# nzfeng/signed-heat-3d

Hardware: AMD Instinct MI355X
Metric: grid-nodes/sec end-to-end SHM (conv+PCG) (higher is better)
Workload: dtype f64 (Step 1: f64 / packed-f32 tiers)

## Files before the change

include/shm_grid.h:

```cpp
#ifndef SHM_GRID_H
#define SHM_GRID_H

#include <stddef.h>
#include <stdint.h>

#ifdef __cplusplus
extern "C" {
#endif

#define SHM_GRID_ABI_VERSION 5

typedef struct shm_solver shm_solver;

typedef enum {
    SHM_OK = 0,
    SHM_ERR_INVALID = 1,
    SHM_ERR_HIP = 2,
    SHM_ERR_NOMEM = 3,
    SHM_ERR_BREAKDOWN = 4,
    SHM_ERR_NOCONV = 5,
    SHM_ERR_RCCL = 6,
    SHM_ERR_STATE = 7,
    SHM_ERR_SINGULAR = 8
} shm_status;
// ... 24 lines not shown
    int32_t n;
    double bbox_min[3];
    double cell;
} shm_grid;

typedef struct {
    int32_t fast_integration;
    int32_t scrub_nonfinite;
    double tol;
    int32_t max_iters;
    int32_t check_every;
    int32_t preconditioner;
    int32_t solver;
    int32_t step1_arith;
    int32_t dual_form;
    double step1_budget;
} shm_opts;

enum { SHM_DUAL_AUTO = 0, SHM_DUAL_DIRECT = 1, SHM_DUAL_EXPLICIT_S_CG = 2, SHM_DUAL_THROUGH_GRID = 3 };

enum { SHM_STEP1_AUTO = 0, SHM_STEP1_EXACT_F64 = 1, SHM_STEP1_REFERENCE_F64 = 2 };

enum { SHM_SOLVER_AUTO = 0, SHM_SOLVER_PRIMAL = 1, SHM_SOLVER_DUAL = 2, SHM_SOLVER_DUAL_SLABS = 3 };

enum { SHM_PRECOND_AUTO = 0, SHM_PRECOND_NONE = 1, SHM_PRECOND_DCT = 2 };

typedef struct {
    int32_t n, m;
    int64_t S;
    int32_t iters;
    double rel_residual;
    double shift;
    double ms_conv;
    double ms_div;
    double ms_setup;
    double ms_wait_setup;
    double ms_pcg;
    double ms_shift;
    double ms_total;
    double ms_stencil_avg;
    double ms_update_xr_avg;
    double ms_project_avg;
    double ms_update_p_avg;
    double ms_precond_avg;
    int32_t kernel_samples;
    int32_t preconditioner;
    int32_t solver;
    double bytes_per_iter;
    int32_t cg_form;
    double pairs_fp64;
    double pairs_fp32;
    int32_t conv_launches;
    double pairs_redone;
} shm_stats;

shm_status shm_grid_create(const shm_config* cfg, shm_solver** out);
void shm_grid_destroy(shm_solver* s);
const char* shm_grid_last_error(const shm_solver* s);
int32_t shm_grid_abi_version(void);

shm_status shm_grid_set_problem(shm_solver* s, const shm_sources* src, const shm_grid* grid);
shm_status shm_grid_solve(shm_solver* s, const shm_opts* opts, shm_stats* stats);
shm_status shm_grid_get_phi(shm_solver* s, double* phi_out, int32_t* k_begin, int32_t* k_end);
shm_status shm_grid_owned_planes(shm_solver* s, int32_t* k_begin, int32_t* k_end);
shm_status shm_grid_compute_distance(shm_solver* s, const shm_sources* src, const shm_grid* grid,
                                     const shm_opts* opts, double* phi_out, shm_stats* stats);

typedef enum {
    SHM_FIELD_Y0 = 0,
    SHM_FIELD_Y1 = 1,
    SHM_FIELD_Y2 = 2,
    SHM_FIELD_DIV = 3,
    SHM_FIELD_PHI = 4
} shm_field;
shm_status shm_grid_run_conv(shm_solver* s);
shm_status shm_grid_run_conv_arith(shm_solver* s, int32_t step1_arith);
shm_status shm_grid_run_divergence(shm_solver* s, int32_t scrub);
shm_status shm_grid_get_field(shm_solver* s, shm_field f, double* out );
shm_status shm_grid_get_field_planes(shm_solver* s, shm_field f, int32_t k_begin, int32_t k_end, double* out);
shm_status shm_grid_apply_laplacian(shm_solver* s, const double* u, double* out);
shm_status shm_grid_set_phi(shm_solver* s, const double* phi );
shm_status shm_grid_get_constraints(shm_solver* s, int64_t* nodes, double* coeffs, int32_t* m);
shm_status shm_grid_get_schur(shm_solver* s, double* out, int32_t* m);
shm_status shm_grid_spd_solve(shm_solver* s, const double* S, int32_t m, const double* rhs, int32_t form, double* u, int32_t* flag);
shm_status shm_grid_apply_projector(shm_solver* s, double* v);

shm_status shm_grid_apply_preconditioner(shm_solver* s, const double* v, double* out);

enum { SHM_ISO_MARCHING_CUBES = 0, SHM_ISO_MARCHING_TETS = 1 };
shm_status shm_grid_isosurface(shm_solver* s, double isovalue, int64_t* n_vertices, int64_t* n_triangles);
shm_status shm_grid_isosurface_ex(shm_solver* s, double isovalue, int32_t method, int64_t* n_vertices, int64_t* n_triangles);
shm_status shm_grid_get_isosurface(shm_solver* s, double* vertices , int64_t* triangles );

shm_status shm_grid_sample(shm_solver* s, int64_t Q, const double* pts, double* phi_out, double* grad_out, int64_t* n_answered);
shm_status shm_grid_sample_device(shm_solver* s, int64_t Q, const void* d_pts, void* d_phi, void* d_grad, int64_t* n_answered);

shm_status shm_grid_isosurface_indexed(shm_solver* s, double isovalue, int64_t* n_vertices, int64_t* n_triangles);
shm_status shm_grid_get_isosurface_indexed(shm_solver* s, double* vertices , int64_t* triangles );
shm_status shm_grid_get_isosurface_indexed_device(shm_solver* s, void* d_vertices , void* d_triangles );

typedef struct {
    int64_t first_vertex;
    int64_t n_vertices, n_triangles;
    double  area, volume;
    double  lo[3], hi[3];
    int32_t touches_box;
    int32_t reserved;
} shm_iso_component;
shm_status shm_grid_label_mesh_device(shm_solver* s, int64_t nv, int64_t nt, const void* d_triangles , void* d_root , int64_t* n_components);
shm_status shm_grid_isosurface_components(shm_solver* s, int64_t* n_components);
shm_status shm_grid_get_isosurface_components(shm_solver* s, shm_iso_component* comps , int64_t* tri_component ,
                                              int64_t* vertex_component );
shm_status shm_grid_isosurface_keep_components(shm_solver* s, const uint8_t* keep , int64_t* n_vertices, int64_t* n_triangles);

typedef struct {
    int64_t n_audited, n_not_owned, n_nonfinite, n_out_of_zone, n_finite_mismatch;
    double  max_dy;
    int64_t worst_node;
    double  worst_ratio;
    double  min_ratio;
    double  budget;
    int32_t step1_arith;
    int32_t within_budget;
    double  ms;
} shm_step1_audit;
shm_status shm_grid_audit_step1(shm_solver* s, int64_t count, const int64_t* nodes, double* dy_out , double* ratio_out ,
                                shm_step1_audit* out);
int64_t shm_audit_sample_nodes(int32_t n, int32_t k_begin, int32_t k_end, int64_t count, uint64_t seed, int64_t* nodes_out);

shm_status shm_grid_raycast(shm_solver* s, int64_t Q, const double* origins , const double* dirs , double isovalue, double t_min, double t_max,
                            double* t_out , double* grad_out , int64_t* n_hits);
shm_status shm_grid_raycast_device(shm_solver* s, int64_t Q, const void* d_origins, const void* d_dirs, double isovalue, double t_min, double t_max, void* d_t,
                                   void* d_grad, int64_t* n_hits);

typedef struct {
    int64_t n_frozen;
    int64_t n_reached;
    int64_t n_nonfinite;
    int64_t n_block_updates;
    int32_t n_rounds;
    int32_t reserved;
    double max_abs;
    double isovalue, band;
    double ms;
} shm_redistance_stats;
shm_status shm_grid_redistance(shm_solver* s, double isovalue, double band, shm_redistance_stats* out );
shm_status shm_grid_get_redistanced(shm_solver* s, double* psi_out );
shm_status shm_grid_get_redistanced_device(shm_solver* s, void* d_psi );

typedef struct {
    int64_t n_vertices, n_triangles;
    int64_t n_reached;
    int64_t n_candidate_pairs;
    double max_abs;
    double isovalue, band;
    double ms;
} shm_redistance_exact_stats;
shm_status shm_grid_redistance_exact(shm_solver* s, double isovalue, double band, shm_redistance_exact_stats* out );
shm_status shm_grid_isosurface_indexed_psi(shm_solver* s, double distance, int64_t* n_vertices, int64_t* n_triangles);

shm_status shm_grid_closest_point(shm_solver* s, int64_t Q, const double* pts , double max_dist, double* dist_out ,
                                  double* cp_out , int64_t* tri_out , int64_t* n_answered);
shm_status shm_grid_closest_point_device(shm_solver* s, int64_t Q, const void* d_pts, double max_dist, void* d_dist, void* d_cp ,
                                         void* d_tri , int64_t* n_answered);

shm_status shm_comm_unique_id(void* out128);
// ... 9 lines not shown
```

signed-heat-3d_amd/csrc/shm_dct.hip.h:

```cpp
#pragma once
#include <hip/hip_runtime.h>
#include <stdint.h>

#include "shm_fft_core.h"
#include "shm_kernels.hip.h"

#ifndef SHM_DCT_HOIST
#define SHM_DCT_HOIST 0
#endif
#ifndef SHM_DCT_WAVES_HINT
#define SHM_DCT_WAVES_HINT 9
#endif
#ifndef SHM_DCT_WAVES_F32
#define SHM_DCT_WAVES_F32 2
#endif
#ifndef SHM_DCT_SPECTRAL_ORIG
#define SHM_DCT_SPECTRAL_ORIG 0
#endif
#ifndef SHM_DCT_RUNTIME_GATE
#define SHM_DCT_RUNTIME_GATE 1
#endif
#ifndef SHM_DCT_WAVES_256
#define SHM_DCT_WAVES_256 0
#endif
#ifndef SHM_DCT_WAVE_FFT
#define SHM_DCT_WAVE_FFT 0x100
#endif
#ifndef SHM_DCT_LC9_F64
#define SHM_DCT_LC9_F64 4
#endif
#ifndef SHM_DCT_LC10_F32
#define SHM_DCT_LC10_F32 4
#endif
#ifndef SHM_DCT_LC9_F32
#define SHM_DCT_LC9_F32 8
#endif
#ifndef SHM_DCT_LC8
#define SHM_DCT_LC8 4
#endif
#ifndef SHM_DCT_TW_LDS_MAX
#define SHM_DCT_TW_LDS_MAX 8
#endif
#ifndef SHM_DCT_POW_ALWAYS
#define SHM_DCT_POW_ALWAYS 1
#endif

namespace shm {

#if SHM_DCT_RUNTIME_GATE
#define SHM_DCT_DBG(P, bit) ((P).debug_skip & (bit))
#else
#define SHM_DCT_DBG(P, bit) 0
#endif

enum DctMode : int { DCT_FWD = 0, DCT_INV = 1, DCT_FUSED = 2 };
template <int LOG2N, int TB > constexpr int dct_lc() {
    return LOG2N >= 10 ? (TB == 8 ? 4 : SHM_DCT_LC10_F32) : (LOG2N == 8 ? SHM_DCT_LC8 : (LOG2N == 9 ? (TB == 8 ? SHM_DCT_LC9_F64 : SHM_DCT_LC9_F32) : 8));
}
constexpr int dct_lines_for(int log2n, int tb) {
    return log2n >= 10 ? (tb == 8 ? 8 : 2 * SHM_DCT_LC10_F32) : (log2n == 8 ? 2 * SHM_DCT_LC8 : (log2n == 9 ? 2 * (tb == 8 ? SHM_DCT_LC9_F64 : SHM_DCT_LC9_F32) : 16));
}

struct DctAddr {
    long long off;
    long long a_stride, b_stride;
    long long line_stride;
    long long elem_stride;
    long long seg_stride;
    int seg_shift, seg_mask;
};
struct DctParams {
    int ntiles;
    int tiles_a;
    int debug_skip;
    DctAddr in, out;
    int ky0;
    double inv_n3_8;
};
__device__ __forceinline__ long long dct_addr(const DctAddr& A, long long base, int l, int k) {
    return A.off + base + (long long)l * A.line_stride + (long long)(k >> A.seg_shift) * A.seg_stride + (long long)(k & A.seg_mask) * A.elem_stride;
}

template <int LOG2N> constexpr bool dct_tw_in_lds() { return LOG2N <= SHM_DCT_TW_LDS_MAX; }
template <int LOG2N, int TB> constexpr size_t dct_lds_bytes() {
    return ((size_t)(1 << LOG2N) * (dct_lc<LOG2N, TB>() + 1) + (dct_tw_in_lds<LOG2N>() ? (size_t)(1 << LOG2N) : 0)) * (size_t)(2 * TB) + 64;
}

template <int LOG2N, int TB> constexpr size_t dct_stage_bytes() { return (size_t)(1 << LOG2N) * (size_t)(2 * dct_lc<LOG2N, TB>()) * (size_t)TB; }

template <typename TP, int LOG2N, int R, int NS, int SIGN>
__device__ __forceinline__ void dct_fft_pass(Cplx<TP>* buf, const Cplx<TP>* tw, int tid) {
    constexpr int LC = dct_lc<LOG2N, (int)sizeof(TP)>();
    constexpr int items = PassGeom<LOG2N, R, LC>::items;
    constexpr int IPT = (items + kBlock - 1) / kBlock;
    Cplx<TP> v[IPT][R];
#pragma unroll
    for (int a = 0; a < IPT; a++) {
        const int w = tid + a * kBlock;
        if (items % kBlock == 0 || w < items) pass_load<TP, LOG2N, R, NS, SIGN, LC, SHM_DCT_POW_ALWAYS || !dct_tw_in_lds<LOG2N>()>(buf, tw, w, v[a]);
    }
    __syncthreads();
#pragma unroll
    for (int a = 0; a < IPT; a++) {
        const int w = tid + a * kBlock;
        if (items % kBlock == 0 || w < items) pass_store<TP, LOG2N, R, NS, LC>(buf, w, v[a]);
    }
    __syncthreads();
}

template <typename TP, int LOG2N, int SIGN>
__device__ __forceinline__ void dct_fft(Cplx<TP>* buf, const Cplx<TP>* tw, int tid) {
    typedef FftPlan<LOG2N> P;
    dct_fft_pass<TP, LOG2N, P::R0, 1, SIGN>(buf, tw, tid);
    if constexpr (P::npass > 1) dct_fft_pass<TP, LOG2N, P::R1, P::R0, SIGN>(buf, tw, tid);
    if constexpr (P::npass > 2) dct_fft_pass<TP, LOG2N, P::R2, P::R0 * P::R1, SIGN>(buf, tw, tid);
    if constexpr (P::npass > 3) dct_fft_pass<TP, LOG2N, P::R3, P::R0 * P::R1 * P::R2, SIGN>(buf, tw, tid);
}

template <int LOG2N> struct FftPlanWave;
template <> struct FftPlanWave<8> { static constexpr int npass = 4; static constexpr int R0 = 4, R1 = 4, R2 = 4, R3 = 4; };
#ifndef SHM_DCT_WAVE_PLAN9
#define SHM_DCT_WAVE_PLAN9 0
#endif
#if SHM_DCT_WAVE_PLAN9
template <> struct FftPlanWave<9> { static constexpr int npass = 3; static constexpr int R0 = 8, R1 = 8, R2 = 8, R3 = 1; };
#else
template <> struct FftPlanWave<9> { static constexpr int npass = 4; static constexpr int R0 = 8, R1 = 4, R2 = 4, R3 = 4; };
#endif
template <> struct FftPlanWave<10> { static constexpr int npass = 4; static constexpr int R0 = 16, R1 = 4, R2 = 4, R3 = 4; };
template <int LOG2N> constexpr bool dct_wave_fft() { return ((SHM_DCT_WAVE_FFT >> LOG2N) & 1) && LOG2N >= 8 && LOG2N <= 10; }

template <typename TP, int LOG2N, int R, int NS, int SIGN>
__device__ __forceinline__ void dct_fft_pass_wave(Cplx<TP>* buf, const Cplx<TP>* tw, int tid) {
    constexpr int LC = dct_lc<LOG2N, (int)sizeof(TP)>(), n = 1 << LOG2N;
    constexpr int B = n / R;
    constexpr int LW = LC / (kBlock / kWave);
    constexpr int IPL = (B + kWave - 1) / kWave;
    static_assert(LW >= 1 && B % kWave == 0, "wave-local FFT: whole lines per wave, full waves of butterflies");
    const int wave = tid >> 6, lane = tid & 63;
    Cplx<TP> v[LW * IPL][R];
#pragma unroll
    for (int a = 0; a < LW * IPL; a++) {
        const int c = wave + (kBlock / kWave) * (a / IPL), jj = lane + kWave * (a % IPL);
        pass_load<TP, LOG2N, R, NS, SIGN, LC, SHM_DCT_POW_ALWAYS || !dct_tw_in_lds<LOG2N>()>(buf, tw, jj * LC + c, v[a]);
    }
    __builtin_amdgcn_wave_barrier();
#pragma unroll
    for (int a = 0; a < LW * IPL; a++) {
        const int c = wave + (kBlock / kWave) * (a / IPL), jj = lane + kWave * (a % IPL);
        pass_store<TP, LOG2N, R, NS, LC>(buf, jj * LC + c, v[a]);
    }
    __builtin_amdgcn_wave_barrier();
}

template <typename TP, int LOG2N, int SIGN>
__device__ __forceinline__ void dct_fft_wave(Cplx<TP>* buf, const Cplx<TP>* tw, int tid) {
    typedef FftPlanWave<LOG2N> P;
    dct_fft_pass_wave<TP, LOG2N, P::R0, 1, SIGN>(buf, tw, tid);
    dct_fft_pass_wave<TP, LOG2N, P::R1, P::R0, SIGN>(buf, tw, tid);
    dct_fft_pass_wave<TP, LOG2N, P::R2, P::R0 * P::R1, SIGN>(buf, tw, tid);
    if constexpr (P::npass > 3) dct_fft_pass_wave<TP, LOG2N, P::R3, P::R0 * P::R1 * P::R2, SIGN>(buf, tw, tid);
}

#ifndef SHM_DCT_SEG9_ONE_WAVE
#define SHM_DCT_SEG9_ONE_WAVE 1
#endif
template <int LOG2N, int CPLX_BYTES> constexpr int dct_waves_per_simd() {
    constexpr int by_lds = (int)((size_t)(160 * 1024) / dct_lds_bytes<LOG2N, CPLX_BYTES / 2>());
    constexpr int want = LOG2N <= 8 ? (SHM_DCT_WAVES_256 > 0 ? SHM_DCT_WAVES_256 : 1) : (CPLX_BYTES == 8 ? SHM_DCT_WAVES_F32 : 2);
    return by_lds >= want ? want : (by_lds >= 1 ? by_lds : 1);
}
template <typename TP, typename TIn, typename TOut, int MODE, bool DOT, int LOG2N, bool XPASS, bool SEG, bool PF = false>
__global__ __launch_bounds__(kBlock, ((LOG2N >= SHM_DCT_WAVES_HINT || SHM_DCT_WAVES_256 > 0) && !(SHM_DCT_SEG9_ONE_WAVE && SEG && LOG2N == 9 && sizeof(TP) == 8) ? dct_waves_per_simd<LOG2N, (int)sizeof(Cplx<TP>)>() : 1)) void dct_lines_kernel(DctParams P, const TIn* __restrict__ in, TOut* __restrict__ out,
                                                           const Cplx<TP>* __restrict__ tw_g, const Cplx<TP>* __restrict__ om_g,
                                                           const TP* __restrict__ lam_g, const TOut* __restrict__ dot_with,
                                                           double* __restrict__ partials, const int* __restrict__ tile_list ,
                                                           const unsigned* __restrict__ elem_mask ) {
    extern __shared__ __attribute__((aligned(16))) char smem[];
    constexpr int LC = dct_lc<LOG2N, (int)sizeof(TP)>(), kFftRow = LC + 1, kFftLC = LC;
    constexpr int n = 1 << LOG2N, L = 2 * LC, LOG2L = ilog2(L), total = n * L;
    constexpr int EPT = (total + kBlock - 1) / kBlock;
    constexpr int CH = EPT < 16 ? EPT : 16;
    Cplx<TP>* buf = reinterpret_cast<Cplx<TP>*>(smem);
    Cplx<TP>* tw_l = buf + (size_t)n * kFftRow;
    double* red = reinterpret_cast<double*>(tw_l + (dct_tw_in_lds<LOG2N>() ? n : 0));
    const Cplx<TP>* tw = dct_tw_in_lds<LOG2N>() ? tw_l : tw_g;
    const int tid = threadIdx.x;
    if (dct_tw_in_lds<LOG2N>())
        for (int a = tid; a < n; a += kBlock) tw_l[a] = tw_g[a];
    constexpr int kSpStep = kBlock / kFftLC;
    constexpr int kSpIters = (n / 2 + 1 + kSpStep - 1) / kSpStep;
    Cplx<TP> sp_om[(MODE == DCT_FWD || !SHM_DCT_HOIST) ? 1 : kSpIters];
    TP sp_lam[(MODE == DCT_FUSED && SHM_DCT_HOIST) ? kSpIters : 1];
    TP sp_lam_n = (TP)0;
    if (MODE != DCT_FWD && SHM_DCT_HOIST) {
#pragma unroll
        for (int i = 0; i < kSpIters; i++) {
            const int k = min((tid >> ilog2(kFftLC)) + i * kSpStep, n / 2);
            sp_om[i] = om_g[k];
            if (MODE == DCT_FUSED) sp_lam[i] = lam_g[k];
        }
    }
    if (MODE == DCT_FUSED) sp_lam_n = (TP)2 * lam_g[n / 2];
    static_assert(!PF || !SEG, "the prefetching variant serves plain layouts");
    static_assert(!PF || (sizeof(TIn) == sizeof(TP) && (total * sizeof(TIn)) % (16 * kBlock) == 0), "the prefetching variant moves whole 16-byte chunks of same-width input");
    TIn* stage = reinterpret_cast<TIn*>(smem + dct_lds_bytes<LOG2N, (int)sizeof(TP)>());
    auto pf_issue = [&](int lbx) {
        if constexpr (PF) {
            constexpr int kChunkElems = 16 / (int)sizeof(TIn);
            constexpr int kChunks = total / kChunkElems, kPer = kChunks / kBlock;
            const int tx = lbx;
            const long long bin = P.in.off + (long long)(tx % P.tiles_a) * P.in.a_stride + (long long)(tx / P.tiles_a) * P.in.b_stride;
            const int wave0 = (tid >> 6) << 6;
#pragma unroll
            for (int a = 0; a < kPer; a++) {
                const int q = a * kBlock + tid;
                long long g;
                if (XPASS) {
                    constexpr int cpl = n / kChunkElems;
                    g = (long long)(q / cpl) * P.in.line_stride + (long long)((q % cpl) * kChunkElems);
                } else {
                    constexpr int cpr = L / kChunkElems;
                    g = (long long)(q / cpr) * P.in.elem_stride + (long long)((q % cpr) * kChunkElems);
                }
                __builtin_amdgcn_global_load_lds(reinterpret_cast<const char*>(in + (bin + g)), reinterpret_cast<char*>(stage) + (size_t)(a * kBlock + wave0) * 16, 16, 0, 0);
            }
        }
    };
    if (PF) {
        const int lb0 = (int)xcd_remap(blockIdx.x, gridDim.x);
        if (lb0 < P.ntiles) pf_issue(lb0);
    }
    for (int lb = (int)xcd_remap(blockIdx.x, gridDim.x); lb < P.ntiles; lb += (int)gridDim.x) {
    __syncthreads();
    const int t = tile_list ? tile_list[lb] : lb;
    const long long base_in = (long long)(t % P.tiles_a) * P.in.a_stride + (long long)(t / P.tiles_a) * P.in.b_stride;
    const long long base_out = (long long)(t % P.tiles_a) * P.out.a_stride + (long long)(t / P.tiles_a) * P.out.b_stride;

    auto line_of = [&](int idx) { return XPASS ? (idx >> LOG2N) : (idx & (L - 1)); };
    auto elem_of = [&](int idx) { return XPASS ? (idx & (n - 1)) : (idx >> LOG2L); };
    auto thread_off = [&](const DctAddr& A) -> unsigned {
        if (XPASS) return n >= kBlock ? (unsigned)(tid * A.elem_stride) : (unsigned)((tid >> LOG2N) * A.line_stride + (tid & (n - 1)) * A.elem_stride);
        return (unsigned)((tid & (L - 1)) * A.line_stride + (tid >> LOG2L) * A.elem_stride);
    };
    auto uniform_off = [&](const DctAddr& A, int a) -> long long {
        if (XPASS) {
            constexpr int per = n >= kBlock ? n / kBlock : 1, lp = n >= kBlock ? 1 : kBlock / n;
            return n >= kBlock ? (long long)(a / per) * A.line_stride + (long long)((a % per) * kBlock) * A.elem_stride : (long long)(a * lp) * A.line_stride;
        }
        return (long long)(a * (kBlock / L)) * A.elem_stride;
    };
    const unsigned toff_in = SEG ? 0u : thread_off(P.in), toff_out = SEG ? 0u : thread_off(P.out);
    auto in_at = [&](const TIn* base, int a, int idx) -> const TIn* {
        return SEG ? base + dct_addr(P.in, base_in, line_of(idx), elem_of(idx)) : (base + (P.in.off + base_in + uniform_off(P.in, a))) + toff_in;
    };
    auto out_at = [&](auto* base, int a, int idx) {
        return SEG ? base + dct_addr(P.out, base_out, line_of(idx), elem_of(idx)) : (base + (P.out.off + base_out + uniform_off(P.out, a))) + toff_out;
    };

    if constexpr (PF) {
        __builtin_amdgcn_s_waitcnt(0x0f70);
        __syncthreads();
#pragma unroll
        for (int a0 = 0; a0 < EPT; a0 += CH) {
            TP v[CH];
#pragma unroll
            for (int a = 0; a < CH; a++) v[a] = (TP)stage[tid + (a0 + a) * kBlock];
#pragma unroll
            for (int a = 0; a < CH; a++) {
                const int idx = tid + (a0 + a) * kBlock;
                const int l = line_of(idx), j = elem_of(idx);
                const int slot = (MODE == DCT_INV) ? j : makhoul_slot(j, n);
                reinterpret_cast<TP*>(&buf[slot * kFftRow + (l >> 1)])[l & 1] = v[a];
            }
        }
        __syncthreads();
        if (lb + (int)gridDim.x < P.ntiles) pf_issue(lb + (int)gridDim.x);
    } else
#pragma unroll 1
    for (int a0 = 0; a0 < EPT; a0 += CH) {
        TP v[CH];
#pragma unroll
        for (int a = 0; a < CH; a++) {
            const int idx = tid + (a0 + a) * kBlock;
            if (total % kBlock == 0 || idx < total) {
                const int j = elem_of(idx);
                v[a] = (!SHM_DCT_DBG(P, 4) && (!elem_mask || ((elem_mask[j >> 5] >> (j & 31)) & 1u))) ? (TP)*in_at(in, a0 + a, idx) : (TP)0;
            }
        }
#pragma unroll
        for (int a = 0; a < CH; a++) {
            const int idx = tid + (a0 + a) * kBlock;
            if (total % kBlock == 0 || idx < total) {
                const int l = line_of(idx), j = elem_of(idx);
                const int slot = (MODE == DCT_INV) ? j : makhoul_slot(j, n);
                reinterpret_cast<TP*>(&buf[slot * kFftRow + (l >> 1)])[l & 1] = v[a];
            }
        }
    }
    __syncthreads();

    constexpr bool kWaveFft = dct_wave_fft<LOG2N>();
    if ((MODE == DCT_FWD || MODE == DCT_FUSED) && !SHM_DCT_DBG(P, 1)) {
        if constexpr (kWaveFft) dct_fft_wave<TP, LOG2N, -1>(buf, tw, tid);
        else dct_fft<TP, LOG2N, -1>(buf, tw, tid);
    }
    if (kWaveFft && MODE == DCT_FWD) __syncthreads();

    if (MODE == DCT_FWD) {
#pragma unroll 1
        for (int a0 = 0; a0 < EPT; a0 += CH) {
#pragma unroll
            for (int a = 0; a < CH; a++) {
                const int idx = tid + (a0 + a) * kBlock;
                if (total % kBlock == 0 || idx < total) {
                    const int l = line_of(idx), k = elem_of(idx), c = l >> 1;
                    TP xa, xb;
                    dct_fwd_post<TP>(buf[k * kFftRow + c], buf[((n - k) & (n - 1)) * kFftRow + c], om_g[k], xa, xb);
                    *out_at(out, a0 + a, idx) = (TOut)((l & 1) ? xb : xa);
                }
            }
        }
        continue;
    }

#if SHM_DCT_SPECTRAL_ORIG
    if (!SHM_DCT_DBG(P, 2)) {
        const int kx0 = (t % P.tiles_a) * L, ky = P.ky0 + t / P.tiles_a;
        constexpr int pairs = (n / 2 + 1) * kFftLC;
        for (int b = tid; b < pairs; b += kBlock) {
            const int c = b & (kFftLC - 1), k = b >> ilog2(kFftLC);
            const int nk = (n - k) & (n - 1);
            const Cplx<TP> omk = om_g[k], omn = om_g[nk];
            TP xa_k, xb_k, xa_n, xb_n;
            if (MODE == DCT_FUSED) {
                const Cplx<TP> zk = buf[k * kFftRow + c], znk = buf[nk * kFftRow + c];
                dct_fwd_post<TP>(zk, znk, omk, xa_k, xb_k);
                dct_fwd_post<TP>(znk, zk, omn, xa_n, xb_n);
                const int kxa = kx0 + 2 * c, kxb = kxa + 1;
                const TP lxy_a = lam_g[kxa] + lam_g[ky], lxy_b = lam_g[kxb] + lam_g[ky];
                const TP sy = ky == 0 ? (TP)0.5 : (TP)1;
                const TP sa = (kxa == 0 ? (TP)0.5 : (TP)1) * sy * (TP)P.inv_n3_8, sb = sy * (TP)P.inv_n3_8;
                const TP lk = lam_g[k], ln = lam_g[nk];
                const TP szk = k == 0 ? (TP)0.5 : (TP)1;
                const TP da_k = lxy_a + lk, db_k = lxy_b + lk, da_n = lxy_a + ln, db_n = lxy_b + ln;
                auto recip = [](TP d) {
                    TP r = t_rcp<TP>(d);
                    r = fma(fma(-d, r, (TP)1), r, r);
                    r = fma(fma(-d, r, (TP)1), r, r);
                    return r;
                };
                xa_k = da_k > (TP)0 ? xa_k * (sa * szk) * recip(da_k) : (TP)0;
                xb_k = xb_k * (sb * szk) * recip(db_k);
                xa_n = da_n > (TP)0 ? xa_n * (sa * szk) * recip(da_n) : (TP)0;
                xb_n = xb_n * (sb * szk) * recip(db_n);
            } else {
                const Cplx<TP> rk = buf[k * kFftRow + c], rn = buf[nk * kFftRow + c];
                xa_k = rk.x; xb_k = rk.y; xa_n = rn.x; xb_n = rn.y;
            }
            buf[k * kFftRow + c] = dct_inv_pre<TP>(k, xa_k, xa_n, xb_k, xb_n, omk);
            if (nk != k) buf[nk * kFftRow + c] = dct_inv_pre<TP>(nk, xa_n, xa_k, xb_n, xb_k, omn);
        }
        __syncthreads();
    }

#else
    if (!SHM_DCT_DBG(P, 2)) {
        const int kx0 = (t % P.tiles_a) * L, ky = P.ky0 + t / P.tiles_a;
        constexpr int kSpLines = kWaveFft ? kFftLC / (kBlock / kWave) : 1;
#pragma unroll
        for (int cl = 0; cl < kSpLines; cl++) {
        const int c = kWaveFft ? (tid >> 6) + (kBlock / kWave) * cl : (tid & (kFftLC - 1));
        const int kxa = kx0 + 2 * c, kxb = kxa + 1;
        TP lxy_a = (TP)0, lxy_b = (TP)0, sa = (TP)0, sb = (TP)0;
        if (MODE == DCT_FUSED) {
            const TP lky = lam_g[ky];
            lxy_a = lam_g[kxa] + lky;
            lxy_b = lam_g[kxb] + lky;
            const TP sy = ky == 0 ? (TP)0.5 : (TP)1;
            sa = (kxa == 0 ? (TP)0.5 : (TP)1) * sy * (TP)P.inv_n3_8;
            sb = sy * (TP)P.inv_n3_8;
        }
#pragma unroll 1
        for (int i = 0; i < (kWaveFft ? (n / 2 + kWave) / kWave : kSpIters); i++) {
            const int k = kWaveFft ? (tid & 63) + i * kWave : (tid >> ilog2(kFftLC)) + i * kSpStep;
            if (k > n / 2) break;
            const int nk = (n - k) & (n - 1);
            const Cplx<TP> omk = SHM_DCT_HOIST ? sp_om[SHM_DCT_HOIST ? i : 0] : om_g[k];
            const Cplx<TP> omn = k == 0 ? omk : Cplx<TP>{-omk.y, -omk.x};
            TP xa_k, xb_k, xa_n, xb_n;
            if (MODE == DCT_FUSED) {
                const Cplx<TP> zk = buf[k * kFftRow + c], znk = buf[nk * kFftRow + c];
                dct_fwd_post<TP>(zk, znk, omk, xa_k, xb_k);
                dct_fwd_post<TP>(znk, zk, omn, xa_n, xb_n);
                const TP lk = SHM_DCT_HOIST ? sp_lam[SHM_DCT_HOIST ? i : 0] : lam_g[k], ln = k == 0 ? lk : sp_lam_n - lk;
                const TP szk = k == 0 ? (TP)0.5 : (TP)1;
                const TP da_k = lxy_a + lk, db_k = lxy_b + lk, da_n = lxy_a + ln, db_n = lxy_b + ln;
                auto recip = [](TP d) {
                    TP r = t_rcp<TP>(d);
                    r = fma(fma(-d, r, (TP)1), r, r);
                    r = fma(fma(-d, r, (TP)1), r, r);
                    return r;
                };
                xa_k = da_k > (TP)0 ? xa_k * (sa * szk) * recip(da_k) : (TP)0;
                xb_k = xb_k * (sb * szk) * recip(db_k);
                xa_n = da_n > (TP)0 ? xa_n * (sa * szk) * recip(da_n) : (TP)0;
                xb_n = xb_n * (sb * szk) * recip(db_n);
            } else {
                const Cplx<TP> rk = buf[k * kFftRow + c], rn = buf[nk * kFftRow + c];
                xa_k = rk.x; xb_k = rk.y; xa_n = rn.x; xb_n = rn.y;
            }
            buf[k * kFftRow + c] = dct_inv_pre<TP>(k, xa_k, xa_n, xb_k, xb_n, omk);
            if (nk != k) buf[nk * kFftRow + c] = dct_inv_pre<TP>(nk, xa_n, xa_k, xb_n, xb_k, omn);
        }
        }
        if (!kWaveFft) __syncthreads();
    }

#endif
    if (!SHM_DCT_DBG(P, 1)) {
        if constexpr (kWaveFft) dct_fft_wave<TP, LOG2N, +1>(buf, tw, tid);
        else dct_fft<TP, LOG2N, +1>(buf, tw, tid);
    }
    if (kWaveFft) __syncthreads();

    double acc = 0.;
#pragma unroll 1
    for (int a0 = 0; a0 < EPT; a0 += CH) {
        TOut dv[CH];
        if (DOT) {
#pragma unroll
            for (int a = 0; a < CH; a++) {
                const int idx = tid + (a0 + a) * kBlock;
                if (total % kBlock == 0 || idx < total)
                    dv[a] = *out_at(dot_with, a0 + a, idx);
            }
        }
#pragma unroll
        for (int a = 0; a < CH; a++) {
            const int idx = tid + (a0 + a) * kBlock;
            if (total % kBlock == 0 || idx < total) {
                const int l = line_of(idx), j = elem_of(idx);
                const TP v = reinterpret_cast<const TP*>(&buf[makhoul_slot(j, n) * kFftRow + (l >> 1)])[l & 1];
                if (!SHM_DCT_DBG(P, 8) && (!elem_mask || ((elem_mask[j >> 5] >> (j & 31)) & 1u))) *out_at(out, a0 + a, idx) = (TOut)v;
                if (DOT) acc += (double)v * (double)dv[a];
            }
        }
    }
    if (DOT) {
        acc = block_sum(acc, red);
        if (tid == 0) partials[t] = acc;
    }
    }
}

constexpr int kZsPer = 4;
__device__ __forceinline__ double zs_block_exclusive(double v, double* buf , double& total) {
    const int t = threadIdx.x;
    int cur = 0;
    buf[t] = v;
    __syncthreads();
    for (int off = 1; off < kBlock; off <<= 1) {
        const double x = buf[cur * kBlock + t] + (t >= off ? buf[cur * kBlock + t - off] : 0.);
        buf[(cur ^ 1) * kBlock + t] = x;
        cur ^= 1;
        __syncthreads();
    }
    const double incl = buf[cur * kBlock + t];
    total = buf[cur * kBlock + kBlock - 1];
    __syncthreads();
    return incl - v;
}
template <typename T>
__device__ void zsolve_zero_line(int n, int n_act, const int* __restrict__ planes, double inv_h2, const T* __restrict__ in, T* __restrict__ out) {
    __shared__ double fz[kBlock * kZsPer], buf[2 * kBlock];
    const int t = threadIdx.x;
    const size_t plane = (size_t)n * n;
    for (int a = t; a < kBlock * kZsPer; a += kBlock) fz[a] = 0.;
    __syncthreads();
    for (int a = t; a < n_act; a += kBlock) fz[planes[a]] = (double)in[(size_t)planes[a] * plane];
    __syncthreads();
    double f[kZsPer], loc = 0., tot = 0.;
#pragma unroll
    for (int e = 0; e < kZsPer; e++) {
        const int z = t * kZsPer + e;
        f[e] = z < n ? fz[z] : 0.;
        loc += f[e];
    }
    zs_block_exclusive(loc, buf, tot);
    const double fmean = tot / n;
    loc = 0.;
#pragma unroll
    for (int e = 0; e < kZsPer; e++) {
        const int z = t * kZsPer + e;
        f[e] = z < n ? f[e] - fmean : 0.;
        loc += f[e];
    }
    double before = zs_block_exclusive(loc, buf, tot);
    double g[kZsPer];
#pragma unroll
    for (int e = 0; e < kZsPer; e++) {
        before += f[e];
        g[e] = -before;
    }
    loc = 0.;
#pragma unroll
    for (int e = 0; e < kZsPer; e++) loc += (t * kZsPer + e < n) ? g[e] : 0.;
    before = zs_block_exclusive(loc, buf, tot);
    double u[kZsPer], usum = 0.;
#pragma unroll
    for (int e = 0; e < kZsPer; e++) {
        const int z = t * kZsPer + e;
        u[e] = before / inv_h2;
        before += z < n ? g[e] : 0.;
        usum += z < n ? u[e] : 0.;
    }
    zs_block_exclusive(usum, buf, tot);
    const double umean = tot / n;
    const double scale = 0.25 * 4.0 / ((double)n * (double)n);
#pragma unroll
    for (int e = 0; e < kZsPer; e++) fz[t * kZsPer + e] = u[e] - umean;
    __syncthreads();
    for (int a = t; a < n_act; a += kBlock) out[(size_t)planes[a] * plane] = (T)(scale * fz[planes[a]]);
}

constexpr int kZsChunk = 16;
template <typename T>
// ... 86 lines not shown
```

signed-heat-3d_amd/csrc/shm_grid.hip:

```cpp
#include "shm_host.hip.h"
#include "shm_audit_sample.h"


struct shm_solver {
    std::unique_ptr<shm::SolverBase> impl;
    std::string err;
    shm_config cfg;
};

static thread_local std::string g_create_error;

template <typename F> static shm_status guard(shm_solver* s, F&& f) {
    if (!s) return SHM_ERR_INVALID;
    try {
        f();
        s->err.clear();
        return SHM_OK;
    } catch (const shm::Error& e) {
        s->err = e.what();
        return e.code;
    } catch (const std::bad_alloc&) {
        s->err = "host allocation failed";
        return SHM_ERR_NOMEM;
    } catch (const std::exception& e) {
// ... 82 lines not shown
    return guard(s, [&] {
        if (!src || !grid) throw shm::Error(SHM_ERR_INVALID, "null argument");
        s->impl->set_problem(*src, *grid);
    });
}

shm_status shm_grid_solve(shm_solver* s, const shm_opts* opts, shm_stats* stats) {
    return guard(s, [&] {
        shm_opts o;
        memset(&o, 0, sizeof o);
        o.scrub_nonfinite = 1;
        if (opts) o = *opts;
        s->impl->solve(o, stats);
    });
}

shm_status shm_grid_get_phi(shm_solver* s, double* phi_out, int32_t* k_begin, int32_t* k_end) {
    return guard(s, [&] {
        if (!phi_out) throw shm::Error(SHM_ERR_INVALID, "null phi_out");
        s->impl->get_phi(phi_out, k_begin, k_end);
    });
}

shm_status shm_grid_owned_planes(shm_solver* s, int32_t* k_begin, int32_t* k_end) {
    return guard(s, [&] { s->impl->owned_planes(k_begin, k_end); });
}

shm_status shm_grid_compute_distance(shm_solver* s, const shm_sources* src, const shm_grid* grid, const shm_opts* opts, double* phi_out,
                                     shm_stats* stats) {
    shm_status rc = shm_grid_set_problem(s, src, grid);
    if (rc != SHM_OK) return rc;
    if (s->cfg.world != 1) {
        s->err = "shm_grid_compute_distance is the single-process entry point; use set_problem/solve/get_phi per rank";
        return SHM_ERR_INVALID;
    }
    rc = shm_grid_solve(s, opts, stats);
    if (rc != SHM_OK && rc != SHM_ERR_NOCONV) return rc;
    std::string keep = s->err;
    shm_status rc2 = shm_grid_get_phi(s, phi_out, nullptr, nullptr);
    if (rc2 != SHM_OK) return rc2;
    s->err = keep;
    return rc;
}

shm_status shm_grid_run_conv(shm_solver* s) { return guard(s, [&] { s->impl->run_conv(SHM_STEP1_AUTO); }); }
shm_status shm_grid_run_conv_arith(shm_solver* s, int32_t step1_arith) { return guard(s, [&] { s->impl->run_conv(step1_arith); }); }
shm_status shm_grid_run_divergence(shm_solver* s, int32_t scrub) { return guard(s, [&] { s->impl->run_divergence(scrub); }); }
shm_status shm_grid_get_field(shm_solver* s, shm_field f, double* out) {
    return guard(s, [&] {
        if (!out) throw shm::Error(SHM_ERR_INVALID, "null out");
        s->impl->get_field(f, out);
    });
}
shm_status shm_grid_get_field_planes(shm_solver* s, shm_field f, int32_t k_begin, int32_t k_end, double* out) {
    return guard(s, [&] {
        if (!out) throw shm::Error(SHM_ERR_INVALID, "null out");
        s->impl->get_field_planes(f, k_begin, k_end, out);
    });
}
shm_status shm_grid_apply_laplacian(shm_solver* s, const double* u, double* out) {
    return guard(s, [&] {
        if (!u || !out) throw shm::Error(SHM_ERR_INVALID, "null argument");
        s->impl->apply_laplacian(u, out);
    });
}
shm_status shm_grid_set_phi(shm_solver* s, const double* phi) {
    return guard(s, [&] {
        if (!phi) throw shm::Error(SHM_ERR_INVALID, "null argument");
        s->impl->set_phi(phi);
    });
}
shm_status shm_grid_get_constraints(shm_solver* s, int64_t* nodes, double* coeffs, int32_t* m) {
    return guard(s, [&] {
        if (!nodes || !coeffs || !m) throw shm::Error(SHM_ERR_INVALID, "null argument");
        s->impl->get_constraints(nodes, coeffs, m);
    });
}
shm_status shm_grid_get_schur(shm_solver* s, double* out, int32_t* m) {
    return guard(s, [&] {
        if (!out || !m) throw shm::Error(SHM_ERR_INVALID, "null argument");
        s->impl->get_schur(out, m);
    });
}
shm_status shm_grid_spd_solve(shm_solver* s, const double* S, int32_t m, const double* rhs, int32_t form, double* u, int32_t* flag) {
    return guard(s, [&] {
        if (!S || !rhs || !u || !flag) throw shm::Error(SHM_ERR_INVALID, "null argument");
        s->impl->spd_solve(S, m, rhs, form, u, flag);
    });
}
shm_status shm_grid_apply_projector(shm_solver* s, double* v) {
    return guard(s, [&] {
        if (!v) throw shm::Error(SHM_ERR_INVALID, "null argument");
        s->impl->apply_projector(v);
    });
}

shm_status shm_grid_apply_preconditioner(shm_solver* s, const double* v, double* out) {
    return guard(s, [&] {
        if (!v || !out) throw shm::Error(SHM_ERR_INVALID, "null argument");
        s->impl->apply_preconditioner(v, out);
    });
}

shm_status shm_grid_isosurface(shm_solver* s, double isovalue, int64_t* n_vertices, int64_t* n_triangles) {
    return guard(s, [&] { s->impl->isosurface(isovalue, SHM_ISO_MARCHING_CUBES, n_vertices, n_triangles); });
}
shm_status shm_grid_isosurface_ex(shm_solver* s, double isovalue, int32_t method, int64_t* n_vertices, int64_t* n_triangles) {
    return guard(s, [&] { s->impl->isosurface(isovalue, method, n_vertices, n_triangles); });
}
shm_status shm_grid_get_isosurface(shm_solver* s, double* vertices, int64_t* triangles) {
    return guard(s, [&] { s->impl->get_isosurface(vertices, triangles); });
}

shm_status shm_grid_isosurface_indexed(shm_solver* s, double isovalue, int64_t* n_vertices, int64_t* n_triangles) {
    return guard(s, [&] { s->impl->isosurface_indexed(isovalue, n_vertices, n_triangles); });
}
shm_status shm_grid_get_isosurface_indexed(shm_solver* s, double* vertices, int64_t* triangles) {
    return guard(s, [&] { s->impl->get_isosurface_indexed(vertices, triangles); });
}
shm_status shm_grid_get_isosurface_indexed_device(shm_solver* s, void* d_vertices, void* d_triangles) {
    return guard(s, [&] { s->impl->get_isosurface_indexed_device(d_vertices, d_triangles); });
}

shm_status shm_grid_label_mesh_device(shm_solver* s, int64_t nv, int64_t nt, const void* d_triangles, void* d_root, int64_t* n_components) {
    return guard(s, [&] { s->impl->label_mesh_device(nv, nt, d_triangles, d_root, n_components); });
}
shm_status shm_grid_isosurface_components(shm_solver* s, int64_t* n_components) {
    return guard(s, [&] { s->impl->isosurface_components(n_components); });
}
shm_status shm_grid_get_isosurface_components(shm_solver* s, shm_iso_component* comps, int64_t* tri_component, int64_t* vertex_component) {
    return guard(s, [&] { s->impl->get_isosurface_components(comps, tri_component, vertex_component); });
}
shm_status shm_grid_isosurface_keep_components(shm_solver* s, const uint8_t* keep, int64_t* n_vertices, int64_t* n_triangles) {
    return guard(s, [&] { s->impl->isosurface_keep_components(keep, n_vertices, n_triangles); });
}

shm_status shm_grid_sample(shm_solver* s, int64_t Q, const double* pts, double* phi_out, double* grad_out, int64_t* n_answered) {
    return guard(s, [&] { s->impl->sample(Q, pts, phi_out, grad_out, n_answered); });
}
shm_status shm_grid_sample_device(shm_solver* s, int64_t Q, const void* d_pts, void* d_phi, void* d_grad, int64_t* n_answered) {
    return guard(s, [&] { s->impl->sample_device(Q, d_pts, d_phi, d_grad, n_answered); });
}

shm_status shm_grid_raycast(shm_solver* s, int64_t Q, const double* origins, const double* dirs, double isovalue, double t_min, double t_max, double* t_out,
                            double* grad_out, int64_t* n_hits) {
    return guard(s, [&] { s->impl->raycast(Q, origins, dirs, isovalue, t_min, t_max, t_out, grad_out, n_hits); });
}
shm_status shm_grid_raycast_device(shm_solver* s, int64_t Q, const void* d_origins, const void* d_dirs, double isovalue, double t_min, double t_max, void* d_t,
                                   void* d_grad, int64_t* n_hits) {
    return guard(s, [&] { s->impl->raycast_device(Q, d_origins, d_dirs, isovalue, t_min, t_max, d_t, d_grad, n_hits); });
}

shm_status shm_grid_redistance(shm_solver* s, double isovalue, double band, shm_redistance_stats* out) {
    return guard(s, [&] { s->impl->redistance(isovalue, band, out); });
}
shm_status shm_grid_redistance_exact(shm_solver* s, double isovalue, double band, shm_redistance_exact_stats* out) {
    return guard(s, [&] { s->impl->redistance_exact(isovalue, band, out); });
}
shm_status shm_grid_isosurface_indexed_psi(shm_solver* s, double distance, int64_t* n_vertices, int64_t* n_triangles) {
    return guard(s, [&] { s->impl->isosurface_indexed_psi(distance, n_vertices, n_triangles); });
}
shm_status shm_grid_get_redistanced(shm_solver* s, double* psi_out) {
    return guard(s, [&] { s->impl->get_redistanced(psi_out); });
}
shm_status shm_grid_get_redistanced_device(shm_solver* s, void* d_psi) {
    return guard(s, [&] { s->impl->get_redistanced_device(d_psi); });
// ... 36 lines not shown
```

signed-heat-3d_amd/csrc/shm_host.hip.h:

```cpp
#pragma once
#include <hip/hip_runtime.h>
#include <rccl/rccl.h>

#include <dlfcn.h>

#include <algorithm>
#include <atomic>
#include <chrono>
#include <cmath>
#include <cstdarg>
#include <cstdio>
#include <cstring>
#include <limits>
#include <memory>
#include <mutex>
#include <stdexcept>
#include <string>
#include <thread>
#include <unordered_map>
#include <unordered_set>
#include <vector>

#include "../../include/shm_grid.h"
#include "shm_constraints.h"
// ... 409 lines not shown
                            lbs[(size_t)(s - g0)] = rel - lhs_drop;
                            if (lbs[(size_t)(s - g0)] <= ln_tau) {
                                bnd[(size_t)(s - g0)] = std::exp(lbs[(size_t)(s - g0)]) * r_hi / d_box;
                                gsum += bnd[(size_t)(s - g0)];
                            }
                        }
                        const bool soft_ok = R + gsum <= eps_soft;
                        if (soft_ok) R += gsum;
                        for (int64_t s = g0; s < g1; s++) {
                            if (!(wmag[(size_t)s] > 0.)) continue;
                            if (bnd[(size_t)(s - g0)] >= 0. && (soft_ok || lbs[(size_t)(s - g0)] <= ln_tau_hard)) continue;
                            const double lhs = lambda * (dist[(size_t)s] - rt - r_hi), rel = std::log(wmag[(size_t)s]) - ln_near;
                            const double d_box = std::max(0., dist[(size_t)s] - rt), d0 = std::max(0., dmin - rt);
                            const bool in_range = 1.4426950408889634 * lambda * (d_box - d0) + range_c <= std::log2(wmag[(size_t)s]) - lwhi;
                            cost += lhs > tier_log + rel && in_range ? far_cost : 1.0;
                        }
                    }
                } else {
                    for (size_t c = 0; c < crad.size(); c++) {
                        const double dx = cx - ccen[3 * c], dy = cy - ccen[3 * c + 1], dz = cz - ccen[3 * c + 2];
                        const double gap = std::sqrt(dx * dx + dy * dy + dz * dz) - rt - crad[c] - r_hi;
                        if (!(gap * lambda > skip_base + clnw[c] - ln_near)) cost += kCl;
                    }
                }
                acc += cost;
            }
        const double per_plane = acc / ((double)K * K * (double)S) + 1e-3;
        for (int k = L * bz; k < std::min(n, (L + 1) * bz); k++) weights[k] = per_plane;
    };
    const unsigned hw = std::thread::hardware_concurrency();
    const int nthr = (int)std::max(1u, std::min({hw ? hw : 1u, 16u, (unsigned)layers, (unsigned)(((double)layers * K * K * (double)S) / 2e6 + 1.)}));
    std::atomic<int> next{0};
    auto worker = [&]() {
        std::vector<double> dist((size_t)S);
        for (int L = next.fetch_add(1); L < layers; L = next.fetch_add(1)) do_layer(L, dist);
    };
    std::vector<std::thread> pool;
    for (int t = 1; t < nthr; t++) pool.emplace_back(worker);
    worker();
    for (std::thread& t : pool) t.join();
}

static void plan_slabs_weighted(int n, int nslabs, const double* w, int granule, std::vector<int32_t>& bounds) {
    bounds.assign((size_t)nslabs + 1, 0);
    bounds[(size_t)nslabs] = n;
    if (granule < 1) granule = 1;
    if ((long long)granule * nslabs > n) granule = std::max(1, n / nslabs);
    std::vector<double> cum((size_t)n + 1, 0.);
    for (int k = 0; k < n; k++) cum[(size_t)k + 1] = cum[(size_t)k] + (w && w[k] > 0. ? w[k] : 0.);
    if (!(cum[(size_t)n] > 0.))
        for (int k = 0; k <= n; k++) cum[(size_t)k] = k;
    for (int i = 1; i < nslabs; i++) {
        const double target = cum[(size_t)n] * i / nslabs;
        const int lo = bounds[(size_t)i - 1] + granule, hi = n - (nslabs - i) * granule;
        int best = lo;
        double best_err = 1e300;
        for (int k = ((lo + granule - 1) / granule) * granule; k <= hi; k += granule) {
            const double e = std::fabs(cum[(size_t)k] - target);
            if (e < best_err) {
                best_err = e;
                best = k;
            }
        }
        bounds[(size_t)i] = std::min(std::max(best, lo), std::max(lo, hi));
    }
}

struct SolverBase {
    virtual ~SolverBase() = default;
    virtual void set_problem(const shm_sources&, const shm_grid&) = 0;
    virtual void solve(const shm_opts&, shm_stats*) = 0;
    virtual void get_phi(double*, int32_t*, int32_t*) = 0;
    virtual void owned_planes(int32_t*, int32_t*) = 0;
    virtual void run_conv(int step1_arith) = 0;
    virtual void run_divergence(int scrub) = 0;
    virtual void get_field(shm_field, double*) = 0;
    virtual void get_field_planes(shm_field, int, int, double*) = 0;
    virtual void apply_laplacian(const double*, double*) = 0;
    virtual void set_phi(const double*) = 0;
    virtual void get_constraints(int64_t*, double*, int32_t*) = 0;
    virtual void apply_projector(double*) = 0;
    virtual void apply_preconditioner(const double*, double*) = 0;
    virtual void get_schur(double*, int32_t*) = 0;
    virtual void spd_solve(const double*, int32_t, const double*, int32_t, double*, int32_t*) = 0;
    virtual void isosurface(double, int, int64_t*, int64_t*) = 0;
    virtual void get_isosurface(double*, int64_t*) = 0;
    virtual void sample(int64_t, const double*, double*, double*, int64_t*) = 0;
    virtual void sample_device(int64_t, const void*, void*, void*, int64_t*) = 0;
    virtual void isosurface_indexed(double, int64_t*, int64_t*) = 0;
    virtual void get_isosurface_indexed(double*, int64_t*) = 0;
    virtual void get_isosurface_indexed_device(void*, void*) = 0;
    virtual void label_mesh_device(int64_t, int64_t, const void*, void*, int64_t*) = 0;
    virtual void isosurface_components(int64_t*) = 0;
    virtual void get_isosurface_components(shm_iso_component*, int64_t*, int64_t*) = 0;
    virtual void isosurface_keep_components(const uint8_t*, int64_t*, int64_t*) = 0;
    virtual void audit_step1(int64_t, const int64_t*, double*, double*, shm_step1_audit*) = 0;
    virtual void raycast(int64_t, const double*, const double*, double, double, double, double*, double*, int64_t*) = 0;
    virtual void raycast_device(int64_t, const void*, const void*, double, double, double, void*, void*, int64_t*) = 0;
    virtual void redistance(double, double, shm_redistance_stats*) = 0;
    virtual void get_redistanced(double*) = 0;
    virtual void get_redistanced_device(void*) = 0;
    virtual void redistance_exact(double, double, shm_redistance_exact_stats*) = 0;
    virtual void isosurface_indexed_psi(double, int64_t*, int64_t*) = 0;
    virtual void closest_point(int64_t, const double*, double, double*, double*, int64_t*, int64_t*) = 0;
    virtual void closest_point_device(int64_t, const void*, double, void*, void*, void*, int64_t*) = 0;
};

SolverBase* make_solver_f64(const shm_config& cfg);
SolverBase* make_solver_f32(const shm_config& cfg);

}
```

signed-heat-3d_amd/csrc/shm_kernels.hip.h:

```cpp
#pragma once
#include <hip/hip_runtime.h>
#include <stdint.h>

#include <type_traits>

#include "shm_constraints.h"
#include "shm_ldl_plan.h"
#include "shm_mc_table.h"

namespace shm {

constexpr int kBlock = 256;
constexpr int kMaxPartials = 8192;

__device__ __forceinline__ double wave_sum(double v) {
#pragma unroll
    for (int off = 32; off > 0; off >>= 1) v += __shfl_down(v, off, kWave);
    return v;
}

__device__ __forceinline__ double block_sum(double v, double* lds ) {
    v = wave_sum(v);
    const int lane = threadIdx.x & 63, w = threadIdx.x >> 6;
    if (lane == 0) lds[w] = v;
// ... 898 lines not shown
template <typename T>
__global__ __launch_bounds__(kBlock) void bfs_z_kernel(GridParams G, double cell, double bz, const T* __restrict__ Y0, const T* __restrict__ Y1,
                                                       const T* __restrict__ Y2, T* __restrict__ x) {
    const size_t plane = (size_t)G.n * G.n;
    const size_t ij = (size_t)blockIdx.x * kBlock + threadIdx.x;
    if (ij >= plane) return;
    const int kk0 = (G.k0 == 0) ? 1 : 0;
    double phi = -(double)x[(size_t)kk0 * plane + ij];
    for (int kk = kk0; kk < G.nzl; kk++) {
        const int k = G.k0 + kk;
        const double e2 = (k * cell + bz) - ((k - 1) * cell + bz);
        const size_t q = (size_t)(kk + 1) * plane + ij, pidx = q - plane;
        phi = phi + bfs_step<T>(Y0, Y1, Y2, pidx, q, 0., 0., e2);
        x[q] = (T)(-phi);
    }
}

constexpr int kDualBlock = 1024;

__device__ __forceinline__ double block_sum_1024(double v, double* lds ) {
    v = wave_sum(v);
    const int lane = threadIdx.x & 63, w = threadIdx.x >> 6;
    __syncthreads();
    if (lane == 0) lds[w] = v;
    __syncthreads();
    if (threadIdx.x == 0) {
        double s = 0.;
        for (int a = 0; a < kDualBlock / kWave; a++) s += lds[a];
        lds[16] = s;
    }
    __syncthreads();
    return lds[16];
}

template <typename T>
__global__ __launch_bounds__(kBlock) void scatter_rows_to_nodes_kernel(int nnodes, const uint32_t* __restrict__ node_id, const int* __restrict__ node_ptr,
                                                                       const int* __restrict__ ent_row, const double* __restrict__ ent_coef,
                                                                       const double* __restrict__ v, int accumulate, T* __restrict__ w, double scale = 1.0,
                                                                       T* __restrict__ saved = nullptr ) {
    const int t = blockIdx.x * kBlock + threadIdx.x;
    if (t >= nnodes) return;
    double s = 0.;
    for (int e = node_ptr[t]; e < node_ptr[t + 1]; e++) s += ent_coef[e] * v[ent_row[e]];
    const T old = w[node_id[t]];
    if (saved) saved[t] = old;
    w[node_id[t]] = (T)((accumulate ? (double)old : 0.) + scale * s);
}
template <typename T>
__global__ __launch_bounds__(kBlock) void restore_nodes_kernel(int nnodes, const uint32_t* __restrict__ node_id, const T* __restrict__ saved, T* __restrict__ w) {
    const int t = blockIdx.x * kBlock + threadIdx.x;
    if (t < nnodes) w[node_id[t]] = saved[t];
}

static __global__ __launch_bounds__(kBlock) void csr_matvec_kernel(int m, const int* __restrict__ ptr, const int* __restrict__ col, const double* __restrict__ val,
                                                            const double* __restrict__ x, double* __restrict__ y) {
    const int r = blockIdx.x * kBlock + threadIdx.x;
    if (r >= m) return;
    double s = 0.;
    for (int e = ptr[r]; e < ptr[r + 1]; e++) s += val[e] * x[col[e]];
    y[r] = s;
}

template <typename T>
__global__ __launch_bounds__(kBlock) void negate_kernel(size_t count, const T* __restrict__ in, T* __restrict__ out) {
    for (size_t v = (size_t)blockIdx.x * kBlock + threadIdx.x; v < count; v += (size_t)gridDim.x * kBlock) out[v] = -in[v];
}

template <typename T>
__global__ __launch_bounds__(kBlock) void sum_kernel(size_t nown, size_t off, const T* __restrict__ v, double* __restrict__ partials) {
    __shared__ double red[8];
    double acc = 0.;
    for (size_t a = (size_t)blockIdx.x * kBlock + threadIdx.x; a < nown; a += (size_t)gridDim.x * kBlock) acc += (double)v[off + a];
    acc = block_sum(acc, red);
    if (threadIdx.x == 0) partials[blockIdx.x] = acc;
}

static __global__ __launch_bounds__(kDualBlock) void dual_init_mu_kernel(int m, const double* __restrict__ sumb, double* __restrict__ mu, double* __restrict__ sc) {
    const double v = *sumb / (double)m;
    for (int a = threadIdx.x; a < m; a += kDualBlock) mu[a] = v;
    if (threadIdx.x == 0) sc[SC_SUMB] = *sumb;
}

static __global__ __launch_bounds__(kDualBlock) void dual_init_residual_kernel(int m, const double* __restrict__ g, const double* __restrict__ Smu,
                                                                        double* __restrict__ r, double* __restrict__ sc, int set_rr0 = 1) {
    __shared__ double lds[17];
    double s = 0.;
    for (int a = threadIdx.x; a < m; a += kDualBlock) s += g[a] - Smu[a];
    const double mean = block_sum_1024(s, lds) / (double)m;
    double rr = 0.;
    for (int a = threadIdx.x; a < m; a += kDualBlock) {
        const double v = g[a] - Smu[a] - mean;
        r[a] = v;
        rr += v * v;
    }
    rr = block_sum_1024(rr, lds);
    if (threadIdx.x == 0) {
        sc[SC_RR] = rr;
        if (set_rr0) sc[SC_RR0] = rr;
    }
}

static __global__ __launch_bounds__(kDualBlock) void dual_direction_kernel(int m, int init, const double* __restrict__ r, double* __restrict__ z,
                                                                    double* __restrict__ p, double* __restrict__ sc) {
    __shared__ double lds[17];
    double s = 0.;
    for (int a = threadIdx.x; a < m; a += kDualBlock) s += z[a];
    const double mean = block_sum_1024(s, lds) / (double)m;
    double rz = 0.;
    for (int a = threadIdx.x; a < m; a += kDualBlock) {
        const double v = z[a] - mean;
        z[a] = v;
        rz += r[a] * v;
    }
    rz = block_sum_1024(rz, lds);
    const double rz_old = sc[SC_RZ];
    const double beta = (init || rz_old == 0.) ? 0. : rz / rz_old;
    for (int a = threadIdx.x; a < m; a += kDualBlock) p[a] = init ? z[a] : z[a] + beta * p[a];
    __syncthreads();
    if (threadIdx.x == 0) sc[SC_RZ] = rz;
}

static __global__ __launch_bounds__(kDualBlock) void dual_update_kernel(int m, const double* __restrict__ Sp, const double* __restrict__ p, double* __restrict__ mu,
                                                                 double* __restrict__ r, double* __restrict__ sc) {
    __shared__ double lds[17];
    double s = 0.;
    for (int a = threadIdx.x; a < m; a += kDualBlock) s += Sp[a];
    const double mean = block_sum_1024(s, lds) / (double)m;
    double pSp = 0.;
    for (int a = threadIdx.x; a < m; a += kDualBlock) pSp += p[a] * (Sp[a] - mean);
    pSp = block_sum_1024(pSp, lds);
    const double rz_cur = sc[SC_RZ];
    const double alpha = rz_cur == 0. ? 0. : rz_cur / pSp;
    double rr = 0.;
    for (int a = threadIdx.x; a < m; a += kDualBlock) {
        mu[a] += alpha * p[a];
        const double v = r[a] - alpha * (Sp[a] - mean);
        r[a] = v;
        rr += v * v;
    }
    rr = block_sum_1024(rr, lds);
    if (threadIdx.x == 0) sc[SC_RR] = rr;
}

static __global__ __launch_bounds__(kBlock) void sum_slabs_kernel(int nslabs, double* const* __restrict__ bufs, int count) {
    const int a = blockIdx.x * kBlock + threadIdx.x;
    if (a >= count) return;
    double s = 0.;
    for (int t = 0; t < nslabs; t++) s += bufs[t][a];
    for (int t = 0; t < nslabs; t++) bufs[t][a] = s;
}

static __global__ __launch_bounds__(kBlock) void scatter_triplets_kernel(size_t cnt, const uint64_t* __restrict__ idx, const double* __restrict__ val,
                                                                  double* __restrict__ dense) {
    for (size_t a = (size_t)blockIdx.x * kBlock + threadIdx.x; a < cnt; a += (size_t)gridDim.x * kBlock) dense[idx[a]] = val[a];
}

template <typename TS, typename TD>
__global__ __launch_bounds__(kBlock) void convert_kernel(size_t count, const TS* __restrict__ src, TD* __restrict__ dst) {
    for (size_t v = (size_t)blockIdx.x * kBlock + threadIdx.x; v < count; v += (size_t)gridDim.x * kBlock) dst[v] = (TD)src[v];
}


struct GjBatch {
    const int* ptrI;
    const size_t* offD;
    const size_t* offW;
    double* D;
    double* P;
    double* R;
    double* C;
};
__device__ __forceinline__ int gj_batch_ld(const GjBatch& B, int a) { return (B.ptrI[a + 1] - B.ptrI[a] + kGJ - 1) / kGJ * kGJ; }

template <int E, int KR>
// ... 767 lines not shown
```

signed-heat-3d_amd/csrc/shm_plan.h:

```cpp
#pragma once
#include <algorithm>
#include <cmath>
#include <cstdint>
#include <cstdlib>
#include <cstring>

#include "../../include/shm_grid.h"
#include "shm_ldl_plan.h"

namespace shm {

enum Step1Kernel { kStep1TieredF64, kStep1TieredF32, kStep1Untiered };
enum PlanPath { kPathFast, kPathGathered, kPathDualSlabs, kPathDualLocal, kPathPrimalFused, kPathPrimalClassic };

struct PlanKnobs {
    bool no_direct = false;
    bool no_dense_s = false;
    bool dense_s_always = false;
    int s_form = 0;
    int tl_min_m = 6144;
};
template <typename Get> PlanKnobs plan_knobs(Get knob) {
    PlanKnobs k;
    k.no_direct = knob("SHM_DUAL_NO_DIRECT") != nullptr;
    k.no_dense_s = knob("SHM_DUAL_NO_DENSE_S") != nullptr;
    k.dense_s_always = knob("SHM_DUAL_DENSE_S_ALWAYS") != nullptr;
    const char* s_form = knob("SHM_S_FORM");
    if (s_form != nullptr) k.s_form = std::strcmp(s_form, "invert") == 0 ? 1 : std::strcmp(s_form, "factor") == 0 ? 2 : 0;
    if (knob("SHM_TL_MIN_M")) k.tl_min_m = atoi(knob("SHM_TL_MIN_M"));
    return k;
}

constexpr bool kSFactorDefault = true;

struct PlanIn {
    bool f64 = true;
    int n = 0;
    int64_t S = 0;
    int total_slabs = 1;
    bool full_wanted = false, fft_available = false, gemm_dct = false, fused_available = false;
    Step1Kernel step1 = kStep1Untiered;
    double conv_est_total_ms = 1e30;
    int solver = SHM_SOLVER_AUTO, preconditioner = SHM_PRECOND_AUTO, dual_form = SHM_DUAL_AUTO;
    double step1_budget = 0.;
    bool fast = false;
    PlanKnobs knobs;
    bool precond_available() const { return fft_available || gemm_dct; }
    bool tiered() const { return step1 != kStep1Untiered; }
};

struct Plan {
    shm_status status = SHM_OK;
    const char* error = nullptr;
    PlanPath path = kPathPrimalClassic;
    bool precond = false;
    bool dual_requested = false;
    int setup_prio = 1;
    bool green_early = false;
    int dual_form = SHM_DUAL_THROUGH_GRID;
    bool explicit_S = false;
    bool two_level = false;
    bool s_factor = false;
    double est_setup_ms = -1., est_step1_ms = -1.;
};

inline Plan plan_error(shm_status s, const char* msg) { Plan p; p.status = s; p.error = msg; return p; }

inline Plan plan_solve(const PlanIn& in) {
    Plan p;
    if (in.preconditioner == SHM_PRECOND_DCT) {
        if (!in.precond_available())
            return plan_error(SHM_ERR_INVALID, "DCT preconditioner needs n = 2^k in [16,1024] and a power-of-two number of EQUAL z-slabs dividing n (shm_config.slab_plan = SHM_SLAB_PLAN_EQUAL); a single z-slab serves any n in [4,1024]");
        p.precond = true;
    } else if (in.preconditioner == SHM_PRECOND_AUTO) {
        p.precond = in.precond_available();
    } else if (in.preconditioner != SHM_PRECOND_NONE) {
        return plan_error(SHM_ERR_INVALID, "unknown preconditioner");
    }
    if (in.dual_form < SHM_DUAL_AUTO || in.dual_form > SHM_DUAL_THROUGH_GRID) return plan_error(SHM_ERR_INVALID, "unknown dual_form");
    if (in.step1_budget != 0. && !(in.step1_budget >= 1e-12 && in.step1_budget <= 1e-3)) return plan_error(SHM_ERR_INVALID, "step1_budget must lie in [1e-12, 1e-3] (0: default 1e-8)");
    if (in.solver != SHM_SOLVER_AUTO && in.solver != SHM_SOLVER_PRIMAL && in.solver != SHM_SOLVER_DUAL && in.solver != SHM_SOLVER_DUAL_SLABS)
        return plan_error(SHM_ERR_INVALID, "unknown solver");
    if (in.fast) {
        p.path = kPathFast;
        return p;
    }
    const bool with_precond = in.preconditioner != SHM_PRECOND_NONE;
    const bool slab_forms_auto = in.solver == SHM_SOLVER_AUTO && with_precond && in.fft_available && in.total_slabs >= 4 && in.n >= 256 && in.n <= 512 && in.S <= 16384 &&
                                 in.dual_form != SHM_DUAL_THROUGH_GRID;
    if (in.full_wanted && !slab_forms_auto && (in.solver == SHM_SOLVER_AUTO || in.solver == SHM_SOLVER_DUAL) && with_precond) {
        p.path = kPathGathered;
        return p;
    }
    p.dual_requested = (in.solver == SHM_SOLVER_DUAL || in.solver == SHM_SOLVER_DUAL_SLABS || (in.solver == SHM_SOLVER_AUTO && with_precond)) && in.precond_available();
    bool dual = false;
    if (in.solver == SHM_SOLVER_DUAL || in.solver == SHM_SOLVER_DUAL_SLABS) {
        if (!in.precond_available())
            return plan_error(SHM_ERR_INVALID, "the dual solver needs the DCT: n = 2^k in [16,1024] and a power-of-two number of EQUAL z-slabs dividing n (shm_config.slab_plan = SHM_SLAB_PLAN_EQUAL); a single z-slab serves any n in [4,1024]");
        dual = true;
    } else if (in.solver == SHM_SOLVER_AUTO) {
        dual = in.precond_available() && with_precond;
    }
    if (dual) p.path = in.total_slabs > 1 ? kPathDualSlabs : kPathDualLocal;
    else p.path = in.fused_available ? kPathPrimalFused : kPathPrimalClassic;
    return p;
}

inline void plan_setup(const PlanIn& in, Plan& p) {
    p.setup_prio = in.step1 == kStep1TieredF64 && in.conv_est_total_ms >= 150. && in.conv_est_total_ms < 1e29 ? 0 : 1;
    const bool iterative_form = in.dual_form == SHM_DUAL_EXPLICIT_S_CG || in.dual_form == SHM_DUAL_THROUGH_GRID;
    p.green_early = !iterative_form && p.dual_requested && !in.knobs.no_direct && !in.knobs.no_dense_s && (in.total_slabs == 1 || in.fft_available) &&
                    in.precond_available() && !in.gemm_dct && in.n <= 512 && in.S > 0 && in.S <= 4096 &&
                    (in.f64 || in.step1 == kStep1TieredF32 || in.n < 512 || in.dual_form == SHM_DUAL_DIRECT);
}

inline bool plan_explicit_S(const PlanIn& in, int m, bool direct) {
    const bool off = in.knobs.no_dense_s || in.dual_form == SHM_DUAL_THROUGH_GRID;
    if (in.gemm_dct) return !off && m > 0 && m <= 16384;
    if (in.total_slabs > 1) return !off && in.fft_available && m > 0 && m <= 16384 && in.n <= 512;
    const bool asked = in.dual_form == SHM_DUAL_DIRECT || in.dual_form == SHM_DUAL_EXPLICIT_S_CG;
    const int max_m = (in.tiered() || asked) ? 16384 : 8192;
    if (off || !in.precond_available() || m <= 0 || m > max_m || in.n > 512) return false;
    if (in.knobs.dense_s_always || asked || direct) return true;
    const double md = (double)m, width = in.f64 ? 1.0 : 0.5;
    const double schur_est_ms = 2.2e-7 * md * md;
    const double dense_iter_ms = 3.6e-9 * md * md * width + 0.08;
    const double grid_iter_ms = std::max(0.15, 1.4 * std::pow((double)in.n / 512.0, 3.0) * width);
    return in.tiered() && in.conv_est_total_ms >= 3.0 * schur_est_ms && grid_iter_ms > 1.3 * dense_iter_ms;
}

template <typename Est> void plan_rows(const PlanIn& in, int m, Est step1_ms, Plan& p) {
    const bool no_direct = in.knobs.no_direct || in.dual_form == SHM_DUAL_EXPLICIT_S_CG || in.dual_form == SHM_DUAL_THROUGH_GRID;
    const int direct_max_m = in.dual_form == SHM_DUAL_DIRECT ? 16384 : 4096;
    bool direct = p.dual_requested && !no_direct && m <= direct_max_m;
    if (!direct && p.dual_requested && !no_direct && in.tiered() && in.precond_available() && !in.gemm_dct && in.n <= 512 && m > direct_max_m && m <= 16384 &&
        in.conv_est_total_ms < 1e29) {
        const double md = (double)m;
        p.est_setup_ms = 5.5e-11 * md * md * md + 1.4e-7 * md * md + 10.0 * std::pow((double)in.n / 512.0, 4.0);
        p.est_step1_ms = step1_ms();
        direct = p.est_setup_ms <= 0.38 * p.est_step1_ms;
    }
    if (!in.f64 && in.step1 != kStep1TieredF32 && in.n >= 512 && !in.gemm_dct && in.dual_form != SHM_DUAL_DIRECT) direct = false;
    direct = direct && plan_explicit_S(in, m, true);
    p.explicit_S = plan_explicit_S(in, m, direct);
    p.dual_form = direct ? SHM_DUAL_DIRECT : p.explicit_S ? SHM_DUAL_EXPLICIT_S_CG : SHM_DUAL_THROUGH_GRID;
    p.two_level = !direct && m > in.knobs.tl_min_m;
    p.s_factor = direct && (in.knobs.s_form == 2 || (in.knobs.s_form == 0 && kSFactorDefault)) && ldl_applies((m + kLdlTile - 1) / kLdlTile);
}

inline const char* plan_path_name(PlanPath path) {
    static const char* const names[] = {"fast", "gathered", "dual-slabs", "dual", "primal-fused", "primal-classic"};
    return names[path];
}

}
```

signed-heat-3d_amd/csrc/shm_solver.hip.h:

```cpp
#pragma once
#include "shm_host.hip.h"
#include "shm_kernels.hip.h"
#include "shm_conv_tiered.hip.h"
#include "shm_cg_fused.hip.h"
#include "shm_twolevel.hip.h"
#include "shm_schur.hip.h"
#include "shm_dct.hip.h"
#include "shm_dct_gemm.hip.h"
#include "shm_green_fft.hip.h"
#include "shm_sample.hip.h"
#include "shm_audit.hip.h"
#include "shm_iso_indexed.hip.h"
#include "shm_iso_components.hip.h"
#include "shm_raycast.hip.h"
#include "shm_redistance.hip.h"
#include "shm_redistance_exact.hip.h"
#include "shm_closest.hip.h"
#include "shm_plan.h"

namespace shm {

template <typename T> constexpr int vec_width() { return sizeof(T) == 8 ? 2 : 4; }

template <typename T>
// ... 44 lines not shown
    double conv_ctr[3] = {0, 0, 0};
    double conv_wscale = 1.;
    int64_t S = 0;
    std::vector<double> h_pos, h_wn, h_area;
    double area_sum = 0., conv_far_gap = 0., conv_skip_base = 3.0e38, last_host_setup_ms = 0., last_setup_wall_ms = 0.;
    double conv_tier_ring = 0.;
    double conv_tier_log = 0., conv_tier_skip_base = 3.0e38;
    double conv_drop_K = 64., conv_drop_eps64 = 2e-9, conv_drop_eps32 = 6.0e-8;
    double conv_w_span = 0.;
    DevArray<double> d_src_t;
    DevArray<float> d_clusters_t;
    int n_clusters_t = 0;
    bool conv_tiered = false;
    bool conv_tier_exact = false;
    bool conv_tiered32 = false;
    bool conv_reference = false;
    int step1_selected = SHM_STEP1_AUTO;
    int last_step1_arith = SHM_STEP1_AUTO;
    double last_step1_budget = 0.;
    bool fold_pq = false;
    int fold_pq_np = 0;
    double step1_budget = 0.;
    DevArray<unsigned long long> d_pair_counters;
    DevArray<unsigned> d_unit_counters;
    static constexpr int kMaxConvLaunches = 256;
    int conv_launch_index = 0;
    int conv_launches_last = 0;
    int n_clusters = 0;
    int conv_grid_cap = 1 << 30;
    bool o_fast_hint = false;
    int num_cus = 256;
    DevArray<T> d_src;
    DevArray<float> d_src32;
    DevArray<float> d_clusters;
    DevArray<double> d_exptab;
    std::vector<Slab<T>> slabs;
    int total_slabs = 1, first_slab = 0;
    std::vector<int32_t> slab_bounds;
    bool slabs_equal = true;
    void slab_range(int slab, int32_t* k0, int32_t* k1) const {
        *k0 = slab_bounds[(size_t)slab];
        *k1 = slab_bounds[(size_t)slab + 1];
    }
    bool have_problem = false, have_conv = false, have_div = false, have_phi = false, have_constraints = false;
    std::vector<Row> rows;
    std::vector<std::vector<ShiftItem>> shift_host;
    int m = 0, mp = 0;
    DevArray<double> Ginv, gjP, gjR, gjC;
    DevArray<float> Ginv32;
    struct TwoLevel {
        bool on = false;
        int box = 16, P = 0, nI = 0, nS = 0, nSp = 0, ysz = 0;
        DevArray<int> ptrI, ptrS, rowsI, colsS, sepRow, adj_ptr, adj_idx, colour_list, rowBox, chunkBox, chunkCol, tBox, tRow, sBox, sRow;
        DevArray<size_t> offW;
        DevArray<double> gjP, gjR, gjC;
        int nChunks = 0, nTChunks = 0, nbMax = 0;
        int schur_ptr[9] = {0, 0, 0, 0, 0, 0, 0, 0, 0};
        DevArray<size_t> offD, offE;
        DevArray<double> D, E, Tm, tbuf, ybuf, vS, uS;
        DevArray<float> D32, E32, T32;
        int colour_ptr[9] = {0, 0, 0, 0, 0, 0, 0, 0, 0};
        size_t szD = 0, szE = 0;
        TlBoxes view() const { return TlBoxes{ptrI.p, ptrS.p, offD.p, offE.p, rowsI.p, colsS.p}; }
    } tl;
    int ginv_rows = 0, ginv_ld = 0;
    DevArray<int> gjFlag;
    DevArray<double*> d_redptrs;
    DevArray<int> Bptr, Bcol;
    DevArray<double> Bval;
    bool have_B = false;
    using TP = T;
    DevArray<Cplx<TP>> d_tw, d_om;
    DevArray<TP> d_lam;
    DevArray<double> d_lam64;
    DevArray<double> gd_Cm, gd_Ct, gd_W1, gd_W2;
    DevArray<double> gs_lam, gs_ctab, gs_Cm, gs_Ct, gs_W0, gs_W1, gs_T, Sdense, d_rowT;
    DevArray<int> d_rowX;
    std::vector<double> h_gs_lam, h_gs_ctab, h_rowT;
    std::vector<Cplx<double>> h_gs_tw;
    DevArray<Cplx<double>> gs_tw;
    std::vector<int> h_rowX;
    bool have_S = false;
    DevArray<double> Sinv, Sinv_ones ;
    DevArray<double> ldlP, ldlPanels, ldlWork;
    PlanIn plan_in;
    Plan plan;
    double conv_est_total_ms = 1e30;
    int log2n = 0;
    bool precond_ready = false;
    double* h_pinned = nullptr;
    Rccl::comm_t comm = nullptr;
    int vec = 1;
    std::unique_ptr<Solver<T>> full;
    bool solve_only = false;
    bool full_problem_set = false;
    bool pool_held = false;

    explicit Solver(const shm_config& c, bool solve_only_ = false) : cfg(c), solve_only(solve_only_) {
        int ndev = 0;
        hipError_t e = hipGetDeviceCount(&ndev);
        if (e != hipSuccess || ndev <= 0)
            throw Error(SHM_ERR_HIP, fmt("no HIP device available (%s); this library has no CPU fallback",
                                          e == hipSuccess ? "device count 0" : hipGetErrorString(e)));
        if (cfg.device < 0 || cfg.device >= ndev) throw Error(SHM_ERR_INVALID, fmt("device %d out of range [0,%d)", cfg.device, ndev));
        HIPCHK(hipSetDevice(cfg.device));
        HIPCHK(hipStreamCreateWithFlags(&stream, hipStreamNonBlocking));
        {
            hipDeviceProp_t prop;
            HIPCHK(hipGetDeviceProperties(&prop, cfg.device));
            conv_grid_cap = std::max(1, prop.multiProcessorCount * 4);
            num_cus = prop.multiProcessorCount;
        }
        {
            int least = 0, greatest = 0;
            HIPCHK(hipDeviceGetStreamPriorityRange(&least, &greatest));
            HIPCHK(hipStreamCreateWithPriority(&stream2, hipStreamNonBlocking, greatest));
        }
        HIPCHK(hipHostMalloc((void**)&h_pinned, 64 * sizeof(double)));
        if (cfg.world > 1 && !cfg.rccl_unique_id) throw Error(SHM_ERR_INVALID, "world>1 needs rccl_unique_id");
        if (cfg.rccl_unique_id) {
            Rccl& R = Rccl::get();
            Rccl::unique_id id;
            memcpy(&id, cfg.rccl_unique_id, sizeof id);
            R.chk(R.CommInitRank(&comm, cfg.world, id, cfg.rank), "ncclCommInitRank");
        }
        PinnedPool::get().acquire(cfg.device);
        pool_held = true;
    }
    ~Solver() override {
        (void)hipSetDevice(cfg.device);
        if (comm) (void)Rccl::get().CommDestroy(comm);
        if (h_pinned) (void)hipHostFree(h_pinned);
        for (void* b : smp_pinned)
            if (b) (void)hipHostFree(b);
        for (void* b : ray_pinned)
            if (b) (void)hipHostFree(b);
        slabs.clear();
        if (stream) (void)hipStreamDestroy(stream);
        if (stream2) (void)hipStreamDestroy(stream2);
        if (stream3) (void)hipStreamDestroy(stream3);
        if (stream_h) (void)hipStreamDestroy(stream_h);
        if (pool_held) PinnedPool::get().release(cfg.device);
    }

    void log(const char* f, ...) {
        if (!cfg.verbose) return;
        va_list ap;
        va_start(ap, f);
        vfprintf(stderr, f, ap);
        va_end(ap);
        fputc('\n', stderr);
    }

    static int grid_for(size_t work_items, int cap = 2048) {
        size_t b = (work_items + kBlock - 1) / kBlock;
        if (b < 1) b = 1;
        if (b > (size_t)cap) b = cap;
        return (int)b;
    }

    void set_problem(const shm_sources& src, const shm_grid& g) override {
        HIPCHK(hipSetDevice(cfg.device));
        if (g.n < 2) throw Error(SHM_ERR_INVALID, "grid.n must be >= 2");
        if (!(g.cell > 0.) || !std::isfinite(g.cell)) throw Error(SHM_ERR_INVALID, "grid.cell must be positive and finite");
        if (src.S <= 0 || !src.pos || !src.wnormal || !src.area) throw Error(SHM_ERR_INVALID, "sources: S>0 and non-null arrays required");
        if (!(src.lambda > 0.) || !std::isfinite(src.lambda)) throw Error(SHM_ERR_INVALID, "sources.lambda must be positive and finite");
// ... 640 lines not shown
        HIPCHK(hipStreamSynchronize(stream));
    }

    void build_rows() {
        shm::build_rows(S, h_pos.data(), bbox_min, cell, n, rows);
        m = (int)rows.size();
        mp = ((m + kGJ - 1) / kGJ) * kGJ;
    }

    void build_shift_items(hipStream_t stream) {
        shift_host.resize(slabs.size());
        for (size_t si = 0; si < slabs.size(); si++) {
            Slab<T>& sl = slabs[si];
            shift_items_for_slab(S, h_pos.data(), h_area.data(), bbox_min, cell, n, sl.k0, sl.k1, shift_host[si]);
            sl.n_shift = (int)shift_host[si].size();
            sl.shift_items.upload(shift_host[si], stream);
        }
    }
    void upload_red_tables(hipStream_t stream) {
        std::vector<double*> ptrs;
        for (Slab<T>& sl : slabs) ptrs.push_back(sl.red.p);
        for (Slab<T>& sl : slabs) ptrs.push_back(sl.pq.p);
        d_redptrs.upload(ptrs, stream);
        HIPCHK(hipStreamSynchronize(stream));
    }
    void build_shift_items_only() {
        build_shift_items(stream);
        upload_red_tables(stream);
    }

    double estimate_step1_ms_tiered() const {
        if (S <= 0) return 0.;
        if (conv_tier_exact) {
            double nodes = 0.;
            for (const Slab<T>& sl : slabs) nodes += (double)sl.nown;
            return nodes * (double)S * 1.229e-9;
        }
        const int K = (int)std::max<int64_t>(32, std::min<int64_t>(128, 2000000 / S));
        const int64_t stride = std::max<int64_t>(1, (S * K + 1999999) / 2000000);
        uint64_t st = 0x9E3779B97F4A7C15ULL;
        auto rnd = [&]() {
            st = st * 6364136223846793005ULL + 1442695040888963407ULL;
            return (double)(st >> 11) * (1.0 / 9007199254740992.0);
        };
        const double ext = (double)(n - 1) * cell, rt2 = 2.0 * 5.17 * cell;
        const double r_near_gap = rt2 + conv_tier_log / lambda, r_keep_gap = rt2 + std::log(std::min((double)S, conv_drop_K) / (0.875 * 2e-9)) / lambda;
        std::vector<float> d2((size_t)S);
        size_t c_near = 0, c_keep = 0;
        for (int k = 0; k < K; k++) {
            const float x = (float)(bbox_min[0] + rnd() * ext), y = (float)(bbox_min[1] + rnd() * ext), z = (float)(bbox_min[2] + rnd() * ext);
            float dmin = 3.0e38f;
            for (int64_t s = 0; s < S; s += stride) {
                const float dx = x - (float)h_pos[3 * s], dy = y - (float)h_pos[3 * s + 1], dz = z - (float)h_pos[3 * s + 2];
                const float v = dx * dx + dy * dy + dz * dz;
                d2[(size_t)s] = v;
                dmin = std::min(dmin, v);
            }
            const double rn = std::sqrt((double)dmin);
            const float tn = (float)((rn + r_near_gap) * (rn + r_near_gap)), tk = (float)((rn + r_keep_gap) * (rn + r_keep_gap));
            for (int64_t s = 0; s < S; s += stride) {
                c_near += d2[(size_t)s] < tn;
                c_keep += d2[(size_t)s] < tk;
            }
        }
        const double sampled = (double)K * (double)((S + stride - 1) / stride);
        const double f_keep = (double)c_keep / sampled;
        const double f_near = conv_tiered32 ? 0. : (double)c_near / sampled;
        double nodes = 0.;
        for (const Slab<T>& sl : slabs) nodes += (double)sl.nown;
        return nodes * (double)S * (1.229e-9 * f_near + 1.84e-10 * (f_keep - f_near) + 3.3e-12);
    }
    double step1_hidden_ms(double conv_est_ms) const {
        double nodes_here = 0.;
        for (const Slab<T>& sl : slabs) nodes_here += (double)sl.nown;
        const double share = std::min(1.0, conv_est_ms / std::max(1e-30, nodes_here * (double)S / 1.2e9));
        return estimate_step1_ms_tiered() * share;
    }

    void build_constraints(const PlanIn& in, const Plan& p) {
        hipStream_t stream = stream2;
        const auto th0 = std::chrono::steady_clock::now();
        plan_in = in;
        plan = p;
        plan_setup(plan_in, plan);
        auto lap = [&](const char* what) { log("[shm]   setup %-28s %.2f ms", what, std::chrono::duration<double, std::milli>(std::chrono::steady_clock::now() - th0).count()); };
        if (plan.green_early) {
            enqueue_green_table(stream);
            if (!e_gs_done) e_gs_done.reset(new Event());
            e_gs_done->record(stream);
        }
        build_rows();
        lap("rows");
        plan_rows(plan_in, m, [&]() { return step1_hidden_ms(plan_in.conv_est_total_ms); }, plan);
        log("[shm] plan: %s, m=%d, form %s%s, precond %d, green table %s, G^-1 %s, prio %d; direct weighed: set-up alone ~%.1f ms, Step 1 ~%.1f ms",
            plan_path_name(plan.path), m, plan.dual_form == SHM_DUAL_DIRECT ? "direct" : plan.dual_form == SHM_DUAL_EXPLICIT_S_CG ? "explicit-S CG" : "through grid",
            plan.explicit_S ? " (S assembled)" : "", (int)plan.precond, plan.green_early ? "early" : "late", plan.two_level ? "two-level" : "dense", plan.setup_prio,
            plan.est_setup_ms, plan.est_step1_ms);
        const bool dual_direct = plan.dual_form == SHM_DUAL_DIRECT;
        std::vector<Row> no_rows;
        const NodeIndex index(dual_direct ? no_rows : rows);
        lap("sorted entries");
        const Csr G = dual_direct ? Csr((size_t)m) : assemble_G(rows, index);
        lap("G rows");
        DevArray<uint64_t> d_tidx;
        DevArray<double> d_tval;
        Triplets dense;
        tl.on = plan.two_level && build_two_level(G, d_tidx, d_tval);
        if (!tl.on && !dual_direct) {
            dense = dense_triplets(G, m, mp);
            upload_and_scatter_G(dense, m, mp, d_tidx, d_tval);
        }
        prepare_schur();
        if (dual_direct) {
            enqueue_schur();
            lap("explicit S and its inversion enqueued");
        } else {
            enqueue_invert_G();
            lap("G uploaded, inversion enqueued");
            enqueue_schur();
            lap("explicit S enqueued");
        }

        const Csr B = dual_direct ? Csr((size_t)m) : assemble_B(rows, index, n, cell);
        lap("B rows");
        std::vector<SlabLists> lists(slabs.size());
        for (size_t si = 0; si < slabs.size(); si++) {
            lists[si] = slab_lists(rows, slabs[si].k0, slabs[si].k1, (size_t)n * n);
            slabs[si].n_touched = (int)lists[si].node_id.size();
        }
        lap("per-slab lists");
        build_shift_items(stream);
        for (size_t si = 0; si < slabs.size(); si++) {
            Slab<T>& sl = slabs[si];
            SlabLists& L = lists[si];
            sl.row_ptr.upload(L.row_ptr, stream);
            sl.ent_node.upload(L.ent_node, stream);
            sl.ent_coef.upload(L.ent_coef, stream);
            sl.node_id.upload(L.node_id, stream);
            sl.node_ptr.upload(L.node_ptr, stream);
            sl.ent_row.upload(L.ent_row, stream);
            sl.nent_coef.upload(L.nent_coef, stream);
            sl.red.alloc((size_t)m + 1);
            sl.u.alloc((size_t)std::max(m, 1));
            sl.dv.alloc((size_t)7 * std::max(mp, 64));
            sl.touched_save.alloc((size_t)std::max(sl.n_touched, 1));
        }
        lap("slab uploads");
        if (total_slabs == 1 && fft_available() && !dual_direct) build_active_tiles(index.unode);
        lap("active tiles");
        Bptr.upload(B.ptr, stream);
        Bcol.upload(B.col, stream);
        Bval.upload(B.val, stream);
        have_B = !dual_direct;
        lap("B uploaded");
        upload_red_tables(stream);
        lap("B, reduction tables uploaded");
        last_host_setup_ms = std::chrono::duration<double, std::milli>(std::chrono::steady_clock::now() - th0).count();
        log("[shm] constraint set-up: host part %.2f ms (m=%d)", last_host_setup_ms, m);
        finish_invert_G();
        last_setup_wall_ms = std::chrono::duration<double, std::milli>(std::chrono::steady_clock::now() - th0).count();
        have_constraints = true;
    }

    void upload_and_scatter_G(const Triplets& t, int nrows, int ld, DevArray<uint64_t>& d_tidx, DevArray<double>& d_tval) {
        hipStream_t stream = stream2;
        ginv_rows = nrows;
        ginv_ld = ld;
        Ginv.alloc((size_t)ld * ld);
        HIPCHK(hipMemsetAsync(Ginv.p, 0, (size_t)ld * ld * sizeof(double), stream));
        d_tidx.upload(t.idx, stream);
        d_tval.upload(t.val, stream);
        hipLaunchKernelGGL(scatter_triplets_kernel, dim3(grid_for(t.idx.size(), 4096)), dim3(kBlock), 0, stream, (size_t)t.idx.size(), d_tidx.p, d_tval.p, Ginv.p);
        HIPCHK(hipGetLastError());
    }

    bool build_two_level(const Csr& G, DevArray<uint64_t>& d_tidx, DevArray<double>& d_tval) {
        hipStream_t stream = stream2;
        static const int box_env = knob("SHM_TL_BOX") ? atoi(knob("SHM_TL_BOX")) : 0;
        const TwoLevelPartition part = two_level_partition(rows, G, box_env);
        tl.box = part.box;
        if (!part.fits) return false;
        const int P = tl.P = part.P;
        tl.nS = part.nS;
        tl.nI = part.nI;
        tl.nSp = part.nSp;
        tl.ysz = (int)part.colsS.size();
        const size_t szD = tl.szD = part.szD, szE = tl.szE = part.szE;
        tl.nChunks = (int)part.chunkBox.size();
        tl.nTChunks = (int)part.tBox.size();
        tl.nbMax = part.nbMax;
        std::copy(part.colour_ptr, part.colour_ptr + 9, tl.colour_ptr);
        std::copy(part.schur_ptr, part.schur_ptr + 9, tl.schur_ptr);
        tl.ptrI.upload(part.ptrI, stream);
        tl.ptrS.upload(part.ptrS, stream);
        tl.rowsI.upload(part.rowsI, stream);
        tl.rowBox.upload(part.rowBox, stream);
        tl.chunkBox.upload(part.chunkBox, stream);
        tl.chunkCol.upload(part.chunkCol, stream);
        tl.tBox.upload(part.tBox, stream);
        tl.tRow.upload(part.tRow, stream);
        tl.sBox.upload(part.sBox, stream);
        tl.sRow.upload(part.sRow, stream);
        tl.offW.upload(part.offW, stream);
        tl.gjP.alloc((size_t)P * kGJ * kGJ);
        tl.gjR.alloc(std::max<size_t>(part.szW, 1));
        tl.gjC.alloc(std::max<size_t>(part.szW, 1));
        tl.colsS.upload(part.colsS, stream);
        tl.sepRow.upload(part.sepRow, stream);
        tl.adj_ptr.upload(part.adj_ptr, stream);
        tl.adj_idx.upload(part.adj_idx, stream);
        tl.colour_list.upload(part.colour_list, stream);
        tl.offD.upload(part.offD, stream);
        tl.offE.upload(part.offE, stream);
        tl.D.upload(part.hD, stream);
        tl.E.upload(part.hE, stream);
        tl.Tm.alloc(std::max<size_t>(szE, 1));
        tl.tbuf.alloc((size_t)tl.nI);
        tl.ybuf.alloc(std::max<size_t>(part.colsS.size(), 1));
        tl.vS.alloc((size_t)tl.nSp);
        tl.uS.alloc((size_t)tl.nSp);
        HIPCHK(hipMemsetAsync(tl.vS.p, 0, (size_t)tl.nSp * sizeof(double), stream));
        upload_and_scatter_G(part.F, tl.nS, tl.nSp, d_tidx, d_tval);
        gjFlag.alloc(2);
        HIPCHK(hipMemsetAsync(gjFlag.p + 1, 0, sizeof(int), stream));
        {
            const GjBatch Bt{tl.ptrI.p, tl.offD.p, tl.offW.p, tl.D.p, tl.gjP.p, tl.gjR.p, tl.gjC.p};
            const unsigned nb = (unsigned)tl.nbMax, uP = (unsigned)P;
            for (unsigned kb = 0; kb < nb; kb++) {
                hipLaunchKernelGGL(gj_pivot_kernel<4>, dim3(1, uP), dim3(256), 0, stream, (double*)nullptr, 0, (int)kb, (double*)nullptr, gjFlag.p + 1, plan.setup_prio, Bt);
                hipLaunchKernelGGL(gj_panels_kernel, dim3(nb, uP), dim3(kBlock), 0, stream, (const double*)nullptr, 0, (int)kb, (const double*)nullptr, (double*)nullptr, 0,
                                   (double*)nullptr, kGJ, 0, plan.setup_prio, Bt);
// ... 172 lines not shown
                HIPCHK(hipMemsetAsync(W1.p, 0, (size_t)n * n * P * sizeof(double), st));
                hipLaunchKernelGGL(green_symbol_kernel, dim3((unsigned)std::min(n * n, 8 * num_cus)), dim3(kBlock), 0, st, n, gs_lam.p, W0.p);
                const long long Pl = P, n1l = (long long)n1;
                auto pass = [&](bool xpass, int ntiles, int tiles_a, DctAddr in, DctAddr out, const double* src, double* dst) {
                    CosiParams C;
                    C.ntiles = ntiles;
                    C.tiles_a = tiles_a;
                    C.in = in;
                    C.out = out;
                    const dim3 g((unsigned)std::min(ntiles, 16 * num_cus));
                    const Cplx<double>*tw = gs_tw.p, *om = gs_tw.p + n;
                    int l2 = 0;
                    while ((1 << l2) < n) l2++;
#define SHM_COSI_CASE(L)                                                                                                                              \
    case L:                                                                                                                                            \
        if (xpass) hipLaunchKernelGGL((cosi_lines_kernel<L, true>), g, dim3(kBlock), 0, st, C, src, dst, tw, om, plan.setup_prio);                         \
        else hipLaunchKernelGGL((cosi_lines_kernel<L, false>), g, dim3(kBlock), 0, st, C, src, dst, tw, om, plan.setup_prio);                              \
        break;
                    switch (l2) {
                        SHM_COSI_CASE(4) SHM_COSI_CASE(5) SHM_COSI_CASE(6) SHM_COSI_CASE(7) SHM_COSI_CASE(8) SHM_COSI_CASE(9)
                        default: throw Error(SHM_ERR_INVALID, "Green's table by FFT: n out of range");
                    }
#undef SHM_COSI_CASE
                };
                auto addr = [](long long a_stride, long long b_stride, long long line_stride, long long elem_stride) {
                    DctAddr A;
                    A.off = 0; A.a_stride = a_stride; A.b_stride = b_stride; A.line_stride = line_stride; A.elem_stride = elem_stride;
                    A.seg_stride = 0; A.seg_shift = 30; A.seg_mask = 0x3fffffff;
                    return A;
                };
                const int L = kCosiL;
                pass(true, n * n / L, n * n / L, addr((long long)L * n, 0, n, 1), addr((long long)L * Pl, 0, Pl, 1), W0.p, W1.p);
                pass(false, n * (P / L), P / L, addr(L, (long long)n * Pl, 1, Pl), addr(L, n1l * Pl, 1, Pl), W1.p, W2.p);
                pass(false, (int)(n1l * Pl / L), (int)(n1l * Pl / L), addr(L, 0, 1, n1l * Pl), addr(L, 0, 1, n1l * Pl), W2.p, gs_T.p);
                HIPCHK(hipGetLastError());
                return;
            }
            HIPCHK(hipMemsetAsync(gs_Ct.p, 0, (size_t)n * P * sizeof(double), st));
            hipLaunchKernelGGL(cosine_tables_kernel, dim3(grid_for(n1 * n, 1024)), dim3(kBlock), 0, st, n, P, gs_ctab.p, gs_Cm.p, gs_Ct.p);
            hipLaunchKernelGGL(green_symbol_kernel, dim3((unsigned)std::min(n * n, 8 * num_cus)), dim3(kBlock), 0, st, n, gs_lam.p, W0.p);
            const bool narrow = plan_in.tiered();
            auto tiles = [](size_t v) { return (unsigned)((v + kGemmT - 1) / kGemmT); };
            auto gemm = [&](unsigned batches, int M, int N, int K, const double* A, int lda, long long sA, const double* B, int ldb, long long sB, double* C, int ldc, long long sC) {
                if (narrow)
                    hipLaunchKernelGGL(dgemm_rm_kernel<1>, dim3((unsigned)((N + 31) / 32), tiles((size_t)M), batches), dim3(kBlock), 0, st, M, N, K, A, lda, sA, B, ldb, sB, C, ldc, sC, plan.setup_prio);
                else
                    hipLaunchKernelGGL(dgemm_rm_kernel<4>, dim3(tiles((size_t)N), tiles((size_t)M), batches), dim3(kBlock), 0, st, M, N, K, A, lda, sA, B, ldb, sB, C, ldc, sC, plan.setup_prio);
            };
            gemm(1, n * n, P, n, W0.p, n, 0LL, gs_Ct.p, P, 0LL, W1.p, P, 0LL);
            gemm((unsigned)n, (int)n1, P, n, gs_Cm.p, n, 0LL, W1.p, P, (long long)n * P, W2.p, P, (long long)(n1 * P));
            gemm(1, (int)n1, (int)(n1 * P), n, gs_Cm.p, n, 0LL, W2.p, (int)(n1 * P), 0LL, gs_T.p, (int)(n1 * P), 0LL);
            HIPCHK(hipGetLastError());
        }
    }
    void prepare_schur() {
        hipStream_t st = stream2;
        have_S = false;
        if (!plan.explicit_S) return;
        if (!plan.green_early) enqueue_green_table(st);
        schur_row_order(rows, h_rowX, h_rowT);
        d_rowX.upload(h_rowX, st);
        d_rowT.upload(h_rowT, st);
        Sdense.alloc((size_t)mp * mp);
        if (!stream3) {
            int least = 0, greatest = 0;
            HIPCHK(hipDeviceGetStreamPriorityRange(&least, &greatest));
            HIPCHK(hipStreamCreateWithPriority(&stream3, hipStreamNonBlocking, greatest));
            e_sch_in.reset(new Event());
            e_sch_done.reset(new Event());
        }
        e_sch_in->record(st);
    }
    void enqueue_schur() {
        if (!plan.explicit_S) return;
        const bool dual_direct = plan.dual_form == SHM_DUAL_DIRECT;
        hipStream_t st = dual_direct ? stream2 : stream3;
        HIPCHK(hipStreamWaitEvent(st, e_sch_in->e, 0));
        const int P = n + 8;
        if (plan.green_early) HIPCHK(hipStreamWaitEvent(st, e_gs_done->e, 0));
        HIPCHK(hipMemsetAsync(Sdense.p, 0, (size_t)mp * mp * sizeof(double), st));
        const unsigned mt = (unsigned)((m + 15) / 16);
        hipLaunchKernelGGL(schur_assemble_kernel, dim3(mt, mt), dim3(kBlock), 0, st, m, mp, n, P, d_rowX.p, d_rowT.p, gs_T.p, Sdense.p, plan.setup_prio);
        HIPCHK(hipGetLastError());
        if (dual_direct) {
            Sinv.alloc((size_t)mp * mp);
            HIPCHK(hipMemcpyAsync(Sinv.p, Sdense.p, (size_t)mp * mp * sizeof(double), hipMemcpyDeviceToDevice, st));
            if (mp > m) hipLaunchKernelGGL(set_diagonal_kernel, dim3((unsigned)((mp - m + kBlock - 1) / kBlock)), dim3(kBlock), 0, st, Sinv.p, mp, m, mp, 1.0);
            if (plan.s_factor) enqueue_ldl_factor(Sinv.p, mp, ldlP, ldlPanels);
            else enqueue_gj_invert(Sinv.p, mp, true);
            Sinv_ones.alloc((size_t)2 * mp);
            hipLaunchKernelGGL(fill_kernel, dim3((unsigned)((m + kBlock - 1) / kBlock)), dim3(kBlock), 0, st, Sinv_ones.p + mp, m, 1.0);
            if (plan.s_factor) {
                ldlWork.alloc((size_t)3 * mp);
                apply_ldl(st, m, mp, Sinv.p, ldlP.p, ldlWork.p, Sinv_ones.p + mp, Sinv_ones.p);
            } else launch_ginv_matvec<double>(st, m, m, mp, Sinv.p, Sinv_ones.p + mp, Sinv_ones.p);
        } else {
            e_sch_done->record(st);
            HIPCHK(hipStreamWaitEvent(stream2, e_sch_done->e, 0));
        }
        have_S = true;
    }
    void finish_invert_G() {
        hipStream_t stream = stream2;
        int flag[2] = {0, 0};
        if (!tl.on) HIPCHK(hipMemsetAsync(gjFlag.p + 1, 0, sizeof(int), stream));
        HIPCHK(hipMemcpyAsync(flag, gjFlag.p, 2 * sizeof(int), hipMemcpyDeviceToHost, stream));
        HIPCHK(hipStreamSynchronize(stream));
        if (flag[0] || flag[1]) throw Error(SHM_ERR_SINGULAR, "A A^T is not positive definite (duplicate or degenerate constraint rows)");
    }

    void allreduce(int which , int count) {
        auto buf = [&](Slab<T>& sl) { return which == 0 ? sl.red.p : sl.pq.p; };
        if (slabs.size() > 1) {
            double** slot = d_redptrs.p + (which ? slabs.size() : 0);
            hipLaunchKernelGGL(sum_slabs_kernel, dim3((count + kBlock - 1) / kBlock), dim3(kBlock), 0, stream, (int)slabs.size(), slot, count);
        }
        if (comm) {
            Rccl& R = Rccl::get();
            R.chk(R.AllReduce(buf(slabs[0]), buf(slabs[0]), (size_t)count, Rccl::kFloat64, Rccl::kSum, comm, stream), "ncclAllReduce");
            for (size_t s = 1; s < slabs.size(); s++)
                HIPCHK(hipMemcpyAsync(buf(slabs[s]), buf(slabs[0]), (size_t)count * sizeof(double), hipMemcpyDeviceToDevice, stream));
        }
    }

    void halo_exchange_p() { halo_exchange(ARR_P); }
    void halo_exchange(int sel) { halo_exchange(sel, stream); }
    void halo_exchange(int sel, hipStream_t stream) {
        const size_t pb = slabs[0].plane * sizeof(T);
        for (size_t s = 0; s + 1 < slabs.size(); s++) {
            Slab<T>&a = slabs[s], &b = slabs[s + 1];
            HIPCHK(hipMemcpyAsync(arr(b, sel), arr(a, sel) + (size_t)a.nzl * a.plane, pb, hipMemcpyDeviceToDevice, stream));
            HIPCHK(hipMemcpyAsync(arr(a, sel) + (size_t)(a.nzl + 1) * a.plane, arr(b, sel) + b.plane, pb, hipMemcpyDeviceToDevice, stream));
        }
        if (comm) {
            Rccl& R = Rccl::get();
            const int dt = sizeof(T) == 8 ? Rccl::kFloat64 : Rccl::kFloat32;
            Slab<T>&lo = slabs.front(), &hi = slabs.back();
            const size_t cnt = lo.plane;
            R.chk(R.GroupStart(), "ncclGroupStart");
            if (cfg.rank > 0) {
                R.chk(R.Send(arr(lo, sel) + lo.plane, cnt, dt, cfg.rank - 1, comm, stream), "ncclSend(lo)");
                R.chk(R.Recv(arr(lo, sel), cnt, dt, cfg.rank - 1, comm, stream), "ncclRecv(lo)");
            }
            if (cfg.rank < cfg.world - 1) {
                R.chk(R.Send(arr(hi, sel) + (size_t)hi.nzl * hi.plane, cnt, dt, cfg.rank + 1, comm, stream), "ncclSend(hi)");
                R.chk(R.Recv(arr(hi, sel) + (size_t)(hi.nzl + 1) * hi.plane, cnt, dt, cfg.rank + 1, comm, stream), "ncclRecv(hi)");
            }
            R.chk(R.GroupEnd(), "ncclGroupEnd");
        }
    }

    struct StencilLaunch {
        dim3 grid, block;
        int xchunks, yblocks, zc;
    };
    StencilLaunch stencil_dims(const Slab<T>& sl) const {
        const int per_row = (n + vec - 1) / vec;
        int tx = 1;
        while (tx < per_row && tx < kBlock) tx <<= 1;
        const int tyb = kBlock / tx;
        const int xchunks = (per_row + tx - 1) / tx;
        const int yblocks = (n + tyb * kStRY - 1) / (tyb * kStRY);
        int zc = 16;
        while (zc > 4 && (long long)xchunks * yblocks * ((sl.nzl + zc - 1) / zc) < 1024) zc >>= 1;
        const int zchunks = (sl.nzl + zc - 1) / zc;
        return {dim3((unsigned)(xchunks * yblocks * zchunks)), dim3((unsigned)tx, (unsigned)tyb), xchunks, yblocks, zc};
// ... 143 lines not shown
        log2n = 0;
        while ((1 << log2n) < n) log2n++;
        std::vector<Cplx<TP>> tw(n), om(n);
        std::vector<TP> lam(n);
        const double pi = 3.14159265358979323846;
        for (int k = 0; k < n; k++) {
            tw[k] = {(TP)std::cos(-2. * pi * k / n), (TP)std::sin(-2. * pi * k / n)};
            om[k] = {(TP)std::cos(-pi * k / (2. * n)), (TP)std::sin(-pi * k / (2. * n))};
            lam[k] = (TP)((2. - 2. * std::cos(pi * k / n)) / (cell * cell));
        }
        d_tw.upload(tw, stream);
        d_om.upload(om, stream);
        d_lam.upload(lam, stream);
        std::vector<double> lam64(n);
        for (int k = 0; k < n; k++) lam64[k] = (2. - 2. * std::cos(pi * k / n)) / (cell * cell);
        d_lam64.upload(lam64, stream);
        for (Slab<T>& sl : slabs) {
            if (!gemm_dct()) sl.W1.alloc(sl.nown);
            if (total_slabs > 1) sl.W2.alloc(sl.nown);
            sl.z.alloc(sl.ntot);
            HIPCHK(hipMemsetAsync(sl.z.p, 0, sl.ntot * sizeof(T), stream));
        }
        if (gemm_dct()) {
            std::vector<double> ctab(4 * (size_t)n);
            for (int r = 0; r < 4 * n; r++) ctab[(size_t)r] = std::cos(pi * r / (2. * n));
            DevArray<double> d_ctab;
            d_ctab.upload(ctab, stream);
            gd_Cm.alloc((size_t)n * n);
            gd_Ct.alloc((size_t)n * n);
            gd_W1.alloc((size_t)n * n * n);
            gd_W2.alloc((size_t)n * n * n);
            hipLaunchKernelGGL(dct_matrix_kernel, dim3(grid_for((size_t)n * n, 1024)), dim3(kBlock), 0, stream, n, d_ctab.p, gd_Cm.p, gd_Ct.p);
            HIPCHK(hipGetLastError());
            HIPCHK(hipStreamSynchronize(stream));
        }
        HIPCHK(hipStreamSynchronize(stream));
        precond_ready = true;
    }

    void launch_dgemm(hipStream_t st, bool narrow, int prio, unsigned batches, int M, int N, int K, const double* A, int lda, long long sA, const double* B, int ldb,
                      long long sB, double* C, int ldc, long long sC) {
        auto tiles = [](size_t v) { return (unsigned)((v + kGemmT - 1) / kGemmT); };
        if (narrow)
            hipLaunchKernelGGL(dgemm_rm_kernel<1>, dim3((unsigned)((N + 31) / 32), tiles((size_t)M), batches), dim3(kBlock), 0, st, M, N, K, A, lda, sA, B, ldb, sB, C, ldc, sC, prio);
        else
            hipLaunchKernelGGL(dgemm_rm_kernel<4>, dim3(tiles((size_t)N), tiles((size_t)M), batches), dim3(kBlock), 0, st, M, N, K, A, lda, sA, B, ldb, sB, C, ldc, sC, prio);
    }

    int launch_precond_gemm(bool dot, int in_sel, int out_sel) {
        Slab<T>& sl = slabs[0];
        const size_t N3 = (size_t)n * n * n;
        const int nn = n, n2 = n * n;
        double *W1 = gd_W1.p, *W2 = gd_W2.p;
        const double* X;
        double* Z;
        if constexpr (sizeof(T) == 8) {
            X = reinterpret_cast<const double*>(arr(sl, in_sel)) + sl.plane;
            Z = reinterpret_cast<double*>(arr(sl, out_sel)) + sl.plane;
        } else {
            hipLaunchKernelGGL((convert_kernel<T, double>), dim3(grid_for(N3, 4096)), dim3(kBlock), 0, stream, N3, arr(sl, in_sel) + sl.plane, W2);
            X = W2;
            Z = W2;
        }
        auto gemm = [&](unsigned batches, int M, int Nc, int K, const double* A, int lda, long long sA, const double* B, int ldb, long long sB, double* C, int ldc, long long sC) {
            launch_dgemm(stream, false, 0, batches, M, Nc, K, A, lda, sA, B, ldb, sB, C, ldc, sC);
        };
        gemm(1, n2, nn, nn, X, nn, 0LL, gd_Ct.p, nn, 0LL, W1, nn, 0LL);
        gemm((unsigned)n, nn, nn, nn, gd_Cm.p, nn, 0LL, W1, nn, (long long)n2, W2, nn, (long long)n2);
        gemm(1, nn, n2, nn, gd_Cm.p, nn, 0LL, W2, n2, 0LL, W1, n2, 0LL);
        hipLaunchKernelGGL(spectral_scale_kernel, dim3(grid_for(N3, 4096)), dim3(kBlock), 0, stream, n, d_lam64.p, W1);
        gemm(1, nn, n2, nn, gd_Ct.p, nn, 0LL, W1, n2, 0LL, W2, n2, 0LL);
        gemm((unsigned)n, nn, nn, nn, gd_Ct.p, nn, 0LL, W2, nn, (long long)n2, W1, nn, (long long)n2);
        gemm(1, n2, nn, nn, W1, nn, 0LL, gd_Cm.p, nn, 0LL, Z, nn, 0LL);
        if constexpr (sizeof(T) != 8) hipLaunchKernelGGL((convert_kernel<double, T>), dim3(grid_for(N3, 4096)), dim3(kBlock), 0, stream, N3, W2, arr(sl, out_sel) + sl.plane);
        int np = 0;
        if (dot) {
            np = grid_for(N3, 2048);
            hipLaunchKernelGGL((dot_partial_kernel<T>), dim3(np), dim3(kBlock), 0, stream, N3, arr(sl, in_sel) + sl.plane, arr(sl, out_sel) + sl.plane, sl.partials.p);
        }
        return np;
    }

    template <int MODE, typename TIn, typename TOut, bool DOT, int LOG2N, bool XPASS>
    void launch_dct_n(const DctParams& P, int ntiles, const TIn* in, TOut* out, const TOut* dotw, double* partials, const int* tile_list, const unsigned* elem_mask) {
        constexpr bool kCanSeg = !XPASS && MODE != DCT_FUSED && !DOT;
        const bool seg = P.in.seg_shift < 30 || P.out.seg_shift < 30;
        if (seg && !kCanSeg) throw Error(SHM_ERR_INVALID, "DCT: segmented layout in a sweep that does not support it");
        if constexpr (kCanSeg) {
            if (seg) {
                launch_dct_pf<MODE, TIn, TOut, DOT, LOG2N, XPASS, true, false>(P, ntiles, in, out, dotw, partials, tile_list, elem_mask);
                return;
            }
        }
        launch_dct_pf<MODE, TIn, TOut, DOT, LOG2N, XPASS, false, false>(P, ntiles, in, out, dotw, partials, tile_list, elem_mask);
    }
    template <int MODE, typename TIn, typename TOut, bool DOT, int LOG2N, bool XPASS, bool SEG, bool PF>
    void launch_dct_pf(const DctParams& P, int ntiles, const TIn* in, TOut* out, const TOut* dotw, double* partials, const int* tile_list, const unsigned* elem_mask) {
        static uint64_t configured = 0;
        constexpr size_t lds = dct_lds_bytes<LOG2N, (int)sizeof(TP)>() + (PF ? dct_stage_bytes<LOG2N, (int)sizeof(TP)>() : 0);
        const uint64_t dev_bit = 1ull << (cfg.device & 63);
        if (!(configured & dev_bit) || cfg.device >= 64) {
            HIPCHK(hipFuncSetAttribute(reinterpret_cast<const void*>(&dct_lines_kernel<TP, TIn, TOut, MODE, DOT, LOG2N, XPASS, SEG, PF>), hipFuncAttributeMaxDynamicSharedMemorySize, (int)lds));
            configured |= dev_bit;
        }
        DctParams Q = P;
        Q.ntiles = ntiles;
        Q.debug_skip = 0;
        hipLaunchKernelGGL((dct_lines_kernel<TP, TIn, TOut, MODE, DOT, LOG2N, XPASS, SEG, PF>), dim3((unsigned)ntiles), dim3(kBlock), lds, stream, Q, in, out, d_tw.p, d_om.p, d_lam.p, dotw,
                           partials, tile_list, elem_mask);
    }
    template <int MODE, typename TIn, typename TOut, bool DOT, bool XPASS>
    void launch_dct(const DctParams& P, int ntiles, const TIn* in, TOut* out, const TOut* dotw, double* partials, const int* tile_list = nullptr,
                    const unsigned* elem_mask = nullptr) {
        switch (log2n) {
            case 4: launch_dct_n<MODE, TIn, TOut, DOT, 4, XPASS>(P, ntiles, in, out, dotw, partials, tile_list, elem_mask); break;
            case 5: launch_dct_n<MODE, TIn, TOut, DOT, 5, XPASS>(P, ntiles, in, out, dotw, partials, tile_list, elem_mask); break;
            case 6: launch_dct_n<MODE, TIn, TOut, DOT, 6, XPASS>(P, ntiles, in, out, dotw, partials, tile_list, elem_mask); break;
            case 7: launch_dct_n<MODE, TIn, TOut, DOT, 7, XPASS>(P, ntiles, in, out, dotw, partials, tile_list, elem_mask); break;
            case 8: launch_dct_n<MODE, TIn, TOut, DOT, 8, XPASS>(P, ntiles, in, out, dotw, partials, tile_list, elem_mask); break;
            case 9: launch_dct_n<MODE, TIn, TOut, DOT, 9, XPASS>(P, ntiles, in, out, dotw, partials, tile_list, elem_mask); break;
            case 10: launch_dct_n<MODE, TIn, TOut, DOT, 10, XPASS>(P, ntiles, in, out, dotw, partials, tile_list, elem_mask); break;
            default: throw Error(SHM_ERR_INVALID, "DCT preconditioner: unsupported grid size");
        }
    }

    static DctAddr plain_addr(long long off, long long a_stride, long long b_stride, long long line_stride, long long elem_stride) {
        DctAddr A{};
        A.off = off; A.a_stride = a_stride; A.b_stride = b_stride; A.line_stride = line_stride; A.elem_stride = elem_stride;
        A.seg_stride = 0; A.seg_shift = 30; A.seg_mask = (1 << 30) - 1;
        return A;
    }

    void alltoall_blocks(bool w1_to_w2, size_t blk) {
        auto srcp = [&](Slab<T>& sl) { return w1_to_w2 ? sl.W1.p : sl.W2.p; };
        auto dstp = [&](Slab<T>& sl) { return w1_to_w2 ? sl.W2.p : sl.W1.p; };
        const int ls = cfg.local_slabs;
        for (int a = 0; a < ls; a++)
            for (int b = 0; b < ls; b++)
                HIPCHK(hipMemcpyAsync(dstp(slabs[b]) + (size_t)(first_slab + a) * blk, srcp(slabs[a]) + (size_t)(first_slab + b) * blk, blk * sizeof(T),
                                      hipMemcpyDeviceToDevice, stream));
        if (comm) {
            Rccl& R = Rccl::get();
            const int dt = sizeof(T) == 8 ? Rccl::kFloat64 : Rccl::kFloat32;
            R.chk(R.GroupStart(), "ncclGroupStart");
            for (int peer = 0; peer < cfg.world; peer++) {
                if (peer == cfg.rank) continue;
                for (int a = 0; a < ls; a++)
                    for (int b = 0; b < ls; b++)
                        R.chk(R.Send(srcp(slabs[a]) + (size_t)(peer * ls + b) * blk, blk, dt, peer, comm, stream), "ncclSend(a2a)");
                for (int b = 0; b < ls; b++)
                    for (int a = 0; a < ls; a++)
                        R.chk(R.Recv(dstp(slabs[a]) + (size_t)(peer * ls + b) * blk, blk, dt, peer, comm, stream), "ncclRecv(a2a)");
            }
            R.chk(R.GroupEnd(), "ncclGroupEnd");
        }
    }

    enum ArrSel { ARR_R = 0, ARR_Z = 1, ARR_P = 2, ARR_X = 3, ARR_Q = 4, ARR_Y0 = 5, ARR_Y1 = 6, ARR_Y2 = 7 };
    static T* arr(Slab<T>& sl, int sel) {
        switch (sel) {
            case ARR_R: return sl.r.p;
            case ARR_Z: return sl.z.p;
            case ARR_P: return sl.p.p;
            case ARR_X: return sl.x.p;
            case ARR_Y0: return sl.Y0.p;
            case ARR_Y1: return sl.Y1.p;
            case ARR_Y2: return sl.Y2.p;
            default: return sl.q.p;
        }
    }
    int launch_precond(bool dot, int in_sel = ARR_R, int out_sel = ARR_Z, double scale = 1.0 ) {
        if (gemm_dct()) {
            if (scale != 1.0) throw Error(SHM_ERR_INVALID, "launch_precond: no scale on the dense-product transforms");
            return launch_precond_gemm(dot, in_sel, out_sel);
        }
        const long long nn = n, plane = (long long)n * n;
        const int P = total_slabs;
        const int nzl = n / P, nyl = n / P;
        const double inv8 = scale * 8.0 / ((double)n * n * n);
        const int kDctLines = dct_lines_for(log2n, (int)sizeof(TP));
        const int tiles_slab = (int)((long long)nzl * nn / kDctLines);
        int log2nyl = 0;
        while ((1 << log2nyl) < nyl) log2nyl++;
        const long long blk = (long long)nzl * nyl * nn;
        for (int pass = 0; pass < 7; pass++) {
            if (P == 1 && (pass == 2 || pass == 4)) continue;
            if (pass == 2) { alltoall_blocks(false, (size_t)blk); continue; }
            if (pass == 4) { alltoall_blocks(true, (size_t)blk); continue; }
            for (size_t si = 0; si < slabs.size(); si++) {
                Slab<T>& sl = slabs[si];
                const int g = first_slab + (int)si;
                DctParams Q{};
                Q.inv_n3_8 = inv8;
                Q.ky0 = 0;
                switch (pass) {
                    case 0:
                        Q.tiles_a = tiles_slab;
                        Q.in = plain_addr((long long)sl.plane, (long long)kDctLines * nn, 0, nn, 1);
                        Q.out = plain_addr(0, (long long)kDctLines * nn, 0, nn, 1);
                        launch_dct<DCT_FWD, T, TP, false, true>(Q, tiles_slab, arr(sl, in_sel), sl.W1.p, (const TP*)nullptr, nullptr);
                        break;
                    case 1:
                        Q.tiles_a = n / kDctLines;
                        Q.in = plain_addr(0, kDctLines, plane, 1, nn);
                        if (P == 1) {
                            Q.out = Q.in;
                            launch_dct<DCT_FWD, TP, TP, false, false>(Q, tiles_slab, sl.W1.p, sl.W1.p, (const TP*)nullptr, nullptr);
                        } else {
                            Q.out = plain_addr(0, kDctLines, (long long)nyl * nn, 1, nn);
                            Q.out.seg_shift = log2nyl; Q.out.seg_mask = nyl - 1; Q.out.seg_stride = blk;
                            launch_dct<DCT_FWD, TP, TP, false, false>(Q, tiles_slab, sl.W1.p, sl.W2.p, (const TP*)nullptr, nullptr);
                        }
                        break;
                    case 3: {
                        Q.tiles_a = n / kDctLines;
                        Q.in = plain_addr(0, kDctLines, nn, 1, (long long)nyl * nn);
                        Q.out = Q.in;
                        Q.ky0 = g * nyl;
                        const int tiles_z = (n / kDctLines) * nyl;
                        launch_dct<DCT_FUSED, TP, TP, false, false>(Q, tiles_z, sl.W1.p, sl.W1.p, (const TP*)nullptr, nullptr);
                        break;
                    }
                    case 5:
                        Q.tiles_a = n / kDctLines;
                        Q.out = plain_addr(0, kDctLines, plane, 1, nn);
                        if (P == 1) {
                            Q.in = Q.out;
                            launch_dct<DCT_INV, TP, TP, false, false>(Q, tiles_slab, sl.W1.p, sl.W1.p, (const TP*)nullptr, nullptr);
                        } else {
                            Q.in = plain_addr(0, kDctLines, (long long)nyl * nn, 1, nn);
                            Q.in.seg_shift = log2nyl; Q.in.seg_mask = nyl - 1; Q.in.seg_stride = blk;
                            launch_dct<DCT_INV, TP, TP, false, false>(Q, tiles_slab, sl.W2.p, sl.W1.p, (const TP*)nullptr, nullptr);
                        }
                        break;
                    case 6:
                        Q.tiles_a = tiles_slab;
                        Q.in = plain_addr(0, (long long)kDctLines * nn, 0, nn, 1);
                        Q.out = plain_addr((long long)sl.plane, (long long)kDctLines * nn, 0, nn, 1);
                        if (dot) launch_dct<DCT_INV, TP, T, true, true>(Q, tiles_slab, sl.W1.p, arr(sl, out_sel), arr(sl, in_sel), sl.partials.p);
                        else launch_dct<DCT_INV, TP, T, false, true>(Q, tiles_slab, sl.W1.p, arr(sl, out_sel), (const T*)nullptr, nullptr);
                        break;
                    default: break;
                }
            }
        }
        return dot ? tiles_slab : 0;
    }

    struct SolveClock {
        Event e_start, e_conv, e_div;
        Event e_s2a, e_s2b;
        Event e_setup;
        std::chrono::steady_clock::time_point wall0 = std::chrono::steady_clock::now();
        bool has_step1 = true;
        bool has_setup = true;
    };
    void fill_phase_stats(shm_stats* st, SolveClock& c, Event& e_pcg, Event& e_end, int iters, double rel_residual) {
        const auto wall1 = std::chrono::steady_clock::now();
        memset(st, 0, sizeof *st);
        st->n = n;
        st->S = S;
        st->iters = iters;
        st->rel_residual = rel_residual;
        st->shift = h_pinned[SC_SHIFT];
        if (c.has_step1) {
            st->ms_conv = elapsed(c.e_start, c.e_conv);
            st->ms_div = elapsed(c.e_conv, c.e_div);
        }
        if (c.has_setup) {
            st->m = m;
            HIPCHK(hipEventSynchronize(c.e_s2b.e));
            st->ms_setup = last_setup_wall_ms;
            if (c.has_step1) st->ms_wait_setup = elapsed(c.e_div, c.e_setup);
        }
        st->ms_pcg = elapsed(c.has_setup ? c.e_setup : c.e_div, e_pcg);
        st->ms_shift = elapsed(e_pcg, e_end);
        st->ms_total = std::chrono::duration<double, std::milli>(wall1 - c.wall0).count();
    }
    struct Residual {
        double rr0 = 0., rr = 0.;
        bool finite = true;
        double rel() const { return rr0 > 0. ? std::sqrt(std::fabs(rr / rr0)) : 0.; }
        bool below(double tol) const { return rr <= tol * tol * rr0; }
    };
    Residual fetch_residual(int extra_slot = -1 ) {
        HIPCHK(hipMemcpyAsync(h_pinned, slabs[0].sc.p, SC_COUNT * sizeof(double), hipMemcpyDeviceToHost, stream));
        HIPCHK(hipStreamSynchronize(stream));
        Residual r;
        r.rr0 = h_pinned[SC_RR0];
        r.rr = h_pinned[SC_RR];
        r.finite = std::isfinite(r.rr) && std::isfinite(r.rr0) && (extra_slot < 0 || std::isfinite(h_pinned[extra_slot]));
        return r;
    }
    void throw_loop_end(const char* name, bool breakdown, bool converged, int it, const Residual& r, const shm_opts& o) {
        if (breakdown) throw Error(SHM_ERR_BREAKDOWN, fmt("%s broke down at iteration %d (rr=%g, rr0=%g)", name, it, r.rr, r.rr0));
        if (!converged) throw Error(SHM_ERR_NOCONV, fmt("%s: max_iters=%d reached, rel. residual %.3e > tol %.1e", name, o.max_iters, r.rel(), o.tol));
    }
    struct SampleTimer {
        std::vector<std::unique_ptr<Event>> ev;
        const int max_samples, per;
        int n = 0;
        bool on = false;
        SampleTimer(bool enabled, int max_samples_, int events_per_sample) : max_samples(max_samples_), per(events_per_sample) {
            if (enabled) for (int a = 0; a < per * max_samples; a++) ev.emplace_back(new Event());
        }
        bool begin(bool wanted = true) { return on = !ev.empty() && n < max_samples && wanted; }
        void mark(int k, hipStream_t st) { if (on) ev[(size_t)(per * n + k)]->record(st); }
        void end() { if (on) n++; on = false; }
        double avg(int i, int j) const {
            double a = 0.;
            for (int q = 0; q < n; q++) a += elapsed(*ev[(size_t)(per * q + i)], *ev[(size_t)(per * q + j)]);
            return n ? a / n : 0.;
        }
    };
    void primal_prologue(bool pre, std::vector<int>& nparts, std::vector<int>& zparts) {
        for (size_t s = 0; s < slabs.size(); s++) {
            Slab<T>& sl = slabs[s];
            HIPCHK(hipMemsetAsync(sl.x.p, 0, sl.ntot * sizeof(T), stream));
            nparts[s] = stream_grid(sl);
            if (vec == 1) launch_norm2<1>(sl, sl.r.p, nparts[s]);
            else launch_norm2<vec_width<T>()>(sl, sl.r.p, nparts[s]);
        }
        launch_projection(nparts, false, 2);
        if (pre) {
            const int np = launch_precond(true);
            for (auto& v : zparts) v = np;
            launch_projection(zparts, true, 0);
        }
// ... 17 lines not shown
        Event e_int, e_end;
        build_shift_items_only();
        Rccl* R = comm ? &Rccl::get() : nullptr;
        const int dt = sizeof(T) == 8 ? Rccl::kFloat64 : Rccl::kFloat32;
        for (size_t si = 0; si < slabs.size(); si++) {
            Slab<T>& sl = slabs[si];
            if (sl.k0 == 0) {
                hipLaunchKernelGGL((bfs_plane0_kernel<T>), dim3(1), dim3(std::min(1024, ((n + 63) / 64) * 64)), 0, stream, n, cell, bbox_min[0], bbox_min[1],
                                   sl.Y0.p, sl.Y1.p, sl.Y2.p, sl.x.p);
            } else if (si == 0) {
                R->chk(R->Recv(sl.x.p, sl.plane, dt, cfg.rank - 1, comm, stream), "ncclRecv(bfs)");
            }
            hipLaunchKernelGGL((bfs_z_kernel<T>), dim3((unsigned)((sl.plane + kBlock - 1) / kBlock)), dim3(kBlock), 0, stream, sl.gp, cell, bbox_min[2], sl.Y0.p,
                               sl.Y1.p, sl.Y2.p, sl.x.p);
            const T* top = sl.x.p + (size_t)sl.nzl * sl.plane;
            if (si + 1 < slabs.size()) HIPCHK(hipMemcpyAsync(slabs[si + 1].x.p, top, sl.plane * sizeof(T), hipMemcpyDeviceToDevice, stream));
            else if (comm && cfg.rank < cfg.world - 1) R->chk(R->Send(top, sl.plane, dt, cfg.rank + 1, comm, stream), "ncclSend(bfs)");
        }
        HIPCHK(hipGetLastError());
        e_int.record(stream);
        launch_shift_and_phi();
        e_end.record(stream);
        fetch_residual();
        have_phi = true;
        if (st) {
            fill_phase_stats(st, clk, e_int, e_end, 0, 0.);
            st->preconditioner = SHM_PRECOND_NONE;
        }
    }

    void build_active_tiles(const std::vector<int64_t>& touched_nodes) {
        Slab<T>& sl = slabs[0];
        const int L = dct_lines_for(log2n_of(n), (int)sizeof(TP));
        const ActiveTiles at = active_tiles(touched_nodes, n, L);
        sl.act_z.upload(at.zmask, stream2);
        sl.n_act_planes = (int)at.planes.size();
        sl.act_planes.upload(at.planes, stream2);
        sl.n_act_x = (int)at.ax.size();
        sl.n_act_y = (int)at.ay.size();
        sl.act_x.upload(at.ax, stream2);
        sl.act_y.upload(at.ay, stream2);
        sl.S1.alloc(sl.nown);
        sl.S2.alloc(sl.nown);
        sl.S4.alloc(sl.nown);
        sl.W1.alloc(sl.nown);
        HIPCHK(hipMemsetAsync(sl.S1.p, 0, sl.nown * sizeof(T), stream2));
        HIPCHK(hipStreamSynchronize(stream2));
    }
    static int log2n_of(int v) {
        int l = 0;
        while ((1 << l) < v) l++;
        return l;
    }
    void launch_precond_sparse(int in_sel, int out_sel) {
        Slab<T>& sl = slabs[0];
        const long long nn = n, plane = (long long)n * n;
        const int L = dct_lines_for(log2n, (int)sizeof(TP));
        const int tiles_all = (int)(plane * nn / L / nn);
        DctParams Q{};
        Q.inv_n3_8 = 8.0 / ((double)n * n * n);
        Q.ky0 = 0;
        Q.tiles_a = tiles_all;
        Q.in = plain_addr((long long)sl.plane, (long long)L * nn, 0, nn, 1);
        Q.out = plain_addr(0, (long long)L * nn, 0, nn, 1);
        launch_dct<DCT_FWD, T, TP, false, true>(Q, sl.n_act_x, arr(sl, in_sel), sl.S1.p, (const TP*)nullptr, nullptr, sl.act_x.p);
        Q.tiles_a = n / L;
        Q.in = plain_addr(0, L, plane, 1, nn);
        Q.out = Q.in;
        launch_dct<DCT_FWD, TP, TP, false, false>(Q, sl.n_act_y, sl.S1.p, sl.S2.p, (const TP*)nullptr, nullptr, sl.act_y.p);
        Q.in = plain_addr(0, L, nn, 1, plane);
        Q.out = Q.in;
        if (n < 256) launch_dct<DCT_FUSED, TP, TP, false, false>(Q, tiles_all, sl.S2.p, sl.W1.p, (const TP*)nullptr, nullptr, nullptr, sl.act_z.p);
        else {
            hipLaunchKernelGGL((zsolve_sparse_kernel<TP>), dim3((unsigned)((plane + kBlock - 1) / kBlock) + 1), dim3(kBlock), 0, stream, n, sl.n_act_planes,
                               sl.act_planes.p, d_lam64.p, sl.gp.inv_h2, sl.S2.p, sl.W1.p);
        }
        Q.in = plain_addr(0, L, plane, 1, nn);
        Q.out = Q.in;
        launch_dct<DCT_INV, TP, TP, false, false>(Q, sl.n_act_y, sl.W1.p, sl.S4.p, (const TP*)nullptr, nullptr, sl.act_y.p);
        Q.tiles_a = tiles_all;
        Q.in = plain_addr(0, (long long)L * nn, 0, nn, 1);
        Q.out = plain_addr((long long)sl.plane, (long long)L * nn, 0, nn, 1);
        launch_dct<DCT_INV, TP, T, false, true>(Q, sl.n_act_x, sl.S4.p, arr(sl, out_sel), (const T*)nullptr, nullptr, sl.act_x.p);
    }

    void solve_dual(const shm_opts& o, shm_stats* st, SolveClock& clk) {
        Event e_pcg, e_end;
        const int check_every = o.check_every > 0 ? std::min(o.check_every, 4) : 2;
        auto mv = [&](Slab<T>& sl, int k) { return sl.dv.p + (size_t)k * mp; };
        enum { V_MU = 0, V_R = 1, V_P = 2, V_Z = 3, V_T1 = 4, V_T2 = 5, V_G = 6 };
        const std::vector<int> nopart(slabs.size(), 0);
        auto gather = [&](int sel) {
            for (Slab<T>& sl : slabs)
                hipLaunchKernelGGL((gather_rows_kernel<T>), dim3(1 + (8 * m + kBlock - 1) / kBlock), dim3(kBlock), 0, stream, m, sl.row_ptr.p, sl.ent_node.p,
                                   sl.ent_coef.p, arr(sl, sel), sl.partials.p, 0, sl.red.p);
            allreduce(0, 1 + m);
        };
        auto scatter = [&](int vec, int sel, int accumulate, double scale = 1.0, bool save = false) {
            for (Slab<T>& sl : slabs)
                hipLaunchKernelGGL((scatter_rows_to_nodes_kernel<T>), dim3((sl.n_touched + kBlock - 1) / kBlock + 1), dim3(kBlock), 0, stream, sl.n_touched,
                                   sl.node_id.p, sl.node_ptr.p, sl.ent_row.p, sl.nent_coef.p, mv(sl, vec), accumulate, arr(sl, sel), scale, save ? sl.touched_save.p : (T*)nullptr);
        };
        auto precondition = [&](int init) {
            for (Slab<T>& sl : slabs) {
                apply_Ginv(mv(sl, V_R), mv(sl, V_T1), true, stream);
                hipLaunchKernelGGL(csr_matvec_kernel, dim3((m + kBlock - 1) / kBlock), dim3(kBlock), 0, stream, m, Bptr.p, Bcol.p, Bval.p, mv(sl, V_T1), mv(sl, V_T2));
                apply_Ginv(mv(sl, V_T2), mv(sl, V_Z), true, stream);
                hipLaunchKernelGGL(dual_direction_kernel, dim3(1), dim3(kDualBlock), 0, stream, m, init, mv(sl, V_R), mv(sl, V_Z), mv(sl, V_P), sl.sc.p);
            }
        };
        launch_precond(false, ARR_R, ARR_Z);
        gather(ARR_Z);
        for (Slab<T>& sl : slabs) {
            HIPCHK(hipMemcpyAsync(mv(sl, V_G), sl.red.p + 1, (size_t)m * sizeof(double), hipMemcpyDeviceToDevice, stream));
            if (sl.div_sum_blocks > 0) {
                hipLaunchKernelGGL(finalize_sum_kernel, dim3(1), dim3(kBlock), 0, stream, sl.div_partials.p, sl.div_sum_blocks, sl.pq.p);
                continue;
            }
            const int g = grid_for(sl.nown, 1024);
            hipLaunchKernelGGL((sum_kernel<T>), dim3(g), dim3(kBlock), 0, stream, sl.nown, sl.plane, sl.r.p, sl.partials.p);
            hipLaunchKernelGGL(finalize_sum_kernel, dim3(1), dim3(kBlock), 0, stream, sl.partials.p, g, sl.pq.p);
        }
        allreduce(1, 1);
        for (Slab<T>& sl : slabs) {
            hipLaunchKernelGGL(dual_init_mu_kernel, dim3(1), dim3(kDualBlock), 0, stream, m, sl.pq.p, mv(sl, V_MU), sl.sc.p);
        }
        const bool sparse_ok = total_slabs == 1 && slabs[0].n_act_x > 0;
        const bool dense_S = have_S;
        if (!dense_S)
            for (Slab<T>& sl : slabs) HIPCHK(hipMemsetAsync(sl.p.p, 0, sl.ntot * sizeof(T), stream));
        auto apply_S = [&](int vec) {
            for (Slab<T>& sl : slabs) launch_ginv_matvec<double>(stream, m, m, mp, Sdense.p, mv(sl, vec), sl.red.p + 1);
        };
        if (dense_S) apply_S(V_MU);
        else {
            scatter(V_MU, ARR_P, 0);
            if (sparse_ok) launch_precond_sparse(ARR_P, ARR_Z);
            else launch_precond(false, ARR_P, ARR_Z);
            gather(ARR_Z);
        }
        for (Slab<T>& sl : slabs)
            hipLaunchKernelGGL(dual_init_residual_kernel, dim3(1), dim3(kDualBlock), 0, stream, m, mv(sl, V_G), sl.red.p + 1, mv(sl, V_R), sl.sc.p, 1);
        const bool direct = plan.dual_form == SHM_DUAL_DIRECT && dense_S;
        if (!direct) precondition(1);
        HIPCHK(hipGetLastError());

        SampleTimer tm(st != nullptr, 32, 3);
        int it = 0;
        Residual res;
        bool converged = false, breakdown = false;
        auto finish = [&]() {
            if (gemm_dct()) {
                for (Slab<T>& sl : slabs)
                    hipLaunchKernelGGL((negate_kernel<T>), dim3(grid_for(sl.ntot, 4096)), dim3(kBlock), 0, stream, sl.ntot, sl.r.p, sl.q.p);
                scatter(V_MU, ARR_Q, 1);
                launch_precond(false, ARR_Q, ARR_X);
            } else {
                scatter(V_MU, ARR_R, 1, -1.0, true);
                launch_precond(false, ARR_R, ARR_X, -1.0);
                for (Slab<T>& sl : slabs)
                    hipLaunchKernelGGL((restore_nodes_kernel<T>), dim3((sl.n_touched + kBlock - 1) / kBlock + 1), dim3(kBlock), 0, stream, sl.n_touched, sl.node_id.p,
                                       sl.touched_save.p, sl.r.p);
            }
            gather(ARR_X);
            for (Slab<T>& sl : slabs) hipLaunchKernelGGL(finalize_sum_kernel, dim3(1), dim3(kBlock), 0, stream, sl.red.p + 1, m, sl.sc.p + SC_AXSUM);
            e_pcg.record(stream);
            launch_shift_and_phi();
            e_end.record(stream);
            return fetch_residual();
        };
        bool finished = false;
        if (direct) {
            auto apply_Sinv = [&](const double* w, double* u) {
                if (plan.s_factor) apply_ldl(stream, m, mp, Sinv.p, ldlP.p, ldlWork.p, w, u);
                else launch_ginv_matvec<double>(stream, m, m, mp, Sinv.p, w, u);
            };
            const int max_passes = std::min(o.max_iters, 6);
            double rr_prev = -1.;
            while (it < max_passes && !converged && !breakdown) {
                tm.begin();
                tm.mark(0, stream);
                for (Slab<T>& sl : slabs) {
                    apply_Sinv(mv(sl, V_R), mv(sl, V_T1));
                    hipLaunchKernelGGL(dual_bordered_kernel, dim3(1), dim3(kDualBlock), 0, stream, m, mv(sl, V_T1), Sinv_ones.p, (const double*)nullptr, 1, mv(sl, V_MU));
                }
                tm.mark(1, stream);
                apply_S(V_MU);
                for (Slab<T>& sl : slabs)
                    hipLaunchKernelGGL(dual_init_residual_kernel, dim3(1), dim3(kDualBlock), 0, stream, m, mv(sl, V_G), sl.red.p + 1, mv(sl, V_R), sl.sc.p, 0);
                tm.mark(2, stream);
                tm.end();
                it++;
                HIPCHK(hipGetLastError());
                res = finish();
                finished = true;
                if (!res.finite) breakdown = true;
                else if (res.below(o.tol)) converged = true;
                else if (rr_prev >= 0. && res.rr > 0.0625 * rr_prev && res.rr <= 1e-18 * res.rr0) converged = true;
                rr_prev = res.rr;
                log("[shm] dual (direct) pass=%d rel_res=%.3e", it, res.rel());
            }
        }
        while (!direct && it < o.max_iters && !converged && !breakdown) {
            const int batch_end = std::min(o.max_iters, it + check_every);
            for (; it < batch_end; it++) {
                tm.begin();
                if (!dense_S) scatter(V_P, ARR_P, 0);
                tm.mark(0, stream);
                if (dense_S) apply_S(V_P);
                else if (sparse_ok) launch_precond_sparse(ARR_P, ARR_Z);
                else launch_precond(false, ARR_P, ARR_Z);
                tm.mark(1, stream);
                if (!dense_S) gather(ARR_Z);
                for (Slab<T>& sl : slabs)
                    hipLaunchKernelGGL(dual_update_kernel, dim3(1), dim3(kDualBlock), 0, stream, m, sl.red.p + 1, mv(sl, V_P), mv(sl, V_MU), mv(sl, V_R), sl.sc.p);
                precondition(0);
                tm.mark(2, stream);
                tm.end();
            }
            HIPCHK(hipGetLastError());
            res = fetch_residual(SC_RZ);
            if (!res.finite) breakdown = true;
            else if (res.below(o.tol)) converged = true;
            log("[shm] dual it=%d rel_res=%.3e", it, res.rel());
        }
        if (!finished) finish();
        have_phi = true;
        have_div = false;
        if (st) {
            fill_phase_stats(st, clk, e_pcg, e_end, it, res.rel());
            st->shift += h_pinned[SC_AXSUM] / (double)m;
            st->ms_precond_avg = tm.avg(0, 1);
            st->ms_project_avg = tm.avg(1, 2);
            st->kernel_samples = tm.n;
            st->preconditioner = SHM_PRECOND_DCT;
            st->solver = total_slabs > 1 ? SHM_SOLVER_DUAL_SLABS : SHM_SOLVER_DUAL;
            if (direct) {
                st->bytes_per_iter = 2.0 * (double)m * m * sizeof(double);
                st->cg_form = 2;
            } else if (dense_S) {
                st->bytes_per_iter = (double)m * m * (sizeof(double) + 2.0 * sizeof(float));
                st->cg_form = 3;
            } else if (sparse_ok) {
                const double L = dct_lines_for(log2n, (int)sizeof(TP)), tile_bytes = L * n * sizeof(TP);
                const double planes_active = (double)slabs[0].n_act_y / (n / L);
                st->bytes_per_iter = 4.0 * slabs[0].n_act_x * tile_bytes + 4.0 * slabs[0].n_act_y * tile_bytes + 2.0 * planes_active * n * n * sizeof(TP);
            } else {
                st->bytes_per_iter = (double)N * (3.0 * sizeof(T) + 8.0 * sizeof(TP)) - (double)N * sizeof(T);
            }
        }
        throw_loop_end("dual CG", breakdown, converged, it, res, o);
    }

    void solve_gathered(const shm_opts& o, const PlanIn& in, shm_stats* st, SolveClock& clk) {
        Solver<T>& F = *full;
        Slab<T>& fs = F.slabs[0];
        Event e_gather;
        SolveClock fclk;
        fclk.wall0 = clk.wall0;
        fclk.has_step1 = false;
        fclk.e_s2a.record(F.stream2);
        PlanIn fin = in;
        fin.total_slabs = 1; fin.fft_available = F.fft_available(); fin.gemm_dct = F.gemm_dct();
        fin.step1 = in.tiered() ? kStep1TieredF64 : kStep1Untiered;
        Plan fplan;
        fplan.path = kPathGathered; fplan.dual_requested = true;
        F.build_constraints(fin, fplan);
        fclk.e_s2b.record(F.stream2);
        F.setup_precond();
        const size_t plane = (size_t)n * n;
        for (Slab<T>& sl : slabs)
            HIPCHK(hipMemcpyAsync(fs.r.p + (size_t)(sl.k0 + 1) * plane, sl.r.p + plane, sl.nown * sizeof(T), hipMemcpyDeviceToDevice, stream));
        if (comm) {
            Rccl& R = Rccl::get();
            const int dt = sizeof(T) == 8 ? Rccl::kFloat64 : Rccl::kFloat32;
            R.chk(R.GroupStart(), "ncclGroupStart");
            for (int peer = 0; peer < cfg.world; peer++) {
                if (peer == cfg.rank) continue;
                for (Slab<T>& sl : slabs) R.chk(R.Send(sl.r.p + plane, sl.nown, dt, peer, comm, stream), "ncclSend(gather b)");
                for (int b = 0; b < cfg.local_slabs; b++) {
                    int32_t k0, k1;
                    slab_range(peer * cfg.local_slabs + b, &k0, &k1);
                    R.chk(R.Recv(fs.r.p + (size_t)(k0 + 1) * plane, (size_t)(k1 - k0) * plane, dt, peer, comm, stream), "ncclRecv(gather b)");
                }
            }
            R.chk(R.GroupEnd(), "ncclGroupEnd");
        }
        e_gather.record(stream);
        HIPCHK(hipStreamWaitEvent(F.stream, e_gather.e, 0));
        fclk.e_start.record(F.stream);
        fclk.e_setup.record(F.stream);
        F.have_div = true;
        F.sum_b_in_div_order(fs, F.stream);
        shm_stats cst;
        memset(&cst, 0, sizeof cst);
        bool noconv = false;
        std::string noconv_msg;
        try {
            F.solve_dual(o, &cst, fclk);
        } catch (const Error& e) {
            if (e.code != SHM_ERR_NOCONV) throw;
            noconv = true;
            noconv_msg = e.what();
        }
        for (Slab<T>& sl : slabs)
            HIPCHK(hipMemcpyAsync(sl.q.p + plane, fs.q.p + (size_t)(sl.k0 + 1) * plane, sl.nown * sizeof(T), hipMemcpyDeviceToDevice, stream));
        HIPCHK(hipStreamSynchronize(stream));
        have_phi = true;
        if (st) {
            *st = cst;
// ... 330 lines not shown
        if (kb) *kb = slabs.front().k0;
        if (ke) *ke = slabs.back().k1;
    }

    void get_field(shm_field f, double* out) override {
        need_problem();
        HIPCHK(hipSetDevice(cfg.device));
        if ((f == SHM_FIELD_Y0 || f == SHM_FIELD_Y1 || f == SHM_FIELD_Y2) && !have_conv) throw Error(SHM_ERR_STATE, "Y not computed");
        if (f == SHM_FIELD_DIV && !have_div) throw Error(SHM_ERR_STATE, "divergence not computed");
        if (f == SHM_FIELD_PHI && !have_phi) throw Error(SHM_ERR_STATE, "phi not computed");
        copy_owned_to_host((int)f, out);
    }

    void get_field_planes(shm_field f, int ka, int kb, double* out) override {
        need_problem();
        HIPCHK(hipSetDevice(cfg.device));
        if ((f == SHM_FIELD_Y0 || f == SHM_FIELD_Y1 || f == SHM_FIELD_Y2) && !have_conv) throw Error(SHM_ERR_STATE, "Y not computed");
        if (f == SHM_FIELD_DIV && !have_div) throw Error(SHM_ERR_STATE, "divergence not computed");
        if (f == SHM_FIELD_PHI && !have_phi) throw Error(SHM_ERR_STATE, "phi not computed");
        if (ka < slabs.front().k0 || kb > slabs.back().k1 || kb < ka) throw Error(SHM_ERR_INVALID, "plane range outside the planes this process owns");
        copy_planes_to_host((int)f, ka, kb, out);
    }

    void upload_owned(const double* in, int which) {
        std::vector<T> tmp;
        for (Slab<T>& sl : slabs) {
            tmp.assign(sl.ntot, (T)0);
            const int klo = std::max(0, sl.k0 - 1), khi = std::min(n, sl.k1 + 1);
            for (int k = klo; k < khi; k++)
                for (size_t a = 0; a < sl.plane; a++) tmp[(size_t)(k - sl.k0 + 1) * sl.plane + a] = (T)in[(size_t)k * sl.plane + a];
            T* dst = which == 0 ? sl.p.p : which == 1 ? sl.r.p : sl.q.p;
            HIPCHK(hipMemcpyAsync(dst, tmp.data(), sl.ntot * sizeof(T), hipMemcpyHostToDevice, stream));
            HIPCHK(hipStreamSynchronize(stream));
        }
    }

    void apply_laplacian(const double* u, double* out) override {
        need_problem();
        if (cfg.world != 1) throw Error(SHM_ERR_INVALID, "apply_laplacian is a single-process test entry point");
        HIPCHK(hipSetDevice(cfg.device));
        upload_owned(u, 0);
        for (Slab<T>& sl : slabs)
            hipLaunchKernelGGL((laplacian_kernel<T>), dim3(grid_for(sl.nown, 4096)), dim3(kBlock), 0, stream, sl.gp, sl.p.p, sl.q.p);
        HIPCHK(hipGetLastError());
        copy_owned_to_host(SHM_FIELD_PHI, out);
        have_phi = false;
        iso_idx_valid = false;
        ray_bricks_valid = false;
        redist_valid = false;
    }

    void set_phi(const double* phi) override {
        need_problem();
        if (cfg.world != 1) throw Error(SHM_ERR_INVALID, "set_phi is a single-process test entry point");
        HIPCHK(hipSetDevice(cfg.device));
        upload_owned(phi, 2);
        have_phi = true;
        iso_idx_valid = false;
        cmp_valid = false;
        ray_bricks_valid = false;
        redist_valid = false;
    }

    void get_constraints(int64_t* nodes, double* coeffs, int32_t* m_out) override {
        need_problem();
        build_rows();
        for (int r = 0; r < m; r++)
            for (int e = 0; e < 8; e++) {
                nodes[8 * (size_t)r + e] = rows[r].nodes[e];
                coeffs[8 * (size_t)r + e] = rows[r].coeffs[e];
            }
        *m_out = m;
    }

    void get_schur(double* out, int32_t* m_out) override {
        need_problem();
        if (cfg.world != 1) throw Error(SHM_ERR_INVALID, "get_schur is a single-process test entry point");
        HIPCHK(hipSetDevice(cfg.device));
        build_constraints(plan_inputs(nullptr), Plan());
        *m_out = m;
        if (!have_S) throw Error(SHM_ERR_STATE, "no explicit Schur complement for this problem (several slabs, more than 16384 rows, or n = 2^k where the plan applies S through the grid: n > 512, or the estimate of plan_explicit_S without SHM_DUAL_DENSE_S_ALWAYS)");
        HIPCHK(hipMemcpy2DAsync(out, (size_t)m * sizeof(double), Sdense.p, (size_t)mp * sizeof(double), (size_t)m * sizeof(double), (size_t)m, hipMemcpyDeviceToHost, stream2));
        HIPCHK(hipStreamSynchronize(stream2));
    }

    void spd_solve(const double* S, int32_t m_, const double* rhs, int32_t form, double* u, int32_t* flag) override {
        if (cfg.world != 1) throw Error(SHM_ERR_INVALID, "spd_solve is a single-process test entry point");
        if (m_ < 1 || m_ > 4096 || (form != 0 && form != 1)) throw Error(SHM_ERR_INVALID, "spd_solve: m in [1, 4096], form 0 (factor) or 1 (invert)");
        const int mp_ = (m_ + kGJ - 1) / kGJ * kGJ;
        if (form == 0 && !ldl_applies(mp_ / kGJ)) throw Error(SHM_ERR_INVALID, "spd_solve: the factorisation serves fewer than 64 pivot blocks");
        HIPCHK(hipSetDevice(cfg.device));
        hipStream_t st = stream2;
        DevArray<double> M, Pd, panels, vecs;
        M.alloc((size_t)mp_ * mp_);
        vecs.alloc((size_t)5 * mp_);
        HIPCHK(hipMemsetAsync(M.p, 0, (size_t)mp_ * mp_ * sizeof(double), st));
        HIPCHK(hipMemsetAsync(vecs.p, 0, (size_t)5 * mp_ * sizeof(double), st));
        HIPCHK(hipMemcpy2DAsync(M.p, (size_t)mp_ * sizeof(double), S, (size_t)m_ * sizeof(double), (size_t)m_ * sizeof(double), (size_t)m_, hipMemcpyHostToDevice, st));
        HIPCHK(hipMemcpyAsync(vecs.p, rhs, (size_t)m_ * sizeof(double), hipMemcpyHostToDevice, st));
        if (mp_ > m_) hipLaunchKernelGGL(set_diagonal_kernel, dim3((unsigned)((mp_ - m_ + kBlock - 1) / kBlock)), dim3(kBlock), 0, st, M.p, mp_, m_, mp_, 1.0);
        if (form == 0) {
            enqueue_ldl_factor(M.p, mp_, Pd, panels);
            apply_ldl(st, m_, mp_, M.p, Pd.p, vecs.p + 2 * (size_t)mp_, vecs.p, vecs.p + mp_);
        } else {
            enqueue_gj_invert(M.p, mp_, true);
            launch_ginv_matvec<double>(st, m_, m_, mp_, M.p, vecs.p, vecs.p + mp_);
        }
        HIPCHK(hipGetLastError());
        int f = 0;
        HIPCHK(hipMemcpyAsync(&f, gjFlag.p, sizeof(int), hipMemcpyDeviceToHost, st));
        HIPCHK(hipMemcpyAsync(u, vecs.p + mp_, (size_t)m_ * sizeof(double), hipMemcpyDeviceToHost, st));
        HIPCHK(hipStreamSynchronize(st));
        *flag = f;
    }

    void apply_projector(double* v) override {
        need_problem();
        if (cfg.world != 1) throw Error(SHM_ERR_INVALID, "apply_projector is a single-process test entry point");
        HIPCHK(hipSetDevice(cfg.device));
        build_constraints(plan_inputs(nullptr), Plan());
        upload_owned(v, 1);
        std::vector<int> nparts(slabs.size(), 0);
        launch_projection(nparts);
        HIPCHK(hipGetLastError());
        have_div = true;
        copy_owned_to_host(SHM_FIELD_DIV, v);
        have_div = false;
    }

    std::vector<double> iso_vertices;
    std::vector<int64_t> iso_triangles;

    void isosurface(double iso, int method, int64_t* nv, int64_t* nt) override {
        need_problem();
        if (method != SHM_ISO_MARCHING_CUBES && method != SHM_ISO_MARCHING_TETS) throw Error(SHM_ERR_INVALID, fmt("isosurface: unknown method %d", method));
        const bool mc = method == SHM_ISO_MARCHING_CUBES;
        if (!have_phi) throw Error(SHM_ERR_STATE, "no phi: shm_grid_solve has not completed");
        HIPCHK(hipSetDevice(cfg.device));
        halo_exchange(ARR_Q);
        iso_vertices.clear();
        iso_triangles.clear();
        std::unordered_map<uint64_t, int64_t> weld;
        for (Slab<T>& sl : slabs) {
            IsoParams P;
            P.n = n; P.nzl = sl.nzl; P.k0 = sl.k0;
            for (int a = 0; a < 3; a++) P.bbox_min[a] = bbox_min[a];
            P.cell = cell; P.iso = iso;
            DevArray<unsigned long long> counter, keys, sortk;
            DevArray<double> pos;
            counter.alloc(1);
            HIPCHK(hipMemsetAsync(counter.p, 0, sizeof(unsigned long long), stream));
            const size_t ncells = (size_t)(n - 1) * (n - 1) * (size_t)std::max(0, std::min(sl.nzl, n - 1 - sl.k0));
            const int grid = grid_for(ncells, 8192);
            if (mc) hipLaunchKernelGGL((iso_mc_kernel<T, false>), dim3(grid), dim3(kBlock), 0, stream, P, sl.q.p, counter.p, (double*)nullptr, (unsigned long long*)nullptr,
                                       (unsigned long long*)nullptr, 0ULL);
            else hipLaunchKernelGGL((iso_kernel<T, false>), dim3(grid), dim3(kBlock), 0, stream, P, sl.q.p, counter.p, (double*)nullptr, (unsigned long long*)nullptr,
                                    (unsigned long long*)nullptr, 0ULL);
            unsigned long long ntri = 0;
            HIPCHK(hipMemcpyAsync(&ntri, counter.p, sizeof ntri, hipMemcpyDeviceToHost, stream));
            HIPCHK(hipStreamSynchronize(stream));
            if (ntri == 0) continue;
            pos.alloc(ntri * 9);
            keys.alloc(ntri * 3);
            sortk.alloc(ntri);
            HIPCHK(hipMemsetAsync(counter.p, 0, sizeof(unsigned long long), stream));
            if (mc) hipLaunchKernelGGL((iso_mc_kernel<T, true>), dim3(grid), dim3(kBlock), 0, stream, P, sl.q.p, counter.p, pos.p, keys.p, sortk.p, ntri);
// ... 1020 lines not shown
```

signed-heat-3d_amd/grid_abi.py:

```python
from __future__ import annotations

import ctypes as C
import os

import numpy as np

SHM_F64, SHM_F32 = 64, 32
_HERE = os.path.dirname(os.path.abspath(__file__))

STATUS_NAMES = {0: "SHM_OK", 1: "SHM_ERR_INVALID", 2: "SHM_ERR_HIP", 3: "SHM_ERR_NOMEM", 4: "SHM_ERR_BREAKDOWN",
                5: "SHM_ERR_NOCONV", 6: "SHM_ERR_RCCL", 7: "SHM_ERR_STATE", 8: "SHM_ERR_SINGULAR"}

ABI_SYMBOLS = ["shm_grid_owned_planes", "shm_grid_create", "shm_grid_destroy", "shm_grid_last_error", "shm_grid_abi_version", "shm_grid_set_problem",
               "shm_grid_solve", "shm_grid_get_phi", "shm_grid_compute_distance", "shm_grid_run_conv", "shm_grid_run_conv_arith", "shm_grid_run_divergence",
               "shm_grid_get_field", "shm_grid_get_field_planes", "shm_grid_apply_laplacian", "shm_grid_set_phi", "shm_grid_get_constraints", "shm_grid_get_schur", "shm_grid_spd_solve", "shm_grid_apply_projector", "shm_grid_apply_preconditioner", "shm_grid_isosurface", "shm_grid_isosurface_ex", "shm_grid_get_isosurface",
               "shm_grid_isosurface_indexed", "shm_grid_get_isosurface_indexed", "shm_grid_get_isosurface_indexed_device",
               "shm_grid_label_mesh_device", "shm_grid_isosurface_components", "shm_grid_get_isosurface_components", "shm_grid_isosurface_keep_components",
               "shm_grid_sample", "shm_grid_sample_device", "shm_grid_raycast", "shm_grid_raycast_device",
               "shm_grid_redistance", "shm_grid_get_redistanced", "shm_grid_get_redistanced_device", "shm_grid_redistance_exact", "shm_grid_isosurface_indexed_psi",
               "shm_grid_closest_point", "shm_grid_closest_point_device",
               "shm_grid_audit_step1", "shm_comm_unique_id", "shm_plan_slab", "shm_step1_plane_weights", "shm_plan_slab_weighted"]


class ShmError(RuntimeError):
    def __init__(self, status, message):
        super().__init__("%s: %s" % (STATUS_NAMES.get(status, status), message))
        self.status = status


class _Config(C.Structure):
    _fields_ = [("device", C.c_int32), ("precision", C.c_int32), ("local_slabs", C.c_int32), ("rank", C.c_int32),
                ("world", C.c_int32), ("verbose", C.c_int32), ("rccl_unique_id", C.c_void_p), ("slab_plan", C.c_int32)]


class _Sources(C.Structure):
    _fields_ = [("S", C.c_int64), ("pos", C.c_void_p), ("wnormal", C.c_void_p), ("area", C.c_void_p), ("lam", C.c_double)]


class _Grid(C.Structure):
    _fields_ = [("n", C.c_int32), ("bbox_min", C.c_double * 3), ("cell", C.c_double)]


class _Opts(C.Structure):
    _fields_ = [("fast_integration", C.c_int32), ("scrub_nonfinite", C.c_int32), ("tol", C.c_double), ("max_iters", C.c_int32),
                ("check_every", C.c_int32), ("preconditioner", C.c_int32), ("solver", C.c_int32), ("step1_arith", C.c_int32),
                ("dual_form", C.c_int32), ("step1_budget", C.c_double)]


class ShmStats(C.Structure):
    _fields_ = [("n", C.c_int32), ("m", C.c_int32), ("S", C.c_int64), ("iters", C.c_int32), ("rel_residual", C.c_double),
                ("shift", C.c_double), ("ms_conv", C.c_double), ("ms_div", C.c_double), ("ms_setup", C.c_double), ("ms_wait_setup", C.c_double),
                ("ms_pcg", C.c_double), ("ms_shift", C.c_double), ("ms_total", C.c_double), ("ms_stencil_avg", C.c_double),
                ("ms_update_xr_avg", C.c_double), ("ms_project_avg", C.c_double), ("ms_update_p_avg", C.c_double),
                ("ms_precond_avg", C.c_double), ("kernel_samples", C.c_int32), ("preconditioner", C.c_int32),
                ("solver", C.c_int32), ("bytes_per_iter", C.c_double), ("cg_form", C.c_int32), ("pairs_fp64", C.c_double), ("pairs_fp32", C.c_double), ("conv_launches", C.c_int32), ("pairs_redone", C.c_double)]

    def as_dict(self):
        return {k: getattr(self, k) for k, _ in self._fields_}


class ShmStep1Audit(C.Structure):
    _fields_ = [("n_audited", C.c_int64), ("n_not_owned", C.c_int64), ("n_nonfinite", C.c_int64), ("n_out_of_zone", C.c_int64),
                ("n_finite_mismatch", C.c_int64), ("max_dy", C.c_double), ("worst_node", C.c_int64), ("worst_ratio", C.c_double), ("min_ratio", C.c_double),
                ("budget", C.c_double), ("step1_arith", C.c_int32), ("within_budget", C.c_int32), ("ms", C.c_double)]

    def as_dict(self):
        return {k: getattr(self, k) for k, _ in self._fields_}


class ShmRedistanceStats(C.Structure):
    _fields_ = [("n_frozen", C.c_int64), ("n_reached", C.c_int64), ("n_nonfinite", C.c_int64), ("n_block_updates", C.c_int64), ("n_rounds", C.c_int32),
                ("reserved", C.c_int32), ("max_abs", C.c_double), ("isovalue", C.c_double), ("band", C.c_double), ("ms", C.c_double)]

    def as_dict(self):
        return {k: getattr(self, k) for k, _ in self._fields_ if k != "reserved"}


class ShmRedistanceExactStats(C.Structure):
    _fields_ = [("n_vertices", C.c_int64), ("n_triangles", C.c_int64), ("n_reached", C.c_int64), ("n_candidate_pairs", C.c_int64), ("max_abs", C.c_double),
                ("isovalue", C.c_double), ("band", C.c_double), ("ms", C.c_double)]

    def as_dict(self):
        return {k: getattr(self, k) for k, _ in self._fields_}


class ShmIsoComponent(C.Structure):
    _fields_ = [("first_vertex", C.c_int64), ("n_vertices", C.c_int64), ("n_triangles", C.c_int64), ("area", C.c_double), ("volume", C.c_double),
                ("lo", C.c_double * 3), ("hi", C.c_double * 3), ("touches_box", C.c_int32), ("reserved", C.c_int32)]


ISO_COMPONENT_DTYPE = np.dtype([("first_vertex", "<i8"), ("n_vertices", "<i8"), ("n_triangles", "<i8"), ("area", "<f8"), ("volume", "<f8"),
                                ("lo", "<f8", (3,)), ("hi", "<f8", (3,)), ("touches_box", "<i4"), ("reserved", "<i4")])
assert ISO_COMPONENT_DTYPE.itemsize == C.sizeof(ShmIsoComponent) == 96


def largest_components_mask(comps, keep_largest=None, min_triangles=None):
    nc = len(comps)
    mask = np.ones(nc, dtype=np.uint8)
    if min_triangles is not None:
        mask &= (comps["n_triangles"] >= int(min_triangles)).astype(np.uint8)
    if keep_largest is not None:
        order = np.lexsort((comps["first_vertex"], -comps["n_triangles"]))
        top = np.zeros(nc, dtype=np.uint8)
        top[order[:max(0, int(keep_largest))]] = 1
        mask &= top
    return mask


def lib_path():
    return os.environ.get("SHM_GRID_LIB") or os.path.join(_HERE, "lib", "libshm_grid.so")


_LIB = None


def load_library():
    global _LIB
    if _LIB is not None:
        return _LIB
    path = lib_path()
    if not os.path.exists(path):
        raise OSError("libshm_grid.so not built: run `python -c 'import __graft_entry__ as g; g.build()'` (%s)" % path)
    lib = C.CDLL(path)
    lib.shm_grid_last_error.restype = C.c_char_p
    lib.shm_grid_last_error.argtypes = [C.c_void_p]
    lib.shm_grid_create.argtypes = [C.POINTER(_Config), C.POINTER(C.c_void_p)]
    lib.shm_grid_destroy.argtypes = [C.c_void_p]
    lib.shm_grid_destroy.restype = None
    lib.shm_grid_set_problem.argtypes = [C.c_void_p, C.POINTER(_Sources), C.POINTER(_Grid)]
    lib.shm_grid_solve.argtypes = [C.c_void_p, C.POINTER(_Opts), C.POINTER(ShmStats)]
    lib.shm_grid_get_phi.argtypes = [C.c_void_p, C.c_void_p, C.POINTER(C.c_int32), C.POINTER(C.c_int32)]
    lib.shm_grid_compute_distance.argtypes = [C.c_void_p, C.POINTER(_Sources), C.POINTER(_Grid), C.POINTER(_Opts), C.c_void_p,
                                              C.POINTER(ShmStats)]
    lib.shm_grid_run_conv.argtypes = [C.c_void_p]
    lib.shm_grid_run_conv_arith.argtypes = [C.c_void_p, C.c_int32]
    lib.shm_grid_run_divergence.argtypes = [C.c_void_p, C.c_int32]
    lib.shm_grid_get_field.argtypes = [C.c_void_p, C.c_int, C.c_void_p]
    lib.shm_grid_get_field_planes.argtypes = [C.c_void_p, C.c_int, C.c_int32, C.c_int32, C.c_void_p]
    lib.shm_grid_apply_laplacian.argtypes = [C.c_void_p, C.c_void_p, C.c_void_p]
    lib.shm_grid_set_phi.argtypes = [C.c_void_p, C.c_void_p]
    lib.shm_grid_get_constraints.argtypes = [C.c_void_p, C.c_void_p, C.c_void_p, C.POINTER(C.c_int32)]
    lib.shm_grid_get_schur.argtypes = [C.c_void_p, C.c_void_p, C.POINTER(C.c_int32)]
    if hasattr(lib, "shm_grid_spd_solve"):
        lib.shm_grid_spd_solve.argtypes = [C.c_void_p, C.c_void_p, C.c_int32, C.c_void_p, C.c_int32, C.c_void_p, C.POINTER(C.c_int32)]
    lib.shm_grid_apply_projector.argtypes = [C.c_void_p, C.c_void_p]
    lib.shm_grid_apply_preconditioner.argtypes = [C.c_void_p, C.c_void_p, C.c_void_p]
    lib.shm_grid_isosurface.argtypes = [C.c_void_p, C.c_double, C.POINTER(C.c_int64), C.POINTER(C.c_int64)]
    lib.shm_grid_isosurface_ex.argtypes = [C.c_void_p, C.c_double, C.c_int32, C.POINTER(C.c_int64), C.POINTER(C.c_int64)]
    lib.shm_grid_get_isosurface.argtypes = [C.c_void_p, C.c_void_p, C.c_void_p]
    lib.shm_grid_sample.argtypes = [C.c_void_p, C.c_int64, C.c_void_p, C.c_void_p, C.c_void_p, C.POINTER(C.c_int64)]
    lib.shm_grid_sample_device.argtypes = [C.c_void_p, C.c_int64, C.c_void_p, C.c_void_p, C.c_void_p, C.POINTER(C.c_int64)]
    if hasattr(lib, "shm_grid_isosurface_indexed"):
        lib.shm_grid_isosurface_indexed.argtypes = [C.c_void_p, C.c_double, C.POINTER(C.c_int64), C.POINTER(C.c_int64)]
        lib.shm_grid_get_isosurface_indexed.argtypes = [C.c_void_p, C.c_void_p, C.c_void_p]
        lib.shm_grid_get_isosurface_indexed_device.argtypes = [C.c_void_p, C.c_void_p, C.c_void_p]
    if hasattr(lib, "shm_grid_label_mesh_device"):
        lib.shm_grid_label_mesh_device.argtypes = [C.c_void_p, C.c_int64, C.c_int64, C.c_void_p, C.c_void_p, C.POINTER(C.c_int64)]
        lib.shm_grid_isosurface_components.argtypes = [C.c_void_p, C.POINTER(C.c_int64)]
        lib.shm_grid_get_isosurface_components.argtypes = [C.c_void_p, C.c_void_p, C.c_void_p, C.c_void_p]
        lib.shm_grid_isosurface_keep_components.argtypes = [C.c_void_p, C.c_void_p, C.POINTER(C.c_int64), C.POINTER(C.c_int64)]
    if hasattr(lib, "shm_grid_audit_step1"):
        lib.shm_grid_audit_step1.argtypes = [C.c_void_p, C.c_int64, C.c_void_p, C.c_void_p, C.c_void_p, C.POINTER(ShmStep1Audit)]
        lib.shm_audit_sample_nodes.argtypes = [C.c_int32, C.c_int32, C.c_int32, C.c_int64, C.c_uint64, C.c_void_p]
        lib.shm_audit_sample_nodes.restype = C.c_int64
    if hasattr(lib, "shm_grid_raycast"):
        lib.shm_grid_raycast.argtypes = [C.c_void_p, C.c_int64, C.c_void_p, C.c_void_p, C.c_double, C.c_double, C.c_double, C.c_void_p, C.c_void_p, C.POINTER(C.c_int64)]
        lib.shm_grid_raycast_device.argtypes = lib.shm_grid_raycast.argtypes
    if hasattr(lib, "shm_grid_redistance"):
        lib.shm_grid_redistance.argtypes = [C.c_void_p, C.c_double, C.c_double, C.POINTER(ShmRedistanceStats)]
        lib.shm_grid_get_redistanced.argtypes = [C.c_void_p, C.c_void_p]
        lib.shm_grid_get_redistanced_device.argtypes = [C.c_void_p, C.c_void_p]
    if hasattr(lib, "shm_grid_redistance_exact"):
        lib.shm_grid_redistance_exact.argtypes = [C.c_void_p, C.c_double, C.c_double, C.POINTER(ShmRedistanceExactStats)]
        lib.shm_grid_isosurface_indexed_psi.argtypes = [C.c_void_p, C.c_double, C.POINTER(C.c_int64), C.POINTER(C.c_int64)]
    if hasattr(lib, "shm_grid_closest_point"):
        lib.shm_grid_closest_point.argtypes = [C.c_void_p, C.c_int64, C.c_void_p, C.c_double, C.c_void_p, C.c_void_p, C.c_void_p, C.POINTER(C.c_int64)]
        lib.shm_grid_closest_point_device.argtypes = lib.shm_grid_closest_point.argtypes
    lib.shm_grid_owned_planes.argtypes = [C.c_void_p, C.POINTER(C.c_int32), C.POINTER(C.c_int32)]
    lib.shm_comm_unique_id.argtypes = [C.c_void_p]
    lib.shm_plan_slab.argtypes = [C.c_int32, C.c_int32, C.c_int32, C.POINTER(C.c_int32), C.POINTER(C.c_int32)]
    lib.shm_plan_slab.restype = None
    lib.shm_step1_plane_weights.argtypes = [C.c_void_p, C.c_void_p, C.c_int32, C.c_void_p]
    lib.shm_plan_slab_weighted.argtypes = [C.c_int32, C.c_int32, C.c_int32, C.c_void_p, C.c_int32, C.POINTER(C.c_int32), C.POINTER(C.c_int32)]
    lib.shm_plan_slab_weighted.restype = None
    _LIB = lib
    return lib


def plan_slab(n, nslabs, slab):
    lib = load_library()
    k0, k1 = C.c_int32(), C.c_int32()
    lib.shm_plan_slab(n, nslabs, slab, C.byref(k0), C.byref(k1))
    return k0.value, k1.value


def audit_sample_nodes(n, k_begin, k_end, count, seed=0):
    lib = load_library()
    out = np.empty(max(0, min(int(count), max(0, int(k_end) - int(k_begin)) * int(n) * int(n))), dtype=np.int64)
    got = lib.shm_audit_sample_nodes(int(n), int(k_begin), int(k_end), int(out.size), int(seed) & 0xFFFFFFFFFFFFFFFF, out.ctypes.data) if out.size else 0
    return out[:got]


def step1_plane_weights(pos, wnormal, lam, n, bbox_min, cell, precision=SHM_F64):
    lib = load_library()
    pos, wn = _f64(pos).reshape(-1), _f64(wnormal).reshape(-1)
    area = np.zeros(pos.size // 3)
    src = _Sources(pos.size // 3, pos.ctypes.data, wn.ctypes.data, area.ctypes.data, float(lam))
    g = _Grid(int(n), (C.c_double * 3)(*[float(x) for x in bbox_min]), float(cell))
    w = np.zeros(int(n))
    rc = lib.shm_step1_plane_weights(C.byref(src), C.byref(g), int(precision), w.ctypes.data)
    if rc != 0:
        raise ShmError(rc, "shm_step1_plane_weights: invalid argument")
    return w


def plan_slab_weighted(n, nslabs, slab, weights, granule):
    lib = load_library()
    w = _f64(weights)
    k0, k1 = C.c_int32(), C.c_int32()
    lib.shm_plan_slab_weighted(int(n), int(nslabs), int(slab), w.ctypes.data, int(granule), C.byref(k0), C.byref(k1))
    return k0.value, k1.value


def comm_unique_id():
    lib = load_library()
# ... 52 lines not shown
        self._chk(self._lib.shm_grid_set_problem(self._h, C.byref(src), C.byref(g)))
        self.n, self.S, self.cell = int(n), S, float(cell)

    def owned_planes(self):
        k0, k1 = C.c_int32(), C.c_int32()
        self._chk(self._lib.shm_grid_owned_planes(self._h, C.byref(k0), C.byref(k1)))
        return k0.value, k1.value

    PRECOND = {"auto": 0, "none": 1, "dct": 2}

    SOLVER = {"auto": 0, "primal": 1, "dual": 2, "dual_slabs": 3}

    STEP1 = {"auto": 0, "exact_f64": 1, "reference_f64": 2}

    DUAL_FORM = {"auto": 0, "direct": 1, "explicit_s_cg": 2, "through_grid": 3}

    def solve(self, tol=0.0, max_iters=0, check_every=0, scrub=True, fast=False, allow_noconv=False, precond="auto", solver="auto", step1="auto",
              dual_form="auto", step1_budget=0.0):
        o = _Opts(int(fast), int(scrub), float(tol), int(max_iters), int(check_every), self.PRECOND[precond], self.SOLVER[solver], self.STEP1[step1],
                  self.DUAL_FORM[dual_form], float(step1_budget))
        st = ShmStats()
        self._chk(self._lib.shm_grid_solve(self._h, C.byref(o), C.byref(st)), allow=(5,) if allow_noconv else ())
        return st

    def _owned_count(self):
        k0, k1 = self.owned_planes()
        return (k1 - k0) * self.n * self.n

    def get_phi(self):
        out = np.empty(self._owned_count(), dtype=np.float64)
        k0, k1 = C.c_int32(), C.c_int32()
        self._chk(self._lib.shm_grid_get_phi(self._h, out.ctypes.data, C.byref(k0), C.byref(k1)))
        return out, (k0.value, k1.value)

    def run_conv(self, step1="auto"):
        if step1 == "auto":
            self._chk(self._lib.shm_grid_run_conv(self._h))
        else:
            self._chk(self._lib.shm_grid_run_conv_arith(self._h, self.STEP1[step1]))

    def run_divergence(self, scrub=True):
        self._chk(self._lib.shm_grid_run_divergence(self._h, int(scrub)))

    def get_field(self, which):
        out = np.empty(self._owned_count(), dtype=np.float64)
        self._chk(self._lib.shm_grid_get_field(self._h, int(which), out.ctypes.data))
        return out

    def get_field_planes(self, which, k_begin, k_end):
        out = np.empty((int(k_end) - int(k_begin)) * self.n * self.n, dtype=np.float64)
        self._chk(self._lib.shm_grid_get_field_planes(self._h, int(which), int(k_begin), int(k_end), out.ctypes.data))
        return out

    def apply_laplacian(self, u):
        u = _f64(u).reshape(-1)
        out = np.empty_like(u)
        self._chk(self._lib.shm_grid_apply_laplacian(self._h, u.ctypes.data, out.ctypes.data))
        return out

    def set_phi(self, phi):
        if phi is None:
            self._chk(self._lib.shm_grid_set_phi(self._h, None))
            return
        phi = _f64(phi).reshape(-1)
        if self.n and phi.size != self.n ** 3:
            raise ValueError("set_phi: phi must hold n^3 = %d values, got %d" % (self.n ** 3, phi.size))
        self._chk(self._lib.shm_grid_set_phi(self._h, phi.ctypes.data))

    def get_constraints(self):
        nodes = np.empty(8 * self.S, dtype=np.int64)
        coeffs = np.empty(8 * self.S, dtype=np.float64)
        m = C.c_int32()
        self._chk(self._lib.shm_grid_get_constraints(self._h, nodes.ctypes.data, coeffs.ctypes.data, C.byref(m)))
        return nodes[:8 * m.value].reshape(-1, 8).copy(), coeffs[:8 * m.value].reshape(-1, 8).copy()

    def get_schur(self):
        m = len(self.get_constraints()[0])
        out = np.empty((m, m), dtype=np.float64)
        mm = C.c_int32(0)
        self._chk(self._lib.shm_grid_get_schur(self._h, out.ctypes.data, C.byref(mm)))
        assert mm.value == m
        return out

    def spd_solve(self, S, rhs, form="factor"):
        S = np.ascontiguousarray(S, dtype=np.float64)
        rhs = np.ascontiguousarray(rhs, dtype=np.float64).reshape(-1)
        m = S.shape[0]
        if S.shape != (m, m) or rhs.size != m:
            raise ValueError("spd_solve: S must be m x m and rhs hold m values")
        u = np.empty(m, dtype=np.float64)
        flag = C.c_int32(0)
        self._chk(self._lib.shm_grid_spd_solve(self._h, S.ctypes.data, m, rhs.ctypes.data, {"factor": 0, "invert": 1}[form], u.ctypes.data, C.byref(flag)))
        return u, flag.value

    def apply_projector(self, v):
        v = _f64(v).reshape(-1).copy()
        self._chk(self._lib.shm_grid_apply_projector(self._h, v.ctypes.data))
        return v

    def apply_preconditioner(self, v):
        v = _f64(v).reshape(-1)
        out = np.empty_like(v)
        self._chk(self._lib.shm_grid_apply_preconditioner(self._h, v.ctypes.data, out.ctypes.data))
        return out

    ISO_METHOD = {"marching_cubes": 0, "marching_tets": 1}

    def isosurface(self, isovalue=0.0, method="marching_cubes"):
        nv, nt = C.c_int64(), C.c_int64()
        if method == "marching_cubes":
            self._chk(self._lib.shm_grid_isosurface(self._h, float(isovalue), C.byref(nv), C.byref(nt)))
        else:
            self._chk(self._lib.shm_grid_isosurface_ex(self._h, float(isovalue), self.ISO_METHOD[method], C.byref(nv), C.byref(nt)))
        V = np.empty((nv.value, 3), dtype=np.float64)
        F = np.empty((nt.value, 3), dtype=np.int64)
        self._chk(self._lib.shm_grid_get_isosurface(self._h, V.ctypes.data, F.ctypes.data))
        return V, F

    def isosurface_indexed(self, isovalue=0.0, device=False, keep_largest=None, min_triangles=None):
        nv, nt = C.c_int64(), C.c_int64()
        self._chk(self._lib.shm_grid_isosurface_indexed(self._h, float(isovalue), C.byref(nv), C.byref(nt)))
        if keep_largest is not None or min_triangles is not None:
            nv.value, nt.value = self.isosurface_keep(largest_components_mask(self.isosurface_components(), keep_largest, min_triangles))
        return self.get_isosurface_indexed(nv.value, nt.value, device)

    def get_isosurface_indexed(self, nv, nt, device=False):
        if not device:
            V = np.empty((nv, 3), dtype=np.float64)
            F = np.empty((nt, 3), dtype=np.int64)
            self._chk(self._lib.shm_grid_get_isosurface_indexed(self._h, V.ctypes.data if nv else None, F.ctypes.data if nt else None))
            return V, F
        import torch
        if not torch.cuda.is_available():
            raise RuntimeError("isosurface_indexed: torch sees no HIP device (was torch imported after libshm_grid.so was loaded? import it first)")
        dev = torch.device("cuda", self.device)
        V = torch.empty((nv, 3), dtype=torch.float64 if self.precision == SHM_F64 else torch.float32, device=dev)
        F = torch.empty((nt, 3), dtype=torch.int64, device=dev)
        self._chk(self._lib.shm_grid_get_isosurface_indexed_device(self._h, V.data_ptr() if nv else None, F.data_ptr() if nt else None))
        return V, F

    def label_mesh_device(self, triangles, nv):
        import torch
        if not torch.cuda.is_available():
            raise RuntimeError("label_mesh_device: torch sees no HIP device (was torch imported after libshm_grid.so was loaded? import it first)")
        if triangles.dtype != torch.int64 or not triangles.is_contiguous() or triangles.numel() % 3:
            raise ValueError("label_mesh_device: triangles must be a contiguous int64 tensor of 3 nt indices")
        nt = triangles.numel() // 3
        root = torch.empty(int(nv), dtype=torch.int64, device=triangles.device)
        if triangles.is_cuda:
            torch.cuda.current_stream(triangles.device).synchronize()
        nc = C.c_int64()
        self._chk(self._lib.shm_grid_label_mesh_device(self._h, int(nv), nt, triangles.data_ptr() if nt else None, root.data_ptr() if nv else None, C.byref(nc)))
        return root, nc.value

    def isosurface_components(self, labels=False):
        nc = C.c_int64()
        self._chk(self._lib.shm_grid_isosurface_components(self._h, C.byref(nc)))
        comps = np.zeros(nc.value, dtype=ISO_COMPONENT_DTYPE)
        if not labels:
            self._chk(self._lib.shm_grid_get_isosurface_components(self._h, comps.ctypes.data if nc.value else None, None, None))
            return comps
        self._chk(self._lib.shm_grid_get_isosurface_components(self._h, comps.ctypes.data if nc.value else None, None, None))
        nv, nt = int(comps["n_vertices"].sum()), int(comps["n_triangles"].sum())
        tc = np.empty(nt, dtype=np.int64)
        vc = np.empty(nv, dtype=np.int64)
        self._chk(self._lib.shm_grid_get_isosurface_components(self._h, comps.ctypes.data if nc.value else None, tc.ctypes.data if nt else None,
# ... 183 lines not shown
```

Measured before the change: 714.0 million.

## Reuse the K^+ spectrum across the dual solve's first and final grid solves

Adds a kplus_reuse plan path for the single-slab explicit-S dual solve. The first preconditioner application saves the scaled spectrum (DCT_FUSED_SAVE), and the final solve subtracts it (DCT_FUSED_SUB) instead of redoing the full transform. S·ones is precomputed once so the initial residual needs no dense S mat-vec. The DCT kernels gain two fused modes, and the change adds a spectrum buffer, an extra active-tile build, and a get_multipliers test entry point. The risk is correctness of the spectral subtraction and the extra memory traffic for the saved spectrum.

```diff
diff --git a/include/shm_grid.h b/include/shm_grid.h
--- a/include/shm_grid.h
+++ b/include/shm_grid.h
@@ -130,6 +130,7 @@
 shm_status shm_grid_set_phi(shm_solver* s, const double* phi );
 shm_status shm_grid_get_constraints(shm_solver* s, int64_t* nodes, double* coeffs, int32_t* m);
 shm_status shm_grid_get_schur(shm_solver* s, double* out, int32_t* m);
+shm_status shm_grid_get_multipliers(shm_solver* s, double* out, int32_t* m);
 shm_status shm_grid_spd_solve(shm_solver* s, const double* S, int32_t m, const double* rhs, int32_t form, double* u, int32_t* flag);
 shm_status shm_grid_apply_projector(shm_solver* s, double* v);
 
diff --git a/signed-heat-3d_amd/csrc/shm_dct.hip.h b/signed-heat-3d_amd/csrc/shm_dct.hip.h
--- a/signed-heat-3d_amd/csrc/shm_dct.hip.h
+++ b/signed-heat-3d_amd/csrc/shm_dct.hip.h
@@ -53,7 +53,7 @@
 #define SHM_DCT_DBG(P, bit) 0
 #endif
 
-enum DctMode : int { DCT_FWD = 0, DCT_INV = 1, DCT_FUSED = 2 };
+enum DctMode : int { DCT_FWD = 0, DCT_INV = 1, DCT_FUSED = 2, DCT_FUSED_SAVE = 3, DCT_FUSED_SUB = 4 };
 template <int LOG2N, int TB > constexpr int dct_lc() {
     return LOG2N >= 10 ? (TB == 8 ? 4 : SHM_DCT_LC10_F32) : (LOG2N == 8 ? SHM_DCT_LC8 : (LOG2N == 9 ? (TB == 8 ? SHM_DCT_LC9_F64 : SHM_DCT_LC9_F32) : 8));
 }
@@ -88,6 +88,8 @@
 
 template <int LOG2N, int TB> constexpr size_t dct_stage_bytes() { return (size_t)(1 << LOG2N) * (size_t)(2 * dct_lc<LOG2N, TB>()) * (size_t)TB; }
 
+template <bool WAVE, int N, int LC> __device__ __forceinline__ int dct_spec_slot(int c, int k) { return WAVE ? c * N + k : k * LC + c; }
+
 template <typename TP, int LOG2N, int R, int NS, int SIGN>
 __device__ __forceinline__ void dct_fft_pass(Cplx<TP>* buf, const Cplx<TP>* tw, int tid) {
     constexpr int LC = dct_lc<LOG2N, (int)sizeof(TP)>();
@@ -175,7 +177,12 @@
                                                            const Cplx<TP>* __restrict__ tw_g, const Cplx<TP>* __restrict__ om_g,
                                                            const TP* __restrict__ lam_g, const TOut* __restrict__ dot_with,
                                                            double* __restrict__ partials, const int* __restrict__ tile_list ,
-                                                           const unsigned* __restrict__ elem_mask ) {
+                                                           const unsigned* __restrict__ elem_mask ,
+                                                           Cplx<TP>* __restrict__ spec ) {
+    constexpr bool kFused = MODE >= DCT_FUSED;
+    static_assert(!(MODE > DCT_FUSED) || !SHM_DCT_SPECTRAL_ORIG, "the spectrum is kept by the current spectral step only");
+    const unsigned* const mask_in = MODE == DCT_FUSED_SAVE ? nullptr : elem_mask;
+    const unsigned* const mask_out = MODE == DCT_FUSED_SUB ? nullptr : elem_mask;
     extern __shared__ __attribute__((aligned(16))) char smem[];
     constexpr int LC = dct_lc<LOG2N, (int)sizeof(TP)>(), kFftRow = LC + 1, kFftLC = LC;
     constexpr int n = 1 << LOG2N, L = 2 * LC, LOG2L = ilog2(L), total = n * L;
@@ -191,17 +198,17 @@
     constexpr int kSpStep = kBlock / kFftLC;
     constexpr int kSpIters = (n / 2 + 1 + kSpStep - 1) / kSpStep;
     Cplx<TP> sp_om[(MODE == DCT_FWD || !SHM_DCT_HOIST) ? 1 : kSpIters];
-    TP sp_lam[(MODE == DCT_FUSED && SHM_DCT_HOIST) ? kSpIters : 1];
+    TP sp_lam[(kFused && SHM_DCT_HOIST) ? kSpIters : 1];
     TP sp_lam_n = (TP)0;
     if (MODE != DCT_FWD && SHM_DCT_HOIST) {
 #pragma unroll
         for (int i = 0; i < kSpIters; i++) {
             const int k = min((tid >> ilog2(kFftLC)) + i * kSpStep, n / 2);
             sp_om[i] = om_g[k];
-            if (MODE == DCT_FUSED) sp_lam[i] = lam_g[k];
-        }
-    }
-    if (MODE == DCT_FUSED) sp_lam_n = (TP)2 * lam_g[n / 2];
+            if (kFused) sp_lam[i] = lam_g[k];
+        }
+    }
+    if (kFused) sp_lam_n = (TP)2 * lam_g[n / 2];
     static_assert(!PF || !SEG, "the prefetching variant serves plain layouts");
     static_assert(!PF || (sizeof(TIn) == sizeof(TP) && (total * sizeof(TIn)) % (16 * kBlock) == 0), "the prefetching variant moves whole 16-byte chunks of same-width input");
     TIn* stage = reinterpret_cast<TIn*>(smem + dct_lds_bytes<LOG2N, (int)sizeof(TP)>());
@@ -285,7 +292,7 @@
             const int idx = tid + (a0 + a) * kBlock;
             if (total % kBlock == 0 || idx < total) {
                 const int j = elem_of(idx);
-                v[a] = (!SHM_DCT_DBG(P, 4) && (!elem_mask || ((elem_mask[j >> 5] >> (j & 31)) & 1u))) ? (TP)*in_at(in, a0 + a, idx) : (TP)0;
+                v[a] = (!SHM_DCT_DBG(P, 4) && (!mask_in || ((mask_in[j >> 5] >> (j & 31)) & 1u))) ? (TP)*in_at(in, a0 + a, idx) : (TP)0;
             }
         }
 #pragma unroll
@@ -301,7 +308,26 @@
     __syncthreads();
 
     constexpr bool kWaveFft = dct_wave_fft<LOG2N>();
-    if ((MODE == DCT_FWD || MODE == DCT_FUSED) && !SHM_DCT_DBG(P, 1)) {
+    constexpr int kSpLines = kWaveFft ? kFftLC / (kBlock / kWave) : 1;
+    constexpr int kSpCount = kWaveFft ? (n / 2 + kWave) / kWave : kSpIters;
+    auto sp_line = [&](int cl) { return kWaveFft ? (tid >> 6) + (kBlock / kWave) * cl : (tid & (kFftLC - 1)); };
+    auto sp_k = [&](int i) { return kWaveFft ? (tid & 63) + i * kWave : (tid >> ilog2(kFftLC)) + i * kSpStep; };
+    constexpr bool kSpecAhead = MODE == DCT_FUSED_SUB && LOG2N <= 8;
+    constexpr int kSpUnroll = kSpecAhead ? kSpCount : 1;
+    Cplx<TP>* const spec_t = MODE > DCT_FUSED ? spec + (size_t)t * (size_t)(n * kFftLC) : nullptr;
+    Cplx<TP> spec_k[kSpecAhead ? kSpLines : 1][kSpecAhead ? kSpCount : 1], spec_n[kSpecAhead ? kSpLines : 1][kSpecAhead ? kSpCount : 1];
+    if constexpr (kSpecAhead) {
+#pragma unroll
+        for (int cl = 0; cl < kSpLines; cl++) {
+#pragma unroll
+            for (int i = 0; i < kSpCount; i++) {
+                const int c = sp_line(cl), k = min(sp_k(i), n / 2), nk = (n - k) & (n - 1);
+                spec_k[cl][i] = spec_t[dct_spec_slot<kWaveFft, n, kFftLC>(c, k)];
+                spec_n[cl][i] = spec_t[dct_spec_slot<kWaveFft, n, kFftLC>(c, nk)];
+            }
+        }
+    }
+    if ((MODE == DCT_FWD || kFused) && !SHM_DCT_DBG(P, 1)) {
         if constexpr (kWaveFft) dct_fft_wave<TP, LOG2N, -1>(buf, tw, tid);
         else dct_fft<TP, LOG2N, -1>(buf, tw, tid);
     }
@@ -333,7 +359,7 @@
             const int nk = (n - k) & (n - 1);
             const Cplx<TP> omk = om_g[k], omn = om_g[nk];
             TP xa_k, xb_k, xa_n, xb_n;
-            if (MODE == DCT_FUSED) {
+            if (kFused) {
                 const Cplx<TP> zk = buf[k * kFftRow + c], znk = buf[nk * kFftRow + c];
                 dct_fwd_post<TP>(zk, znk, omk, xa_k, xb_k);
                 dct_fwd_post<TP>(znk, zk, omn, xa_n, xb_n);
@@ -367,13 +393,12 @@
 #else
     if (!SHM_DCT_DBG(P, 2)) {
         const int kx0 = (t % P.tiles_a) * L, ky = P.ky0 + t / P.tiles_a;
-        constexpr int kSpLines = kWaveFft ? kFftLC / (kBlock / kWave) : 1;
 #pragma unroll
         for (int cl = 0; cl < kSpLines; cl++) {
-        const int c = kWaveFft ? (tid >> 6) + (kBlock / kWave) * cl : (tid & (kFftLC - 1));
+        const int c = sp_line(cl);
         const int kxa = kx0 + 2 * c, kxb = kxa + 1;
         TP lxy_a = (TP)0, lxy_b = (TP)0, sa = (TP)0, sb = (TP)0;
-        if (MODE == DCT_FUSED) {
+        if (kFused) {
             const TP lky = lam_g[ky];
             lxy_a = lam_g[kxa] + lky;
             lxy_b = lam_g[kxb] + lky;
@@ -381,15 +406,15 @@
             sa = (kxa == 0 ? (TP)0.5 : (TP)1) * sy * (TP)P.inv_n3_8;
             sb = sy * (TP)P.inv_n3_8;
         }
-#pragma unroll 1
-        for (int i = 0; i < (kWaveFft ? (n / 2 + kWave) / kWave : kSpIters); i++) {
-            const int k = kWaveFft ? (tid & 63) + i * kWave : (tid >> ilog2(kFftLC)) + i * kSpStep;
+#pragma unroll kSpUnroll
+        for (int i = 0; i < kSpCount; i++) {
+            const int k = sp_k(i);
             if (k > n / 2) break;
             const int nk = (n - k) & (n - 1);
             const Cplx<TP> omk = SHM_DCT_HOIST ? sp_om[SHM_DCT_HOIST ? i : 0] : om_g[k];
             const Cplx<TP> omn = k == 0 ? omk : Cplx<TP>{-omk.y, -omk.x};
             TP xa_k, xb_k, xa_n, xb_n;
-            if (MODE == DCT_FUSED) {
+            if (kFused) {
                 const Cplx<TP> zk = buf[k * kFftRow + c], znk = buf[nk * kFftRow + c];
                 dct_fwd_post<TP>(zk, znk, omk, xa_k, xb_k);
                 dct_fwd_post<TP>(znk, zk, omn, xa_n, xb_n);
@@ -406,6 +431,21 @@
                 xb_k = xb_k * (sb * szk) * recip(db_k);
                 xa_n = da_n > (TP)0 ? xa_n * (sa * szk) * recip(da_n) : (TP)0;
                 xb_n = xb_n * (sb * szk) * recip(db_n);
+                if constexpr (MODE == DCT_FUSED_SAVE) {
+                    spec_t[dct_spec_slot<kWaveFft, n, kFftLC>(c, k)] = Cplx<TP>{xa_k, xb_k};
+                    if (nk != k) spec_t[dct_spec_slot<kWaveFft, n, kFftLC>(c, nk)] = Cplx<TP>{xa_n, xb_n};
+                }
+                if constexpr (MODE == DCT_FUSED_SUB) {
+                    Cplx<TP> sk, sn;
+                    if constexpr (kSpecAhead) {
+                        sk = spec_k[cl][kSpecAhead ? i : 0];
+                        sn = spec_n[cl][kSpecAhead ? i : 0];
+                    } else {
+                        sk = spec_t[dct_spec_slot<kWaveFft, n, kFftLC>(c, k)];
+                        sn = nk != k ? spec_t[dct_spec_slot<kWaveFft, n, kFftLC>(c, nk)] : sk;
+                    }
+                    xa_k -= sk.x; xb_k -= sk.y; xa_n -= sn.x; xb_n -= sn.y;
+                }
             } else {
                 const Cplx<TP> rk = buf[k * kFftRow + c], rn = buf[nk * kFftRow + c];
                 xa_k = rk.x; xb_k = rk.y; xa_n = rn.x; xb_n = rn.y;
@@ -442,7 +482,7 @@
             if (total % kBlock == 0 || idx < total) {
                 const int l = line_of(idx), j = elem_of(idx);
                 const TP v = reinterpret_cast<const TP*>(&buf[makhoul_slot(j, n) * kFftRow + (l >> 1)])[l & 1];
-                if (!SHM_DCT_DBG(P, 8) && (!elem_mask || ((elem_mask[j >> 5] >> (j & 31)) & 1u))) *out_at(out, a0 + a, idx) = (TOut)v;
+                if (!SHM_DCT_DBG(P, 8) && (!mask_out || ((mask_out[j >> 5] >> (j & 31)) & 1u))) *out_at(out, a0 + a, idx) = (TOut)v;
                 if (DOT) acc += (double)v * (double)dv[a];
             }
         }
diff --git a/signed-heat-3d_amd/csrc/shm_grid.hip b/signed-heat-3d_amd/csrc/shm_grid.hip
--- a/signed-heat-3d_amd/csrc/shm_grid.hip
+++ b/signed-heat-3d_amd/csrc/shm_grid.hip
@@ -188,6 +188,12 @@
         s->impl->get_schur(out, m);
     });
 }
+shm_status shm_grid_get_multipliers(shm_solver* s, double* out, int32_t* m) {
+    return guard(s, [&] {
+        if (!out || !m) throw shm::Error(SHM_ERR_INVALID, "null argument");
+        s->impl->get_multipliers(out, m);
+    });
+}
 shm_status shm_grid_spd_solve(shm_solver* s, const double* S, int32_t m, const double* rhs, int32_t form, double* u, int32_t* flag) {
     return guard(s, [&] {
         if (!S || !rhs || !u || !flag) throw shm::Error(SHM_ERR_INVALID, "null argument");
diff --git a/signed-heat-3d_amd/csrc/shm_host.hip.h b/signed-heat-3d_amd/csrc/shm_host.hip.h
--- a/signed-heat-3d_amd/csrc/shm_host.hip.h
+++ b/signed-heat-3d_amd/csrc/shm_host.hip.h
@@ -515,6 +515,7 @@
     virtual void apply_projector(double*) = 0;
     virtual void apply_preconditioner(const double*, double*) = 0;
     virtual void get_schur(double*, int32_t*) = 0;
+    virtual void get_multipliers(double*, int32_t*) = 0;
     virtual void spd_solve(const double*, int32_t, const double*, int32_t, double*, int32_t*) = 0;
     virtual void isosurface(double, int, int64_t*, int64_t*) = 0;
     virtual void get_isosurface(double*, int64_t*) = 0;
diff --git a/signed-heat-3d_amd/csrc/shm_kernels.hip.h b/signed-heat-3d_amd/csrc/shm_kernels.hip.h
--- a/signed-heat-3d_amd/csrc/shm_kernels.hip.h
+++ b/signed-heat-3d_amd/csrc/shm_kernels.hip.h
@@ -1004,14 +1004,16 @@
 }
 
 static __global__ __launch_bounds__(kDualBlock) void dual_init_residual_kernel(int m, const double* __restrict__ g, const double* __restrict__ Smu,
-                                                                        double* __restrict__ r, double* __restrict__ sc, int set_rr0 = 1) {
+                                                                        double* __restrict__ r, double* __restrict__ sc, int set_rr0 = 1,
+                                                                        const double* __restrict__ sumb = nullptr) {
     __shared__ double lds[17];
+    const double c = sumb ? *sumb / (double)m : 1.;
     double s = 0.;
-    for (int a = threadIdx.x; a < m; a += kDualBlock) s += g[a] - Smu[a];
+    for (int a = threadIdx.x; a < m; a += kDualBlock) s += g[a] - c * Smu[a];
     const double mean = block_sum_1024(s, lds) / (double)m;
     double rr = 0.;
     for (int a = threadIdx.x; a < m; a += kDualBlock) {
-        const double v = g[a] - Smu[a] - mean;
+        const double v = g[a] - c * Smu[a] - mean;
         r[a] = v;
         rr += v * v;
     }
diff --git a/signed-heat-3d_amd/csrc/shm_plan.h b/signed-heat-3d_amd/csrc/shm_plan.h
--- a/signed-heat-3d_amd/csrc/shm_plan.h
+++ b/signed-heat-3d_amd/csrc/shm_plan.h
@@ -18,6 +18,7 @@
     bool no_dense_s = false;
     bool dense_s_always = false;
     int s_form = 0;
+    int kplus_reuse = 1;
     int tl_min_m = 6144;
 };
 template <typename Get> PlanKnobs plan_knobs(Get knob) {
@@ -27,6 +28,8 @@
     k.dense_s_always = knob("SHM_DUAL_DENSE_S_ALWAYS") != nullptr;
     const char* s_form = knob("SHM_S_FORM");
     if (s_form != nullptr) k.s_form = std::strcmp(s_form, "invert") == 0 ? 1 : std::strcmp(s_form, "factor") == 0 ? 2 : 0;
+    const char* kplus = knob("SHM_KPLUS_REUSE");
+    if (kplus != nullptr) k.kplus_reuse = std::strcmp(kplus, "dense") == 0 ? 2 : atoi(kplus) != 0 ? 1 : 0;
     if (knob("SHM_TL_MIN_M")) k.tl_min_m = atoi(knob("SHM_TL_MIN_M"));
     return k;
 }
@@ -60,6 +63,8 @@
     int dual_form = SHM_DUAL_THROUGH_GRID;
     bool explicit_S = false;
     bool two_level = false;
+    bool kplus_reuse = false;
+    bool kplus_dense_halves = false;
     bool s_factor = false;
     double est_setup_ms = -1., est_step1_ms = -1.;
 };
@@ -145,6 +150,8 @@
     p.explicit_S = plan_explicit_S(in, m, direct);
     p.dual_form = direct ? SHM_DUAL_DIRECT : p.explicit_S ? SHM_DUAL_EXPLICIT_S_CG : SHM_DUAL_THROUGH_GRID;
     p.two_level = !direct && m > in.knobs.tl_min_m;
+    p.kplus_reuse = in.knobs.kplus_reuse != 0 && p.dual_requested && p.explicit_S && in.total_slabs == 1 && in.fft_available;
+    p.kplus_dense_halves = p.kplus_reuse && in.knobs.kplus_reuse == 2;
     p.s_factor = direct && (in.knobs.s_form == 2 || (in.knobs.s_form == 0 && kSFactorDefault)) && ldl_applies((m + kLdlTile - 1) / kLdlTile);
 }
 
diff --git a/signed-heat-3d_amd/csrc/shm_solver.hip.h b/signed-heat-3d_amd/csrc/shm_solver.hip.h
--- a/signed-heat-3d_amd/csrc/shm_solver.hip.h
+++ b/signed-heat-3d_amd/csrc/shm_solver.hip.h
@@ -150,6 +150,9 @@
     std::vector<int> h_rowX;
     bool have_S = false;
     DevArray<double> Sinv, Sinv_ones ;
+    DevArray<double> S_ones;
+    bool have_mu = false;
+    int sweeps_dense = 0, sweeps_sparse = 0, matvecs = 0;
     DevArray<double> ldlP, ldlPanels, ldlWork;
     PlanIn plan_in;
     Plan plan;
@@ -956,6 +959,7 @@
         const auto th0 = std::chrono::steady_clock::now();
         plan_in = in;
         plan = p;
+        have_mu = false;
         plan_setup(plan_in, plan);
         auto lap = [&](const char* what) { log("[shm]   setup %-28s %.2f ms", what, std::chrono::duration<double, std::milli>(std::chrono::steady_clock::now() - th0).count()); };
         if (plan.green_early) {
@@ -1021,6 +1025,13 @@
         }
         lap("slab uploads");
         if (total_slabs == 1 && fft_available() && !dual_direct) build_active_tiles(index.unode);
+        else if (plan.kplus_reuse) {
+            std::vector<int64_t> touched(lists[0].node_id.begin(), lists[0].node_id.end());
+            for (int64_t& g : touched) g -= (int64_t)slabs[0].plane;
+            build_active_tiles(touched);
+        }
+        if (plan.kplus_reuse)
+            HIPCHK(hipMemsetAsync(slabs[0].p.p, 0, slabs[0].ntot * sizeof(T), stream));
         lap("active tiles");
         Bptr.upload(B.ptr, stream);
         Bcol.upload(B.col, stream);
@@ -1359,6 +1370,11 @@
         const unsigned mt = (unsigned)((m + 15) / 16);
         hipLaunchKernelGGL(schur_assemble_kernel, dim3(mt, mt), dim3(kBlock), 0, st, m, mp, n, P, d_rowX.p, d_rowT.p, gs_T.p, Sdense.p, plan.setup_prio);
         HIPCHK(hipGetLastError());
+        if (plan.kplus_reuse) {
+            S_ones.alloc((size_t)2 * mp);
+            hipLaunchKernelGGL(fill_kernel, dim3((unsigned)((m + kBlock - 1) / kBlock)), dim3(kBlock), 0, st, S_ones.p + mp, m, 1.0);
+            launch_ginv_matvec<double>(st, m, m, mp, Sdense.p, S_ones.p + mp, S_ones.p);
+        }
         if (dual_direct) {
             Sinv.alloc((size_t)mp * mp);
             HIPCHK(hipMemcpyAsync(Sinv.p, Sdense.p, (size_t)mp * mp * sizeof(double), hipMemcpyDeviceToDevice, st));
@@ -1668,20 +1684,20 @@
     }
 
     template <int MODE, typename TIn, typename TOut, bool DOT, int LOG2N, bool XPASS>
-    void launch_dct_n(const DctParams& P, int ntiles, const TIn* in, TOut* out, const TOut* dotw, double* partials, const int* tile_list, const unsigned* elem_mask) {
-        constexpr bool kCanSeg = !XPASS && MODE != DCT_FUSED && !DOT;
+    void launch_dct_n(const DctParams& P, int ntiles, const TIn* in, TOut* out, const TOut* dotw, double* partials, const int* tile_list, const unsigned* elem_mask, TP* spec) {
+        constexpr bool kCanSeg = !XPASS && MODE < DCT_FUSED && !DOT;
         const bool seg = P.in.seg_shift < 30 || P.out.seg_shift < 30;
         if (seg && !kCanSeg) throw Error(SHM_ERR_INVALID, "DCT: segmented layout in a sweep that does not support it");
         if constexpr (kCanSeg) {
             if (seg) {
-                launch_dct_pf<MODE, TIn, TOut, DOT, LOG2N, XPASS, true, false>(P, ntiles, in, out, dotw, partials, tile_list, elem_mask);
+                launch_dct_pf<MODE, TIn, TOut, DOT, LOG2N, XPASS, true, false>(P, ntiles, in, out, dotw, partials, tile_list, elem_mask, spec);
                 return;
             }
         }
-        launch_dct_pf<MODE, TIn, TOut, DOT, LOG2N, XPASS, false, false>(P, ntiles, in, out, dotw, partials, tile_list, elem_mask);
+        launch_dct_pf<MODE, TIn, TOut, DOT, LOG2N, XPASS, false, false>(P, ntiles, in, out, dotw, partials, tile_list, elem_mask, spec);
     }
     template <int MODE, typename TIn, typename TOut, bool DOT, int LOG2N, bool XPASS, bool SEG, bool PF>
-    void launch_dct_pf(const DctParams& P, int ntiles, const TIn* in, TOut* out, const TOut* dotw, double* partials, const int* tile_list, const unsigned* elem_mask) {
+    void launch_dct_pf(const DctParams& P, int ntiles, const TIn* in, TOut* out, const TOut* dotw, double* partials, const int* tile_list, const unsigned* elem_mask, TP* spec) {
         static uint64_t configured = 0;
         constexpr size_t lds = dct_lds_bytes<LOG2N, (int)sizeof(TP)>() + (PF ? dct_stage_bytes<LOG2N, (int)sizeof(TP)>() : 0);
         const uint64_t dev_bit = 1ull << (cfg.device & 63);
@@ -1693,19 +1709,19 @@
         Q.ntiles = ntiles;
         Q.debug_skip = 0;
         hipLaunchKernelGGL((dct_lines_kernel<TP, TIn, TOut, MODE, DOT, LOG2N, XPASS, SEG, PF>), dim3((unsigned)ntiles), dim3(kBlock), lds, stream, Q, in, out, d_tw.p, d_om.p, d_lam.p, dotw,
-                           partials, tile_list, elem_mask);
+                           partials, tile_list, elem_mask, reinterpret_cast<Cplx<TP>*>(spec));
     }
     template <int MODE, typename TIn, typename TOut, bool DOT, bool XPASS>
     void launch_dct(const DctParams& P, int ntiles, const TIn* in, TOut* out, const TOut* dotw, double* partials, const int* tile_list = nullptr,
-                    const unsigned* elem_mask = nullptr) {
+                    const unsigned* elem_mask = nullptr, TP* spec = nullptr ) {
         switch (log2n) {
-            case 4: launch_dct_n<MODE, TIn, TOut, DOT, 4, XPASS>(P, ntiles, in, out, dotw, partials, tile_list, elem_mask); break;
-            case 5: launch_dct_n<MODE, TIn, TOut, DOT, 5, XPASS>(P, ntiles, in, out, dotw, partials, tile_list, elem_mask); break;
-            case 6: launch_dct_n<MODE, TIn, TOut, DOT, 6, XPASS>(P, ntiles, in, out, dotw, partials, tile_list, elem_mask); break;
-            case 7: launch_dct_n<MODE, TIn, TOut, DOT, 7, XPASS>(P, ntiles, in, out, dotw, partials, tile_list, elem_mask); break;
-            case 8: launch_dct_n<MODE, TIn, TOut, DOT, 8, XPASS>(P, ntiles, in, out, dotw, partials, tile_list, elem_mask); break;
-            case 9: launch_dct_n<MODE, TIn, TOut, DOT, 9, XPASS>(P, ntiles, in, out, dotw, partials, tile_list, elem_mask); break;
-            case 10: launch_dct_n<MODE, TIn, TOut, DOT, 10, XPASS>(P, ntiles, in, out, dotw, partials, tile_list, elem_mask); break;
+            case 4: launch_dct_n<MODE, TIn, TOut, DOT, 4, XPASS>(P, ntiles, in, out, dotw, partials, tile_list, elem_mask, spec); break;
+            case 5: launch_dct_n<MODE, TIn, TOut, DOT, 5, XPASS>(P, ntiles, in, out, dotw, partials, tile_list, elem_mask, spec); break;
+            case 6: launch_dct_n<MODE, TIn, TOut, DOT, 6, XPASS>(P, ntiles, in, out, dotw, partials, tile_list, elem_mask, spec); break;
+            case 7: launch_dct_n<MODE, TIn, TOut, DOT, 7, XPASS>(P, ntiles, in, out, dotw, partials, tile_list, elem_mask, spec); break;
+            case 8: launch_dct_n<MODE, TIn, TOut, DOT, 8, XPASS>(P, ntiles, in, out, dotw, partials, tile_list, elem_mask, spec); break;
+            case 9: launch_dct_n<MODE, TIn, TOut, DOT, 9, XPASS>(P, ntiles, in, out, dotw, partials, tile_list, elem_mask, spec); break;
+            case 10: launch_dct_n<MODE, TIn, TOut, DOT, 10, XPASS>(P, ntiles, in, out, dotw, partials, tile_list, elem_mask, spec); break;
             default: throw Error(SHM_ERR_INVALID, "DCT preconditioner: unsupported grid size");
         }
     }
@@ -1830,6 +1846,7 @@
                 }
             }
         }
+        sweeps_dense += 5;
         return dot ? tiles_slab : 0;
     }
 
@@ -2013,6 +2030,75 @@
         Q.in = plain_addr(0, (long long)L * nn, 0, nn, 1);
         Q.out = plain_addr((long long)sl.plane, (long long)L * nn, 0, nn, 1);
         launch_dct<DCT_INV, TP, T, false, true>(Q, sl.n_act_x, sl.S4.p, arr(sl, out_sel), (const T*)nullptr, nullptr, sl.act_x.p);
+        sweeps_sparse += 5;
+    }
+
+    void launch_kplus_first(int in_sel, int out_sel) {
+        Slab<T>& sl = slabs[0];
+        const long long nn = n, plane = (long long)n * n;
+        const int L = dct_lines_for(log2n, (int)sizeof(TP));
+        const int tiles_all = (int)(plane / L);
+        const bool sparse = !plan.kplus_dense_halves;
+        const int nx = sparse ? sl.n_act_x : tiles_all, ny = sparse ? sl.n_act_y : tiles_all;
+        const int *lx = sparse ? sl.act_x.p : nullptr, *ly = sparse ? sl.act_y.p : nullptr;
+        const unsigned* zmask = sparse ? sl.act_z.p : nullptr;
+        DctParams Q{};
+        Q.inv_n3_8 = 8.0 / ((double)n * n * n);
+        Q.ky0 = 0;
+        Q.tiles_a = tiles_all;
+        Q.in = plain_addr((long long)sl.plane, (long long)L * nn, 0, nn, 1);
+        Q.out = plain_addr(0, (long long)L * nn, 0, nn, 1);
+        launch_dct<DCT_FWD, T, TP, false, true>(Q, tiles_all, arr(sl, in_sel), sl.W1.p, (const TP*)nullptr, nullptr);
+        Q.tiles_a = n / L;
+        Q.in = plain_addr(0, L, plane, 1, nn);
+        Q.out = Q.in;
+        launch_dct<DCT_FWD, TP, TP, false, false>(Q, tiles_all, sl.W1.p, sl.W1.p, (const TP*)nullptr, nullptr);
+        Q.in = plain_addr(0, L, nn, 1, plane);
+        Q.out = Q.in;
+        launch_dct<DCT_FUSED_SAVE, TP, TP, false, false>(Q, tiles_all, sl.W1.p, sl.W1.p, (const TP*)nullptr, nullptr, nullptr, zmask, sl.S4.p);
+        Q.in = plain_addr(0, L, plane, 1, nn);
+        Q.out = Q.in;
+        launch_dct<DCT_INV, TP, TP, false, false>(Q, ny, sl.W1.p, sl.W1.p, (const TP*)nullptr, nullptr, ly);
+        Q.tiles_a = tiles_all;
+        Q.in = plain_addr(0, (long long)L * nn, 0, nn, 1);
+        Q.out = plain_addr((long long)sl.plane, (long long)L * nn, 0, nn, 1);
+        launch_dct<DCT_INV, TP, T, false, true>(Q, nx, sl.W1.p, arr(sl, out_sel), (const T*)nullptr, nullptr, lx);
+        sweeps_dense += sparse ? 3 : 5;
+        sweeps_sparse += sparse ? 2 : 0;
+    }
+    void launch_kplus_second(int in_sel, int out_sel) {
+        Slab<T>& sl = slabs[0];
+        const long long nn = n, plane = (long long)n * n;
+        const int L = dct_lines_for(log2n, (int)sizeof(TP));
+        const int tiles_all = (int)(plane / L);
+        const bool sparse = !plan.kplus_dense_halves;
+        const int nx = sparse ? sl.n_act_x : tiles_all, ny = sparse ? sl.n_act_y : tiles_all;
+        const int *lx = sparse ? sl.act_x.p : nullptr, *ly = sparse ? sl.act_y.p : nullptr;
+        const unsigned* zmask = sparse ? sl.act_z.p : nullptr;
+        TP *xf = sparse ? sl.S1.p : sl.W1.p, *yf = sparse ? sl.S2.p : sl.W1.p;
+        DctParams Q{};
+        Q.inv_n3_8 = 8.0 / ((double)n * n * n);
+        Q.ky0 = 0;
+        Q.tiles_a = tiles_all;
+        Q.in = plain_addr((long long)sl.plane, (long long)L * nn, 0, nn, 1);
+        Q.out = plain_addr(0, (long long)L * nn, 0, nn, 1);
+        launch_dct<DCT_FWD, T, TP, false, true>(Q, nx, arr(sl, in_sel), xf, (const TP*)nullptr, nullptr, lx);
+        Q.tiles_a = n / L;
+        Q.in = plain_addr(0, L, plane, 1, nn);
+        Q.out = Q.in;
+        launch_dct<DCT_FWD, TP, TP, false, false>(Q, ny, xf, yf, (const TP*)nullptr, nullptr, ly);
+        Q.in = plain_addr(0, L, nn, 1, plane);
+        Q.out = Q.in;
+        launch_dct<DCT_FUSED_SUB, TP, TP, false, false>(Q, tiles_all, yf, sl.W1.p, (const TP*)nullptr, nullptr, nullptr, zmask, sl.S4.p);
+        Q.in = plain_addr(0, L, plane, 1, nn);
+        Q.out = Q.in;
+        launch_dct<DCT_INV, TP, TP, false, false>(Q, tiles_all, sl.W1.p, sl.W1.p, (const TP*)nullptr, nullptr);
+        Q.tiles_a = tiles_all;
+        Q.in = plain_addr(0, (long long)L * nn, 0, nn, 1);
+        Q.out = plain_addr((long long)sl.plane, (long long)L * nn, 0, nn, 1);
+        launch_dct<DCT_INV, TP, T, false, true>(Q, tiles_all, sl.W1.p, arr(sl, out_sel), (const T*)nullptr, nullptr);
+        sweeps_dense += sparse ? 3 : 5;
+        sweeps_sparse += sparse ? 2 : 0;
     }
 
     void solve_dual(const shm_opts& o, shm_stats* st, SolveClock& clk) {
@@ -2040,7 +2126,10 @@
                 hipLaunchKernelGGL(dual_direction_kernel, dim3(1), dim3(kDualBlock), 0, stream, m, init, mv(sl, V_R), mv(sl, V_Z), mv(sl, V_P), sl.sc.p);
             }
         };
-        launch_precond(false, ARR_R, ARR_Z);
+        const bool reuse = plan.kplus_reuse && have_S && total_slabs == 1 && !gemm_dct() && slabs[0].n_act_x > 0;
+        sweeps_dense = sweeps_sparse = matvecs = 0;
+        if (reuse) launch_kplus_first(ARR_R, ARR_Z);
+        else launch_precond(false, ARR_R, ARR_Z);
         gather(ARR_Z);
         for (Slab<T>& sl : slabs) {
             HIPCHK(hipMemcpyAsync(mv(sl, V_G), sl.red.p + 1, (size_t)m * sizeof(double), hipMemcpyDeviceToDevice, stream));
@@ -2062,8 +2151,10 @@
             for (Slab<T>& sl : slabs) HIPCHK(hipMemsetAsync(sl.p.p, 0, sl.ntot * sizeof(T), stream));
         auto apply_S = [&](int vec) {
             for (Slab<T>& sl : slabs) launch_ginv_matvec<double>(stream, m, m, mp, Sdense.p, mv(sl, vec), sl.red.p + 1);
+            matvecs++;
         };
-        if (dense_S) apply_S(V_MU);
+        if (dense_S && reuse) {
+        } else if (dense_S) apply_S(V_MU);
         else {
             scatter(V_MU, ARR_P, 0);
             if (sparse_ok) launch_precond_sparse(ARR_P, ARR_Z);
@@ -2071,7 +2162,8 @@
             gather(ARR_Z);
         }
         for (Slab<T>& sl : slabs)
-            hipLaunchKernelGGL(dual_init_residual_kernel, dim3(1), dim3(kDualBlock), 0, stream, m, mv(sl, V_G), sl.red.p + 1, mv(sl, V_R), sl.sc.p, 1);
+            hipLaunchKernelGGL(dual_init_residual_kernel, dim3(1), dim3(kDualBlock), 0, stream, m, mv(sl, V_G), dense_S && reuse ? (const double*)S_ones.p : (const double*)sl.red.p + 1,
+                               mv(sl, V_R), sl.sc.p, 1, dense_S && reuse ? (const double*)sl.pq.p : (const double*)nullptr);
         const bool direct = plan.dual_form == SHM_DUAL_DIRECT && dense_S;
         if (!direct) precondition(1);
         HIPCHK(hipGetLastError());
@@ -2081,7 +2173,10 @@
         Residual res;
         bool converged = false, breakdown = false;
         auto finish = [&]() {
-            if (gemm_dct()) {
+            if (reuse) {
+                scatter(V_MU, ARR_P, 0);
+                launch_kplus_second(ARR_P, ARR_X);
+            } else if (gemm_dct()) {
                 for (Slab<T>& sl : slabs)
                     hipLaunchKernelGGL((negate_kernel<T>), dim3(grid_for(sl.ntot, 4096)), dim3(kBlock), 0, stream, sl.ntot, sl.r.p, sl.q.p);
                 scatter(V_MU, ARR_Q, 1);
@@ -2118,7 +2213,7 @@
                 tm.mark(1, stream);
                 apply_S(V_MU);
                 for (Slab<T>& sl : slabs)
-                    hipLaunchKernelGGL(dual_init_residual_kernel, dim3(1), dim3(kDualBlock), 0, stream, m, mv(sl, V_G), sl.red.p + 1, mv(sl, V_R), sl.sc.p, 0);
+                    hipLaunchKernelGGL(dual_init_residual_kernel, dim3(1), dim3(kDualBlock), 0, stream, m, mv(sl, V_G), sl.red.p + 1, mv(sl, V_R), sl.sc.p, 0, (const double*)nullptr);
                 tm.mark(2, stream);
                 tm.end();
                 it++;
@@ -2156,7 +2251,9 @@
             log("[shm] dual it=%d rel_res=%.3e", it, res.rel());
         }
         if (!finished) finish();
+        log("[shm] dual solve phase: kplus_reuse %d, transform sweeps %d dense + %d sparse, S mat-vecs %d", (int)reuse, sweeps_dense, sweeps_sparse, matvecs);
         have_phi = true;
+        have_mu = true;
         have_div = false;
         if (st) {
             fill_phase_stats(st, clk, e_pcg, e_end, it, res.rel());
@@ -2653,6 +2750,16 @@
         if (!have_S) throw Error(SHM_ERR_STATE, "no explicit Schur complement for this problem (several slabs, more than 16384 rows, or n = 2^k where the plan applies S through the grid: n > 512, or the estimate of plan_explicit_S without SHM_DUAL_DENSE_S_ALWAYS)");
         HIPCHK(hipMemcpy2DAsync(out, (size_t)m * sizeof(double), Sdense.p, (size_t)mp * sizeof(double), (size_t)m * sizeof(double), (size_t)m, hipMemcpyDeviceToHost, stream2));
         HIPCHK(hipStreamSynchronize(stream2));
+    }
+
+    void get_multipliers(double* out, int32_t* m_out) override {
+        need_problem();
+        if (cfg.world != 1) throw Error(SHM_ERR_INVALID, "get_multipliers is a single-process test entry point");
+        if (!have_mu || !have_constraints) throw Error(SHM_ERR_STATE, "no dual solve has run on this handle's current constraints");
+        HIPCHK(hipSetDevice(cfg.device));
+        *m_out = m;
+        HIPCHK(hipMemcpyAsync(out, slabs[0].dv.p, (size_t)m * sizeof(double), hipMemcpyDeviceToHost, stream));
+        HIPCHK(hipStreamSynchronize(stream));
     }
 
     void spd_solve(const double* S, int32_t m_, const double* rhs, int32_t form, double* u, int32_t* flag) override {
diff --git a/signed-heat-3d_amd/grid_abi.py b/signed-heat-3d_amd/grid_abi.py
--- a/signed-heat-3d_amd/grid_abi.py
+++ b/signed-heat-3d_amd/grid_abi.py
@@ -13,7 +13,7 @@
 
 ABI_SYMBOLS = ["shm_grid_owned_planes", "shm_grid_create", "shm_grid_destroy", "shm_grid_last_error", "shm_grid_abi_version", "shm_grid_set_problem",
                "shm_grid_solve", "shm_grid_get_phi", "shm_grid_compute_distance", "shm_grid_run_conv", "shm_grid_run_conv_arith", "shm_grid_run_divergence",
-               "shm_grid_get_field", "shm_grid_get_field_planes", "shm_grid_apply_laplacian", "shm_grid_set_phi", "shm_grid_get_constraints", "shm_grid_get_schur", "shm_grid_spd_solve", "shm_grid_apply_projector", "shm_grid_apply_preconditioner", "shm_grid_isosurface", "shm_grid_isosurface_ex", "shm_grid_get_isosurface",
+               "shm_grid_get_field", "shm_grid_get_field_planes", "shm_grid_apply_laplacian", "shm_grid_set_phi", "shm_grid_get_constraints", "shm_grid_get_schur", "shm_grid_get_multipliers", "shm_grid_spd_solve", "shm_grid_apply_projector", "shm_grid_apply_preconditioner", "shm_grid_isosurface", "shm_grid_isosurface_ex", "shm_grid_get_isosurface",
                "shm_grid_isosurface_indexed", "shm_grid_get_isosurface_indexed", "shm_grid_get_isosurface_indexed_device",
                "shm_grid_label_mesh_device", "shm_grid_isosurface_components", "shm_grid_get_isosurface_components", "shm_grid_isosurface_keep_components",
                "shm_grid_sample", "shm_grid_sample_device", "shm_grid_raycast", "shm_grid_raycast_device",
@@ -141,6 +141,8 @@
     lib.shm_grid_set_phi.argtypes = [C.c_void_p, C.c_void_p]
     lib.shm_grid_get_constraints.argtypes = [C.c_void_p, C.c_void_p, C.c_void_p, C.POINTER(C.c_int32)]
     lib.shm_grid_get_schur.argtypes = [C.c_void_p, C.c_void_p, C.POINTER(C.c_int32)]
+    if hasattr(lib, "shm_grid_get_multipliers"):
+        lib.shm_grid_get_multipliers.argtypes = [C.c_void_p, C.c_void_p, C.POINTER(C.c_int32)]
     if hasattr(lib, "shm_grid_spd_solve"):
         lib.shm_grid_spd_solve.argtypes = [C.c_void_p, C.c_void_p, C.c_int32, C.c_void_p, C.c_int32, C.c_void_p, C.POINTER(C.c_int32)]
     lib.shm_grid_apply_projector.argtypes = [C.c_void_p, C.c_void_p]
@@ -359,6 +361,12 @@
         assert mm.value == m
         return out
 
+    def get_multipliers(self):
+        out = np.empty(max(self.S, 1), dtype=np.float64)
+        m = C.c_int32(0)
+        self._chk(self._lib.shm_grid_get_multipliers(self._h, out.ctypes.data, C.byref(m)))
+        return out[:m.value].copy()
+
     def spd_solve(self, S, rhs, form="factor"):
         S = np.ascontiguousarray(S, dtype=np.float64)
         rhs = np.ascontiguousarray(rhs, dtype=np.float64).reshape(-1)
```

New measurement: 717.0 million (median of 6 runs). No clear change (+0.4%).
